# edouardlp/Mask-RCNN-CoreML

Measured on AMD Instinct MI355X. Metric: images/sec (1024x1024, COCO-80), higher is better.
Workload: dtype f32x3

## Files before the change

mask-rcnn-coreml_amd/csrc/conv_dispatch.hip:

```cpp
#include "conv_device.h"
#include "knobs.h"

namespace mrcnn {

void conv_mfma_launch(hipStream_t s, const ConvArgs& a, int mode, int bn, bool wide_waves);
void conv_pp_launch(hipStream_t s, const ConvArgs& a, int mode);
void conv_chain_launch(hipStream_t s, const ConvArgs& p, const ConvArgs& q, int parts, bool wlds, int n_cus);

static inline int conv_wdtype(const ConvDesc& d) { return d.wdtype < 0 ? d.dtype : d.wdtype; }
static inline bool conv_is_split(const ConvDesc& d) { return d.dtype == MRCNN_F32 && (conv_wdtype(d) == MRCNN_F16 || conv_wdtype(d) == MRCNN_F32X3); }
static inline int conv_split_parts(const ConvDesc& d) { return conv_wdtype(d) == MRCNN_F32X3 ? 3 : 2; }
static inline bool conv_is_f16(const ConvDesc& d) { return d.dtype == MRCNN_F16 && (d.wdtype < 0 || d.wdtype == MRCNN_F16) && !d.out_f32; }
static inline bool is_pointwise(const ConvDesc& d) { return d.KH == 1 && d.KW == 1 && d.stride == 1 && !d.padH && !d.padW; }
static inline bool is_3x3_same(const ConvDesc& d) { return d.KH == 3 && d.KW == 3 && d.stride == 1 && d.padH == 1 && d.padW == 1; }
static inline bool dense_in(const ConvDesc& d, int h, int w, int c) { return d.H == h && d.W == w && d.Cin == c && d.in_sW == c && d.in_sH == (long)w * c && d.in_sB == (long)h * w * c; }
static inline bool dense_out(const ConvDesc& d, int h, int w, int c) { return d.OH == h && d.OW == w && d.Cout == c && d.out_sP == c && d.out_sB == (long)h * w * c; }
static inline bool plain_epilogue(const ConvDesc& d, int act) { return !d.out2 && !d.deconv2 && !d.sel_partial && !d.head_w && d.res_shift == 0 && d.act == act && d.scale && d.shift; }
static inline bool fills_chip(long tiles, int n_cus) { return tiles * 8 >= (long)n_cus * 7; }

static thread_local ConvProfile* g_prof = nullptr;
void conv_set_profiler(ConvProfile* p) { g_prof = p; }
static thread_local int* g_range_flag = nullptr;
void conv_set_range_flag(int* device_flag) { g_range_flag = device_flag; }
void ConvProfile::reset()
{
    for (auto& s : by_tile) s = Slot();
    for (auto& s : by_group) s = Slot();
    by_shape.clear();
    pending.clear();
    used = 0;
}
void ConvProfile::collect()
{
    for (auto& pd : pending) {
        float ms = 0;
        HIP_CHECK(hipEventElapsedTime(&ms, pool[pd.e0], pool[pd.e1]));
        by_tile[pd.tile].launches += 1;
        by_tile[pd.tile].ms += ms;
        by_tile[pd.tile].flops += pd.flops;
        by_tile[pd.tile].bytes += pd.bytes;
        Slot& sh = by_shape[pd.shape];
        sh.launches += 1; sh.ms += ms; sh.flops += pd.flops; sh.bytes += pd.bytes;
        Slot& gr = by_group[pd.group == 1 ? 1 : 0];
        gr.launches += 1; gr.ms += ms; gr.flops += pd.flops; gr.bytes += pd.bytes;
    }
    pending.clear();
    used = 0;
}
ConvProfile::~ConvProfile()
{
    for (auto e : pool) (void)hipEventDestroy(e);
}
static double conv_algorithmic_bytes(const ConvDesc& d, const ConvDesc* sc = nullptr)
{
    const double es = d.dtype == MRCNN_F16 ? 2.0 : 4.0;
    const double ws = conv_wdtype(d) == MRCNN_F32 ? 4.0 : 2.0;
    const double M = (double)d.B * d.OH * d.OW;
    const double ncols = d.deconv2 ? 4.0 * d.Cout : d.Cout;
    double b = 0;
    if (d.algo_k > 0) b += (double)d.B * d.H * d.W * 16.0;
    else b += (d.KH * d.KW == 1 ? M : (double)d.B * d.H * d.W) * d.Cin * es;
    b += ncols * d.KH * d.KW * (d.algo_k > 0 ? (double)d.algo_k / (d.KH * d.KW) : (double)d.Cin) * ws;
    if (d.res) b += M * d.Cout * es / (d.res_shift ? 4.0 : 1.0);
    if (sc) b += M * sc->Cin * es + (double)d.Cout * sc->Cin * ws;
    if (d.head_w) b += M * d.head_cols * 4.0;
    else if (!d.sel_partial) b += M * ncols * (d.out_f32 ? 4.0 : es);
    return b;
}
static int prof_event(ConvProfile* p, hipStream_t s)
{
    if (p->used == (int)p->pool.size()) {
        hipEvent_t e;
        HIP_CHECK(hipEventCreate(&e));
        p->pool.push_back(e);
    }
    HIP_CHECK(hipEventRecord(p->pool[p->used], s));
    return p->used++;
}
struct ProfScope {
    ConvProfile* const prof = (g_prof && g_prof->active) ? g_prof : nullptr;
    const hipStream_t s;
    const int e0;
    explicit ProfScope(hipStream_t s_) : s(s_), e0(prof ? prof_event(prof, s_) : 0) {}
    explicit operator bool() const { return prof != nullptr; }
    void finish(ConvTileClass tile, double flops, int M, int N, int K, int group, double bytes) const
    {
        const int e1 = prof_event(prof, s);
        prof->pending.push_back({tile, flops, e0, e1, {M, N, K, tile}, group, bytes});
    }
};

int conv_n_tile(int Cout)
{
    if (Cout > 64) return 128;
    if (Cout > 32) return 64;
    return 32;
}

static int& g_min_blocks = knob("conv_min_blocks", nullptr, 448);
static int& g_min_blocks_split = knob("conv_min_blocks_split", nullptr, 256, "conv_min_blocks");
static inline int min_blocks_for(bool split_mode) { return split_mode ? g_min_blocks_split : g_min_blocks; }
static int& g_direct = knob("conv_direct", "MRCNN_DIRECT", 3);
static int& g_stem = knob("conv_stem", "MRCNN_STEM", 1);
static int& g_tail_dbg = knob("conv_tail_dbg", "MRCNN_TAIL_DBG", 0);
static int& g_tail = knob("conv_tail", "MRCNN_TAIL", 0);
static int& g_bneck = knob("conv_bneck", "MRCNN_BNECK", 1);
static int& g_bneck_stage = knob("conv_bneck_stage", "MRCNN_BNECK_STAGE", 0);
static int& g_c3h = knob("conv_c3h", "MRCNN_C3H", 1);
int conv_c3h_mode() { return g_c3h; }
bool conv_bneck_enabled() { return g_bneck != 0; }
static int& g_scfuse = knob("conv_scfuse", "MRCNN_SCFUSE", 1);
static int& g_sel_wave = knob("mask_sel_wave", "MRCNN_SEL_WAVE", 1);
int conv_sel_part_cols() { return g_sel_wave ? 64 : 128; }
static int& g_kchunk = knob("conv_kchunk", "MRCNN_KCHUNK", 1);
static int& g_ksplit = knob("conv_ksplit", "MRCNN_KSPLIT", 1);
static int& g_ksplit_below = knob("conv_ksplit_below", "MRCNN_KSPLIT_BELOW", 256);
static int& g_halo = knob("conv_halo", "MRCNN_HALO", 1);
bool conv_halo_enabled() { return g_halo != 0; }
static int& g_chain = knob("conv_chain", "MRCNN_CHAIN", 1);
static int& g_tn4 = knob("conv_tn4", nullptr, -1);

static int& g_pp = knob("conv_pp", "MRCNN_PP", 1);
static int& g_pp_min_tiles = knob("conv_pp_min_tiles", "MRCNN_PP_MIN_TILES", 512);
static int& g_pp_min_kt = knob("conv_pp_min_kt", "MRCNN_PP_MIN_KT", 16);
static int& g_pp_dbg = knob("conv_pp_dbg", "MRCNN_PP_DBG", 0);
static int& g_pp_min_fill = knob("conv_pp_min_fill", "MRCNN_PP_MIN_FILL", 85);
static int& g_pp_split = knob("conv_pp_split", "MRCNN_PP_SPLIT", 0);

static void conv_fill_args(const ConvDesc& d, ConvArgs& a)
{
    const bool half = d.dtype == MRCNN_F16;
    a.in = d.in; a.wgt = d.wgt; a.scale = d.scale; a.shift = d.shift; a.res = d.res; a.out = d.out; a.out2 = d.out2;
    a.in_sB = d.in_sB; a.in_sH = d.in_sH; a.in_sW = d.in_sW;
    a.res_sB = d.res_sB; a.res_sH = d.res_sH; a.res_sW = d.res_sW;
    a.out_sB = d.out_sB; a.out_sP = d.out_sP; a.out_sH = d.out_sH; a.out_sW = d.out_sW;
    a.out2_sB = d.out2_sB; a.out2_sP = d.out2_sP;
    a.B = d.B; a.H = d.H; a.W = d.W; a.Cin = d.Cin; a.KH = d.KH; a.KW = d.KW; a.stride = d.stride; a.padH = d.padH; a.padW = d.padW;
    a.OH = d.OH; a.OW = d.OW; a.Cout = d.Cout;
    a.ncols = d.deconv2 ? 4 * d.Cout : d.Cout;
    a.Ktot = d.KH * d.KW * d.Cin;
    const long M = (long)d.B * d.OH * d.OW;
    MRCNN_REQUIRE(M > 0 && M < (1L << 31) - 256, MRCNN_ERR_SHAPE, "conv: M out of range");
    a.M = (int)M;
    a.res_shift = d.res_shift; a.act = d.act; a.n_split = d.n_split; a.deconv2 = d.deconv2;
    a.out_f32 = (!half || d.out_f32) ? 1 : 0;
    a.range_flag = g_range_flag;
    a.dbg = g_pp_dbg;
    a.sel_w = d.sel_w; a.sel_cid = d.sel_cid; a.sel_partial = d.sel_partial;
    a.kchunks = 1; a.ksplit = 1; a.ks_scratch = nullptr; a.ks_count = nullptr;
    a.sel_part_cols = 128;
    a.sc_in = nullptr; a.sc_wgt = nullptr; a.sc_scale = nullptr; a.sc_shift = nullptr;
    a.sc_in_sB = a.sc_in_sH = a.sc_in_sW = 0; a.sc_H = a.sc_W = a.sc_Cin = 0; a.sc_stride = 1;
}

int conv_k_chunks(const ConvDesc& d)
{
    if (!g_kchunk || !conv_is_split(d) || d.KH != 1 || d.KW != 1 || d.Cin < 2048 || d.Cin % 32 != 0 || d.head_w) return 1;
    int n = d.Cin >= 8192 ? 8 : 4;
    while ((d.Cin / 32) % n) n >>= 1;
    return n;
}

static constexpr size_t KS_BYTES = 64u << 20;
static constexpr int KS_TILES = 8192;
static thread_local ConvScratch* g_scratch = nullptr;
void conv_set_scratch(ConvScratch* c) { g_scratch = c; }
size_t ConvScratch::ks_bytes() { return KS_BYTES; }
void ConvScratch::alloc()
{
    ks_buf.alloc(KS_BYTES);
    ks_cnt.alloc(KS_TILES * sizeof(unsigned));
    HIP_CHECK(hipMemset(ks_cnt.p, 0, KS_TILES * sizeof(unsigned)));
}
ConvScratch* conv_current_scratch() { return g_scratch; }

static int conv_vec_ok(const ConvDesc& d, const ConvArgs& a)
{
    const bool half = d.dtype == MRCNN_F16;
    auto al = [](const void* p, size_t n) { return (reinterpret_cast<uintptr_t>(p) & (n - 1)) == 0; };
    const int cpt = half ? 8 : 4;
    return a.ncols % cpt == 0 && d.out2 == nullptr && d.out_sP % cpt == 0 && d.out_sB % cpt == 0 && al(d.out, 16) &&
               (!d.scale || al(d.scale, 16)) && (!d.shift || al(d.shift, 16)) &&
               (!d.res || (d.res_sW % cpt == 0 && d.res_sH % cpt == 0 && d.res_sB % cpt == 0 && al(d.res, 16))) &&
               (!d.deconv2 || (d.Cout % cpt == 0 && d.out_sH % cpt == 0 && d.out_sW % cpt == 0));
}

static bool conv_shortcut_fusable(const ConvDesc& m, const ConvDesc& sc)
{
    if (!conv_is_split(m) || !conv_is_split(sc) || conv_wdtype(m) != conv_wdtype(sc)) return false;
    if (m.KH != 1 || m.KW != 1 || sc.KH != 1 || sc.KW != 1 || m.padH || m.padW || sc.padH || sc.padW || m.stride != 1) return false;
    if (m.B != sc.B || m.OH != sc.OH || m.OW != sc.OW || m.Cout != sc.Cout || m.Npad != sc.Npad || sc.Cin % 32 != 0) return false;
    if (sc.act != ACT_NONE || sc.res || sc.out2 || sc.deconv2 || sc.sel_partial || sc.head_w || m.out2 || m.deconv2 || m.sel_partial || m.head_w || m.act == ACT_SIGMOID) return false;
    if (m.res != sc.out || m.res_shift != 0 || m.res_sW != sc.out_sP || m.res_sB != sc.out_sB || m.res_sH != (long)m.OW * m.res_sW) return false;
    if (sc.out_sB != (long)sc.OH * sc.OW * sc.out_sP) return false;
    return true;
}

static bool conv_shortcut_rides(const ConvDesc& d_in, const ConvDesc* sc)
{
    bool fuse = sc && g_scfuse && conv_shortcut_fusable(d_in, *sc) && conv_k_chunks(d_in) == 1 && conv_k_chunks(*sc) == 1;
    if (fuse) {
        const int bn_max = conv_n_tile(d_in.Cout);
        int bn = bn_max;
        const long tiles_m = ((long)d_in.B * d_in.OH * d_in.OW + BM_DEFAULT - 1) / BM_DEFAULT;
        while (bn > 32 && tiles_m * (d_in.Npad / bn) < min_blocks_for(true)) bn >>= 1;
        ConvDesc probe = d_in;
        probe.res = nullptr;
        ConvArgs pa;
        conv_fill_args(probe, pa);
        if (bn < 64 || g_direct < 2 || !conv_vec_ok(probe, pa)) fuse = false;
#ifndef MRCNN_CONV_ABLATE
        if (g_pp_dbg) fuse = false;
#endif
    }
    return fuse;
}

void conv_forward(hipStream_t s, const ConvDesc& d_in, const ConvDesc* sc)
{
    const bool fuse = conv_shortcut_rides(d_in, sc);
    if (sc && !fuse) conv_forward(s, *sc, nullptr);
    ConvDesc d = d_in;
    if (fuse) { d.res = nullptr; d.res_sB = d.res_sH = d.res_sW = 0; }
    const bool half = d.dtype == MRCNN_F16;
    const int wdtype = conv_wdtype(d);
    if (half && g_c3h && (d.head_w || d.prefer_c3h || g_c3h == 2) && conv3x3h_eligible(d)) {
        const int n_cus_c3h = device_cu_count();
        const ProfScope prof(s);
        conv3x3h_launch(s, d, g_range_flag, n_cus_c3h);
        if (prof) {
            const double M = (double)d.B * d.OH * d.OW;
            prof.finish(TILE_C3H, 2.0 * M * d.Cout * 9.0 * d.Cin, (int)M, d.Cout, 9 * d.Cin, d.group, conv_algorithmic_bytes(d));
        }
        return;
    }
    const bool split = conv_is_split(d);
    const int parts = conv_split_parts(d);
    MRCNN_REQUIRE(d.dtype == MRCNN_F32 || half, MRCNN_ERR_UNSUPPORTED, "conv: dtype %d", d.dtype);
    MRCNN_REQUIRE(wdtype == d.dtype || split, MRCNN_ERR_UNSUPPORTED, "conv: activation dtype %d with filter dtype %d", d.dtype, wdtype);
    const int bk = half ? 64 : 32;
    MRCNN_REQUIRE(d.Cin % bk == 0, MRCNN_ERR_SHAPE, "conv: Cin %d not a multiple of %d", d.Cin, bk);
    ConvArgs a;
    conv_fill_args(d, a);
    MRCNN_REQUIRE(!d.sel_partial || (d.deconv2 && d.sel_w && d.sel_cid && d.Cout % 128 == 0 && d.Npad == 4 * d.Cout && !d.out2),
                  MRCNN_ERR_INVALID, "conv: the selected-class mode needs a 2x2 transposed convolution with Cout a multiple of 128");
    const int bn_max = conv_n_tile(a.ncols);
    MRCNN_REQUIRE(d.Npad % bn_max == 0 && d.Npad >= a.ncols, MRCNN_ERR_SHAPE, "conv: Npad %d incompatible with tile %d", d.Npad, bn_max);
    a.tiles_m = (a.M + BM_DEFAULT - 1) / BM_DEFAULT;
    int bn = bn_max;
    while (bn > 32 && !d.sel_partial && (long)a.tiles_m * (d.Npad / bn) < min_blocks_for(split)) bn >>= 1;
    if (fuse) {
        a.sc_in = sc->in; a.sc_wgt = sc->wgt; a.sc_scale = sc->scale; a.sc_shift = sc->shift;
        a.sc_in_sB = sc->in_sB; a.sc_in_sH = sc->in_sH; a.sc_in_sW = sc->in_sW;
        a.sc_H = sc->H; a.sc_W = sc->W; a.sc_Cin = sc->Cin; a.sc_stride = sc->stride;
    }
    a.kchunks = d.sel_partial ? 1 : conv_k_chunks(d);
    if (a.kchunks > 1 && g_ksplit && (long)a.tiles_m * (d.Npad / bn_max) < g_ksplit_below) {
        int bs = bn_max;
        while (bs > 32 && (long)a.tiles_m * (d.Npad / bs) * a.kchunks < min_blocks_for(true)) bs >>= 1;
        const long tiles = (long)a.tiles_m * (d.Npad / bs);
        if (g_scratch && g_scratch->ks_buf.p && tiles <= KS_TILES && (size_t)tiles * a.kchunks * BM_DEFAULT * bs * 4 <= KS_BYTES) {
            bn = bs;
            a.ksplit = a.kchunks;
            a.ks_scratch = g_scratch->ks_buf.as<float>();
            a.ks_count = g_scratch->ks_cnt.as<unsigned>();
        }
    }
    a.vec_ok = conv_vec_ok(d, a);
    a.tiles_n = d.Npad / bn;
    MRCNN_REQUIRE(!d.sel_partial || (bn == 128 && a.vec_ok), MRCNN_ERR_INVALID, "conv: the selected-class mode needs the 128-wide vector epilogue");
    a.direct = (g_direct && (half || g_direct > 1) && a.vec_ok && !d.out2 && !d.deconv2 && d.act != ACT_SIGMOID && (!half || !a.out_f32)) ? 1 : 0;
    MRCNN_REQUIRE(!fuse || (a.direct && bn >= 64), MRCNN_ERR_INVALID, "conv: fused shortcut without the direct epilogue (conv_forward's own check should have said so)");
    if (a.direct && half && g_direct > 2) a.direct = 2;
    if (d.sel_partial && g_sel_wave && bn == 128 && a.vec_ok && d.act != ACT_SIGMOID && d.Cout % 64 == 0) { a.direct = 1; a.sel_part_cols = 64; }
    int pp_bn = 0;
    {
        const long tiles = (long)((a.M + 255) / 256) * (d.Npad / 256);
        const long rounds = (tiles + 255) / 256;
        const bool fills = tiles >= g_pp_min_tiles && tiles * 100 >= rounds * 256 * g_pp_min_fill;
        const int bk_pp = half ? 64 : 32;
        if (g_pp && (half || (split && g_pp_split)) && d.Cin % bk_pp == 0 && a.Ktot / bk_pp >= g_pp_min_kt && d.Npad % 256 == 0 && fills &&
            a.kchunks == 1 && !fuse && a.vec_ok && (!half || !a.out_f32) && !d.deconv2 && !d.out2 && d.act != ACT_SIGMOID && d.H < 32760 && d.W < 32760)
            pp_bn = 256;
    }
    if (pp_bn) { a.tiles_m = (a.M + 255) / 256; a.tiles_n = d.Npad / pp_bn; }
    const bool wide_waves = split && bn == 128 && !d.sel_partial && (a.kchunks > 1 || fuse || (g_tn4 < 0 ? a.Ktot / bk >= 64 : g_tn4 != 0));
    const ProfScope prof(s);
    const bool halo = g_halo && d.wgt_halo && a.vec_ok && conv_halo_eligible(d);
    MRCNN_REQUIRE(!d.head_w || (halo && conv_halo_head_eligible(d)), MRCNN_ERR_INVALID, "conv: a fused head needs the halo kernel (layer not eligible, or switched off)");
    if (halo) {
        const int n_cus = device_cu_count();
        pp_bn = 0;
        (void)conv_halo_forward(s, a, d, parts, n_cus);
    } else
    if (pp_bn) conv_pp_launch(s, a, half ? 0 : parts);
    else conv_mfma_launch(s, a, half ? 0 : (split ? parts : 1), bn, wide_waves);
    if (prof) {
        const double k = (d.algo_k > 0 ? d.algo_k : a.Ktot) + (fuse ? sc->Cin : 0);
        const ConvTileClass tile = halo ? TILE_HALO : pp_bn == 256 ? TILE_PP_256x256 : (wide_waves ? TILE_128x128_4WAVE : (bn == 128 ? TILE_128x128 : (bn == 64 ? TILE_128x64 : TILE_128x32)));
        prof.finish(tile, 2.0 * (double)a.M * (double)a.ncols * k, a.M, a.ncols, a.Ktot, d.group, conv_algorithmic_bytes(d, fuse ? sc : nullptr));
    }
    HIP_CHECK(hipGetLastError());
}

bool conv_stem_enabled() { return g_stem != 0; }
bool conv_stem_eligible(const ConvDesc& d)
{
    const bool half = conv_is_f16(d);
    const int pxc = half ? 8 : 4;
    return (conv_is_split(d) || half) && d.KH == 7 && d.KW == 1 && d.Cin == 8 * pxc && d.stride == 2 && d.padH == 0 && d.padW == 0 && d.Cout == 64 && d.Npad == 64 &&
           d.act == ACT_RELU && !d.res && !d.out2 && !d.deconv2 && d.in_sW == pxc && d.in_sH == (long)d.W * pxc && d.in_sB == (long)d.H * d.W * pxc &&
           d.OH == (d.H - 7) / 2 + 1 && d.OW == (d.W - 7) / 2 + 1;
}

void conv_stem_forward(hipStream_t s, const ConvDesc& d, void* pooled, int PH, int PW)
{
    MRCNN_REQUIRE(conv_stem_eligible(d) && pooled && PH == (d.OH + 1) / 2 && PW == (d.OW + 1) / 2, MRCNN_ERR_INVALID, "conv_stem_forward: not the stem layer");
    const int n_cus = device_cu_count();
    const ProfScope prof(s);
    conv_stem_launch(s, d.in, d.B, d.H, d.W, d.wgt, d.scale, d.shift, d.OH, d.OW, pooled, PH, PW,
                     d.dtype == MRCNN_F16 ? 1 : conv_split_parts(d), g_range_flag, n_cus, g_stem != 2);
    if (prof) {
        const long M = (long)d.B * d.OH * d.OW;
        const double k = d.algo_k > 0 ? d.algo_k : d.KH * d.KW * d.Cin;
        const double by = (double)d.B * d.H * d.W * 16.0 + 64.0 * k * 2.0 + (double)d.B * PH * PW * 64.0 * (d.dtype == MRCNN_F16 ? 2.0 : 4.0);
        prof.finish(TILE_128x64, 2.0 * (double)M * 64.0 * k, (int)M, 64, d.KH * d.KW * d.Cin, d.group, by);
    }
}

bool conv_tail_fusable(const ConvDesc& d3, const ConvDesc& d1)
{
    if (!conv_is_split(d3) || !conv_is_split(d1) || conv_wdtype(d3) != conv_wdtype(d1)) return false;
    if (!d3.wgt_halo || !d1.wgt_halo || !conv_halo_eligible(d3) || d3.head_w || !conv_halo_tail_geometry_ok(d3.H, d3.W)) return false;
    if (d3.Npad != 256 || d3.act != ACT_RELU) return false;
    if (!conv_halo_tail_packable(d1.KH, d1.KW, d1.Cin, d1.Npad) || d1.Cout != 1024 || !is_pointwise(d1)) return false;
    if (d1.deconv2 || d1.out2 || d1.sel_partial || d1.act == ACT_SIGMOID || d1.res_shift || d1.head_w) return false;
    if (d1.in != d3.out || d1.B != d3.B || d1.OH != d3.OH || d1.OW != d3.OW) return false;
    if (!dense_out(d3, d3.OH, d3.OW, 256) || !dense_in(d1, d3.OH, d3.OW, 256)) return false;
    return true;
}

bool conv_chain_fusable(const ConvDesc& dP, const ConvDesc& dQ, const ConvDesc* sc)
{
    if (!conv_is_split(dP) || !conv_is_split(dQ) || conv_wdtype(dP) != conv_wdtype(dQ)) return false;
    const int C = dQ.Cout, H = dP.OH, W = dP.OW;
    if (!(C == 64 || C == 128) || dQ.Npad != C || dP.Cin != C || dP.Cout != 4 * C || dP.Npad != 4 * C) return false;
    if (!is_pointwise(dP) || !is_pointwise(dQ) || dP.B != dQ.B) return false;
    if (!plain_epilogue(dP, ACT_RELU) || !plain_epilogue(dQ, ACT_RELU) || dQ.res) return false;
    if (!dense_in(dP, H, W, C) || !dense_out(dP, H, W, 4 * C) || dQ.in != dP.out || !dense_in(dQ, H, W, 4 * C) || !dense_out(dQ, H, W, C)) return false;
    if (conv_k_chunks(dP) != 1 || conv_k_chunks(dQ) != 1) return false;
    auto al = [](const void* p) { return (reinterpret_cast<uintptr_t>(p) & 15) == 0; };
    if (!al(dP.in) || !al(dP.out) || !al(dQ.out) || !al(dP.wgt) || !al(dQ.wgt) || !al(dP.scale) || !al(dP.shift) || !al(dQ.scale) || !al(dQ.shift)) return false;
    if (sc) {
        if (!g_scfuse || !conv_shortcut_fusable(dP, *sc) || conv_k_chunks(*sc) != 1 || !sc->scale || !sc->shift) return false;
        if (C == 64 && sc->Cin != 64) return false;
        if (!al(sc->in) || !al(sc->wgt) || !al(sc->scale) || !al(sc->shift) || sc->in_sW % 4 || sc->in_sH % 4 || sc->in_sB % 4 || sc->Npad != 4 * C) return false;
    } else {
        if (!dP.res || !al(dP.res) || dP.res_sW != 4 * C || dP.res_sH != (long)W * 4 * C || dP.res_sB != (long)H * W * 4 * C) return false;
    }
    return true;
}

void conv_forward_chain(hipStream_t s, const ConvDesc& dP, const ConvDesc& dQ, const ConvDesc* sc)
{
    const long tiles = ((long)dP.B * dP.OH * dP.OW + 127) / 128;
    const bool sc_rides = g_chain >= 3 ? sc != nullptr && conv_chain_fusable(dP, dQ, sc) : conv_shortcut_rides(dP, sc);
    const int n_cus = device_cu_count();
    bool chain = g_chain && g_direct >= 2 && conv_chain_fusable(dP, dQ, sc_rides ? sc : nullptr) && (g_chain >= 2 || (dQ.Cout == 64 && fills_chip(tiles, n_cus)));
#ifndef MRCNN_CONV_ABLATE
    if (g_pp_dbg) chain = false;
#endif
    if (!chain) {
        conv_forward(s, dP, sc);
        conv_forward(s, dQ);
        return;
    }
    if (sc && !sc_rides) { conv_forward(s, *sc); sc = nullptr; }
    ConvDesc d = dP;
    if (sc) { d.res = nullptr; d.res_sB = d.res_sH = d.res_sW = 0; }
    ConvArgs aP, aQ;
    conv_fill_args(d, aP);
    conv_fill_args(dQ, aQ);
    if (sc) {
        aP.sc_in = sc->in; aP.sc_wgt = sc->wgt; aP.sc_scale = sc->scale; aP.sc_shift = sc->shift;
        aP.sc_in_sB = sc->in_sB; aP.sc_in_sH = sc->in_sH; aP.sc_in_sW = sc->in_sW;
        aP.sc_H = sc->H; aP.sc_W = sc->W; aP.sc_Cin = sc->Cin; aP.sc_stride = sc->stride;
    }
    const ProfScope prof(s);
    conv_chain_launch(s, aP, aQ, conv_split_parts(dP), dQ.Cout == 64, n_cus);
    if (prof) {
        const double fl = 2.0 * (double)aP.M * ((double)aP.ncols * (aP.Ktot + (sc ? sc->Cin : 0)) + (double)aQ.ncols * aQ.Ktot);
        prof.finish(sc ? TILE_128x128_4WAVE : TILE_128x128, fl, aP.M, aP.ncols, aP.Ktot, dP.group,
                    conv_algorithmic_bytes(d, sc) + conv_algorithmic_bytes(dQ) - (double)aP.M * dQ.Cin * 4.0);
    }
    HIP_CHECK(hipGetLastError());
}

void conv_forward_tail(hipStream_t s, const ConvDesc& d3, const ConvDesc& d1, const ConvDesc* sc, const ConvDesc* q)
{
    const int n_cus = device_cu_count();
    const long tiles = ((long)d3.B * d3.OH * d3.OW + 127) / 128;
    ConvArgs a3, a1;
    bool fuse = g_tail && g_halo && g_scratch && conv_tail_fusable(d3, d1) && fills_chip(tiles, n_cus);
    if (sc && fuse) { conv_forward(s, *sc); sc = nullptr; }
    if (fuse) {
        conv_fill_args(d3, a3);
        conv_fill_args(d1, a1);
        a3.vec_ok = conv_vec_ok(d3, a3);
        a1.vec_ok = conv_vec_ok(d1, a1);
        a3.tiles_m = a1.tiles_m = 0; a3.tiles_n = a1.tiles_n = 0; a3.direct = a1.direct = 1;
        a1.dbg = g_tail_dbg;
        fuse = a3.vec_ok && a1.vec_ok && a3.dbg == 0;
    }
    if (!fuse) {
        conv_forward(s, d3);
        if (q) conv_forward_chain(s, d1, *q, sc);
        else conv_forward(s, d1, sc);
        return;
    }
    const ProfScope prof(s);
    (void)conv_halo_forward(s, a3, d3, conv_split_parts(d3), n_cus, &a1, d1.wgt_halo);
    if (prof) {
        const double fl = 2.0 * (double)a3.M * ((double)a3.ncols * a3.Ktot + (double)a1.ncols * a1.Ktot);
        ConvDesc d3n = d3; d3n.sel_partial = (float*)1;
        prof.finish(TILE_HALO_TAIL, fl, a3.M, a1.ncols, a3.Ktot + a1.Ktot, d3.group, conv_algorithmic_bytes(d3n) + conv_algorithmic_bytes(d1) - (double)a3.M * d1.Cin * 4.0);
    }
    HIP_CHECK(hipGetLastError());
    if (q) conv_forward(s, *q);
}

bool conv_bneck_fusable(const ConvDesc& da, const ConvDesc& db, const ConvDesc& dc)
{
    if (!conv_is_f16(da) || !conv_is_f16(db) || !conv_is_f16(dc)) return false;
    const int C = da.Cout, H = da.H, W = da.W;
    if (!(C == 64 || C == 128 || C == 256) || !bneck_geometry_ok(C, H, W)) return false;
    if (!plain_epilogue(da, ACT_RELU) || !plain_epilogue(db, ACT_RELU) || !plain_epilogue(dc, ACT_RELU) || da.res || db.res) return false;
    if (!is_pointwise(da) || !dense_in(da, H, W, 4 * C) || !dense_out(da, H, W, C)) return false;
    if (!is_3x3_same(db) || db.in != da.out || !dense_in(db, H, W, C) || !dense_out(db, H, W, C)) return false;
    if (!is_pointwise(dc) || dc.in != db.out || !dense_in(dc, H, W, C) || !dense_out(dc, H, W, 4 * C)) return false;
    if (dc.res != da.in || dc.res_sW != 4 * C || dc.res_sH != (long)W * 4 * C || dc.res_sB != (long)H * W * 4 * C) return false;
    if (dc.out == da.in) return false;
    if (da.B != db.B || da.B != dc.B) return false;
    return true;
}

void conv_bneck_forward(hipStream_t s, const ConvDesc& da, const ConvDesc& db, const ConvDesc& dc)
{
    const int n_cus = device_cu_count();
    const int C_ = da.Cout;
    const long ntiles = (long)da.B * (da.H / (C_ == 256 ? 8 : 16)) * (da.W / 16);
    if (!g_bneck || !conv_bneck_fusable(da, db, dc) || (g_bneck < 3 && !fills_chip(ntiles, n_cus))) {
        conv_forward(s, da);
        conv_forward_tail(s, db, dc, nullptr);
        return;
    }
    const ProfScope prof(s);
    bneck_launch(s, da.Cout, da.in, dc.out, da.B, da.H, da.W, da.wgt, db.wgt, dc.wgt, da.scale, da.shift, db.scale, db.shift, dc.scale, dc.shift,
                 g_range_flag, n_cus, g_bneck >= 2 ? nullptr : db.wgt_frag, g_bneck >= 2 ? nullptr : dc.wgt_frag, g_bneck >= 2 ? nullptr : da.wgt_frag);
    if (prof) {
        const double M = (double)da.B * da.H * da.W, C = da.Cout;
        const double fl = 2.0 * M * (4 * C * C + 9 * C * C + 4 * C * C);
        prof.finish(TILE_BNECK, fl, (int)M, 4 * da.Cout, 17 * da.Cout, da.group, 2.0 * M * 4 * C * 2.0 + 17.0 * C * C * 2.0);
    }
}

void conv_bneck_stage_forward(hipStream_t s, const BneckTriple* blocks, int n, const void* layers_dev, unsigned* done)
{
    const int n_cus = device_cu_count();
    bool stage = n >= 2 && g_bneck == 1 && g_bneck_stage && layers_dev && done && g_range_flag;
    if (stage) {
        const ConvDesc& a0 = blocks[0].a;
        const long ntiles = (long)a0.B * (a0.H / 8) * (a0.W / 16);
        stage = a0.Cout == 256 && fills_chip(ntiles, n_cus);
        for (int i = 0; i < n && stage; ++i) {
            const BneckTriple& t = blocks[i];
            stage = conv_bneck_fusable(t.a, t.b, t.c) && t.a.wgt_frag && t.b.wgt_frag && t.c.wgt_frag && t.a.Cout == 256 && t.a.B == a0.B && t.a.H == a0.H && t.a.W == a0.W;
            if (i > 0) stage = stage && t.a.in == blocks[i - 1].c.out && (i < 2 || t.c.out == blocks[i - 2].c.out);
        }
        stage = stage && blocks[1].c.out == a0.in;
    }
    if (!stage) {
        for (int i = 0; i < n; ++i) conv_bneck_forward(s, blocks[i].a, blocks[i].b, blocks[i].c);
        return;
    }
    const ConvDesc& a0 = blocks[0].a;
    const ProfScope prof(s);
    bneck_stage_launch(s, layers_dev, n, const_cast<void*>(a0.in), blocks[0].c.out, a0.B, a0.H, a0.W, done, g_range_flag, n_cus);
    if (prof) {
        const double M = (double)a0.B * a0.H * a0.W, C = a0.Cout;
        const double fl = 2.0 * M * (4 * C * C + 9 * C * C + 4 * C * C) * n;
        prof.finish(TILE_BNECK, fl, (int)M, 4 * a0.Cout, 17 * a0.Cout * n, a0.group, (2.0 * M * 4 * C * 2.0 + 17.0 * C * C * 2.0) * n);
    }
}

bool conv_bneck_first_fusable(const ConvDesc& da, const ConvDesc& db, const ConvDesc& dc, const ConvDesc& ds)
{
    if (!conv_is_f16(da) || !conv_is_f16(db) || !conv_is_f16(dc) || !conv_is_f16(ds)) return false;
    const int C = da.Cout, H = da.H, W = da.W;
    if (C != 64 || da.Cin != C || !bneck_geometry_ok(C, H, W)) return false;
    if (!plain_epilogue(da, ACT_RELU) || !plain_epilogue(db, ACT_RELU) || !plain_epilogue(dc, ACT_RELU) || !plain_epilogue(ds, ACT_NONE) || da.res || db.res || ds.res) return false;
    if (!is_pointwise(da) || !dense_in(da, H, W, C) || !dense_out(da, H, W, C)) return false;
    if (!is_pointwise(ds) || ds.in != da.in || !dense_in(ds, H, W, C) || !dense_out(ds, H, W, 4 * C)) return false;
    if (!is_3x3_same(db) || db.in != da.out || !dense_in(db, H, W, C) || !dense_out(db, H, W, C)) return false;
    if (!is_pointwise(dc) || dc.in != db.out || !dense_in(dc, H, W, C) || !dense_out(dc, H, W, 4 * C)) return false;
    if (dc.res != ds.out || dc.res_sW != 4 * C || dc.res_sH != (long)W * 4 * C || dc.res_sB != (long)H * W * 4 * C) return false;
    if (dc.out == da.in || da.B != db.B || da.B != dc.B || da.B != ds.B) return false;
    return true;
}

void conv_bneck_first_forward(hipStream_t s, const ConvDesc& da, const ConvDesc& db, const ConvDesc& dc, const ConvDesc& ds)
{
    const int n_cus = device_cu_count();
    const long ntiles = (long)da.B * (da.H / 16) * (da.W / 16);
    if (!g_bneck || !conv_bneck_first_fusable(da, db, dc, ds) || (g_bneck < 3 && !fills_chip(ntiles, n_cus))) {
        conv_forward(s, da);
        conv_forward_tail(s, db, dc, &ds);
        return;
    }
    const ProfScope prof(s);
    bneck_launch(s, da.Cout, da.in, dc.out, da.B, da.H, da.W, da.wgt, db.wgt, dc.wgt, da.scale, da.shift, db.scale, db.shift, dc.scale, dc.shift,
                 g_range_flag, n_cus, nullptr, nullptr, nullptr, ds.wgt, ds.scale, ds.shift);
    if (prof) {
        const double M = (double)da.B * da.H * da.W, C = da.Cout;
        const double fl = 2.0 * M * (C * C + 9 * C * C + 4 * C * C + 4 * C * C);
        prof.finish(TILE_BNECK, fl, (int)M, 4 * da.Cout, 18 * da.Cout, da.group, M * C * 2.0 + M * 4 * C * 2.0 + 18.0 * C * C * 2.0);
    }
}

}
```

mask-rcnn-coreml_amd/csrc/engine.h:

```cpp
#pragma once
#include <functional>
#include <map>
#include <mutex>
#include <memory>
#include <string>
#include <vector>

#include "kernels.h"

namespace mrcnn {

struct MrcwTensor {
    int dtype = 0;
    std::vector<uint32_t> dims;
    const unsigned char* data = nullptr;
    size_t nbytes = 0;
    size_t count() const { size_t n = 1; for (auto d : dims) n *= d; return n; }
};
struct MrcwFile {
    std::string path;
    std::vector<unsigned char> buf;
    std::map<std::string, int64_t> ints;
    std::map<std::string, double> doubles;
    std::map<std::string, std::string> strings;
    std::map<std::string, MrcwTensor> tensors;
    void load(const std::string& path);
    int64_t get_int(const std::string& k) const;
    int64_t get_int(const std::string& k, int64_t dflt) const;
    double get_double(const std::string& k, double dflt) const;
    std::string get_string(const std::string& k) const;
    const MrcwTensor& tensor(const std::string& name) const;
    std::vector<float> floats(const std::string& name) const;
};

inline int mode_act(int mode) { return (mode == MRCNN_F32S || mode == MRCNN_F32X3) ? MRCNN_F32 : mode; }
inline int mode_wgt(int mode) { return mode == MRCNN_F32 ? MRCNN_F32 : (mode == MRCNN_F32X3 ? MRCNN_F32X3 : MRCNN_F16); }

struct PackedConv {
    DevBuf wgt, scale, shift;
    std::vector<float> h_scale, h_shift;
    DevBuf wgt_halo;
    DevBuf wgt_c3h;
    DevBuf wgt_frag;
    int Cin = 0, Cout = 0, KH = 1, KW = 1, Npad = 0;
    int dtype = MRCNN_F32;
    int wdtype = MRCNN_F32;
};

struct Tensor4 {
    void* p = nullptr;
    int H = 0, W = 0, C = 0;
    long sB() const { return (long)H * W * C; }
};

using Op = std::function<void(hipStream_t, int )>;

struct SplitGroup {
    std::string name;
    int exp = 0;
    bool fixed = false;
    float absmax = 0.f;
    long long small = 0, inexact = 0, counted = 0;
};
struct ScaledOp {
    const PackedConv* pc = nullptr;
    int g_in = 0, g_out = 0;
    DevBuf scale, shift;
};
using SplitObserver = std::function<void(hipStream_t, int, const void*, size_t)>;

struct Arena {
    char* base = nullptr;
    size_t off = 0;
    void* alloc_e(size_t n_elems, int dtype) { return alloc_b(n_elems * (dtype == MRCNN_F16 ? 2 : 4)); }
    float* alloc_f(size_t n_floats)
    {
        size_t bytes = (n_floats * 4 + 255) / 256 * 256;
        char* r = base ? base + off : nullptr;
        off += bytes;
        return reinterpret_cast<float*>(r);
    }
    void* alloc_b(size_t bytes)
    {
        bytes = (bytes + 255) / 256 * 256;
        char* r = base ? base + off : nullptr;
        off += bytes;
        return r;
    }
};

struct ClassifierHead {
    int nc = 0, pool = 7, C = 256, cap = 0, dtype = MRCNN_F32;
    PackedConv fc1, fc2, fc3;
    DevBuf arena;
    void *h1 = nullptr, *h2 = nullptr, *stage_in = nullptr;
    float *lb = nullptr, *probs = nullptr, *bbox = nullptr, *cls6 = nullptr;
    int mode = MRCNN_F32;
    ScaledOp sop[3];
    int grp[3] = {-1, -1, -1};
    SplitObserver observe;
    void load(const MrcwFile& f, int capacity_rows, int mode);
    void forward(hipStream_t s, const void* pooled_nhwc, int n, float* cls6_out, long cls6_stride);
};

struct MaskHead {
    int nc = 0, pool = 14, C = 256, cap = 0, dtype = MRCNN_F32;
    PackedConv conv[4], deconv, final_full;
    DevBuf final_w, final_b;
    DevBuf arena;
    void *t0 = nullptr, *t1 = nullptr, *feat = nullptr, *stage_in = nullptr;
    float* full = nullptr;
    int mode = MRCNN_F32;
    ScaledOp sop[5];
    int grp[5] = {-1, -1, -1, -1, -1};
    SplitObserver observe;
    void load(const MrcwFile& f, int capacity_rows, int mode);
    void forward_features(hipStream_t s, const void* pooled_nhwc, int n, const int32_t* sel_cid = nullptr, float* sel_partial = nullptr);
    void forward_full(hipStream_t s, int n);
};


struct StageTimer {
    bool enabled = false;
    std::vector<std::string> names;
    std::vector<hipEvent_t> ev;
    std::map<std::string, float> ms;
    void begin(hipStream_t s);
    void mark(hipStream_t s, const char* name);
    void finish();
    ~StageTimer();
};

struct JpegScratch {
    uint8_t* pinned = nullptr;
    size_t pinned_bytes = 0;
    DevBuf staged, planes, rgb;
    DevBuf ent_work;
    JpegScratch() = default;
    JpegScratch(const JpegScratch&) = delete;
    JpegScratch& operator=(const JpegScratch&) = delete;
    ~JpegScratch() { if (pinned) (void)hipHostFree(pinned); }
};

struct Model {
    int kind = 0;
    int max_batch = 1;
    bool mode_defaulted = false;
    int mode = MRCNN_F32;
    int dtype = MRCNN_F32;
    MrcwFile file;
    hipStream_t stream = nullptr;
    bool own_stream = false;
    std::string arch;
    int H = 0, W = 0, nc = 0, pre_nms = 0, max_prop = 0, max_det = 0, na = 3, A = 0, K = 0;
    float mean[3] = {0, 0, 0};
    float prop_std[4], det_std[4];
    float prop_nms_thr = 0.7f, det_score_thr = 0.7f, det_nms_thr = 0.3f;
    int cls_pool = 7, mask_pool = 14;
    double roi_img_w = 0, roi_img_h = 0;
    std::map<std::string, PackedConv> convs;
    DevBuf anchors;
    DevBuf rpn_head_frag;
    ClassifierHead cls_head;
    MaskHead mask_head;
    DevBuf arena;
    std::vector<Op> trunk_ops;
    std::vector<std::unique_ptr<DevBuf>> stage_tabs;
    struct Tap { void* base; long per_image; int dtype; int group = -1; };
    std::map<std::string, Tap> taps;
    uint8_t* d_rgb = nullptr;
    void* stem_in = nullptr;
    DevBuf fit_src;
    size_t fit_table_off = 0;
    uint8_t* fit_pack = nullptr;
    size_t fit_pack_bytes = 0;
    bool fit_mixed = false;
    JpegScratch jpeg;
    float *rpn_logits = nullptr, *rpn_probs = nullptr, *rpn_deltas = nullptr, *rois = nullptr;
    float *cls6 = nullptr, *detections = nullptr, *mask_out = nullptr;
    void *pooled = nullptr, *pooled_mask = nullptr;
    Tensor4 P[4];
    ProposalWorkspace prop_ws;
    DetectionWorkspace det_ws;
    MaskSelectWorkspace msel_ws;
    float* mask_partial = nullptr;
    bool fuse_mask_tail = true;
    StageTimer timer;
    ConvProfile conv_profile;
    ConvScratch conv_scratch;
    struct GraphSlot { hipGraph_t graph = nullptr; hipGraphExec_t exec = nullptr; int eager_runs = 0; };
    std::map<int, GraphSlot> graphs;
    bool use_graph = false;
    std::vector<SplitGroup> sgroups;
    std::vector<std::unique_ptr<ScaledOp>> sops;
    int g_P[4] = {-1, -1, -1, -1}, g_rpn[5] = {-1, -1, -1, -1, -1}, g_pooled = -1, g_pooled_mask = -1;
    int calib_phase = 0;
    DevBuf calib_buf;
    bool split_calibrated = false;
    int new_split_group(const std::string& name, bool fixed = false);
    ScaledOp* new_scaled_op(const PackedConv* pc, int g_in, int g_out);
    void apply_split_exponents();
    void observe_split(hipStream_t s, int group, const void* x, size_t n);
    void calibrate_split(const uint8_t* rgb, int batch, int h, int w, int memspace, bool apply);
    void measure_split_groups(const uint8_t* rgb, int batch, int h, int w, int memspace, bool fit, bool resident);
    static int split_exponent_for(float absmax);
    bool recover_range(int batch, int h, int w, bool fit);
    long range_recoveries = 0;
    bool exponents_from_artefact = false;
    DevBuf range_flag;
    long range_overflows = 0;
    long graph_launches = 0;
    hipEvent_t ev_p0 = nullptr, ev_p1 = nullptr;
    double gpu_busy_ms = 0;
    long predict_calls = 0;
    struct PipeSlot {
        DevBuf rgb, det, mask, flag;
        hipEvent_t ev_in = nullptr, ev_done = nullptr;
        int batch = 0;
        bool busy = false;
    };
    PipeSlot pipe[2];
    hipStream_t pipe_in = nullptr, pipe_out = nullptr;
    long pipe_submitted = 0, pipe_collected = 0;
    void submit(const uint8_t* rgb_host, int batch, int h, int w);
    void collect(float* det_host, float* masks_host, int* batch_out);
    std::mutex eval_mu;

    ~Model();
    void load(int kind, const std::string& path, int max_batch, int dtype);
    void build_maskrcnn();
    void predict(const uint8_t* rgb, int batch, int h, int w, int memspace, float* det, float* masks, bool sync, bool fit = false, bool resident = false);
    void predict_images(const mrcnn_image* images, int batch, int memspace, float* det, float* masks);
    void predict_tiles(const mrcnn_image* images, int n_images, const mrcnn_tile* tiles, int n_tiles, int memspace, float* det, float* masks);
    void enqueue_pipeline(hipStream_t s, int batch, const int* fit = nullptr);
    void drop_graphs();
    void read_tensor(const std::string& name, int image, float* dst, int64_t cap, int64_t* count);
};

}

struct mrcnn_model {
    mrcnn::Model m;
};
```

mask-rcnn-coreml_amd/csrc/engine_internal.h:

```cpp
#pragma once
#include "engine.h"

namespace mrcnn {

float half_to_float(uint16_t h);
void upload(DevBuf& d, const std::vector<float>& h);
PackedConv pack_conv_oihw(const MrcwFile& f, const std::string& conv, const std::string& bn, int mode);
PackedConv pack_conv1(const MrcwFile& f, int mode);
PackedConv pack_stacked_1x1(const MrcwFile& f, const std::vector<std::string>& names, int mode);
PackedConv pack_deconv2(const MrcwFile& f, const std::string& name, int mode);
void init_scaled_op(ScaledOp& op, const PackedConv* pc, int g_in, int g_out);

struct ConvView {
    void* p = nullptr;
    int H = 0, W = 0;
    long sB = 0, sH = 0, sW = 0;
};
inline ConvView dense_view(const void* p, int H, int W, int C)
{
    return {const_cast<void*>(p), H, W, (long)H * W * C, (long)W * C, (long)C};
}
inline ConvView view_of(const Tensor4& t) { return dense_view(t.p, t.H, t.W, t.C); }

enum : unsigned { RETILED_NONE = 0, RETILED_HALO = 1, RETILED_C3H = 2, RETILED_FRAG = 4, RETILED_ALL = 7 };

inline ConvDesc make_conv_desc(const PackedConv& pc, const float* scale, const float* shift, const ConvView& in, const ConvView& out,
                               int stride, int pad, int act, unsigned retiled)
{
    ConvDesc d;
    d.dtype = pc.dtype; d.wdtype = pc.wdtype;
    d.in = in.p; d.H = in.H; d.W = in.W; d.Cin = pc.Cin;
    d.in_sB = in.sB; d.in_sH = in.sH; d.in_sW = in.sW;
    d.wgt = pc.wgt.p; d.KH = pc.KH; d.KW = pc.KW; d.stride = stride; d.padH = d.padW = pad;
    if (retiled & RETILED_HALO) d.wgt_halo = pc.wgt_halo.p;
    if (retiled & RETILED_C3H) d.wgt_c3h = pc.wgt_c3h.p;
    if (retiled & RETILED_FRAG) d.wgt_frag = pc.wgt_frag.p;
    d.scale = scale; d.shift = shift;
    d.act = act;
    d.out = out.p; d.OH = out.H; d.OW = out.W; d.Cout = pc.Cout; d.Npad = pc.Npad;
    d.out_sB = out.sB; d.out_sP = out.sW;
    return d;
}
inline void set_residual(ConvDesc& d, const ConvView& res, int res_shift)
{
    d.res = res.p; d.res_sB = res.sB; d.res_sH = res.sH; d.res_sW = res.sW; d.res_shift = res_shift;
}

void run_conv_dense(hipStream_t s, const PackedConv& pc, const void* in, int B, int H, int W, void* out, int stride,
                    int pad, int act, const void* res = nullptr, int out_f32 = 0, const ScaledOp* sop = nullptr);

template <class F>
void lay_out_twice(DevBuf& arena, F&& lay_out)
{
    Arena ar;
    lay_out(ar, false);
    arena.alloc(ar.off);
    ar.base = arena.as<char>();
    ar.off = 0;
    lay_out(ar, true);
}

}
```

mask-rcnn-coreml_amd/csrc/engine_weights.hip:

```cpp
#include "engine_internal.h"
#include "conv_pack.h"

#include <math.h>
#include <string.h>

#include <fstream>

namespace mrcnn {

float half_to_float(uint16_t h)
{
    const uint32_t sign = (uint32_t)(h & 0x8000u) << 16;
    uint32_t exp = (h >> 10) & 0x1Fu, man = h & 0x3FFu, f;
    if (exp == 0) {
        if (man == 0) f = sign;
        else {
            exp = 113;
            while ((man & 0x400u) == 0) { man <<= 1; --exp; }
            man &= 0x3FFu;
            f = sign | (exp << 23) | (man << 13);
        }
    } else if (exp == 31) f = sign | 0x7F800000u | (man << 13);
    else f = sign | ((exp + 112) << 23) | (man << 13);
    float r;
    memcpy(&r, &f, 4);
    return r;
}

void MrcwFile::load(const std::string& p)
{
    path = p;
    std::ifstream in(p, std::ios::binary | std::ios::ate);
    MRCNN_REQUIRE(in.good(), MRCNN_ERR_IO, "cannot open model artefact '%s'", p.c_str());
    const std::streamsize sz = in.tellg();
    in.seekg(0);
    buf.resize((size_t)sz);
    in.read(reinterpret_cast<char*>(buf.data()), sz);
    MRCNN_REQUIRE(in.good() && sz >= 16 && memcmp(buf.data(), "MRCW", 4) == 0, MRCNN_ERR_IO, "'%s' is not a .mrcw file", p.c_str());
    size_t pos = 4;
    auto need = [&](size_t n) { MRCNN_REQUIRE(pos + n <= buf.size(), MRCNN_ERR_IO, "'%s': truncated header", p.c_str()); };
    auto rd = [&](void* dst, size_t n) { need(n); memcpy(dst, buf.data() + pos, n); pos += n; };
    uint32_t ver, n_meta, n_t;
    rd(&ver, 4); rd(&n_meta, 4); rd(&n_t, 4);
    MRCNN_REQUIRE(ver == 1, MRCNN_ERR_IO, "'%s': unsupported .mrcw version %u", p.c_str(), ver);
    for (uint32_t i = 0; i < n_meta; ++i) {
        uint16_t kl; rd(&kl, 2);
        need(kl);
        std::string k((const char*)buf.data() + pos, kl); pos += kl;
        uint8_t t; rd(&t, 1);
        if (t == 0) { int64_t v; rd(&v, 8); ints[k] = v; }
        else if (t == 1) { double v; rd(&v, 8); doubles[k] = v; }
        else { uint32_t sl; rd(&sl, 4); need(sl); strings[k] = std::string((const char*)buf.data() + pos, sl); pos += sl; }
    }
    struct Ent { std::string name; MrcwTensor t; uint64_t off; };
    std::vector<Ent> ents;
    for (uint32_t i = 0; i < n_t; ++i) {
        uint16_t nl; rd(&nl, 2);
        need(nl);
        Ent e;
        e.name = std::string((const char*)buf.data() + pos, nl); pos += nl;
        uint8_t dt, nd; rd(&dt, 1); rd(&nd, 1);
        e.t.dtype = dt;
        e.t.dims.resize(nd);
        for (int d = 0; d < nd; ++d) rd(&e.t.dims[d], 4);
        uint64_t nb; rd(&e.off, 8); rd(&nb, 8);
        e.t.nbytes = (size_t)nb;
        ents.push_back(std::move(e));
    }
    const size_t base = (pos + 63) / 64 * 64;
    for (auto& e : ents) {
        MRCNN_REQUIRE(base + e.off + e.t.nbytes <= buf.size(), MRCNN_ERR_IO, "'%s': tensor %s out of bounds", p.c_str(), e.name.c_str());
        MRCNN_REQUIRE(e.t.dtype == 0 || e.t.dtype == 2, MRCNN_ERR_IO, "'%s': tensor %s has unsupported dtype", p.c_str(), e.name.c_str());
        e.t.data = buf.data() + base + e.off;
        tensors[e.name] = e.t;
    }
}
int64_t MrcwFile::get_int(const std::string& k) const
{
    auto it = ints.find(k);
    MRCNN_REQUIRE(it != ints.end(), MRCNN_ERR_IO, "'%s': missing integer metadata key '%s'", path.c_str(), k.c_str());
    return it->second;
}
int64_t MrcwFile::get_int(const std::string& k, int64_t dflt) const
{
    auto it = ints.find(k);
    return it == ints.end() ? dflt : it->second;
}
double MrcwFile::get_double(const std::string& k, double dflt) const
{
    auto it = doubles.find(k);
    if (it != doubles.end()) return it->second;
    auto ii = ints.find(k);
    return ii == ints.end() ? dflt : (double)ii->second;
}
std::string MrcwFile::get_string(const std::string& k) const
{
    auto it = strings.find(k);
    MRCNN_REQUIRE(it != strings.end(), MRCNN_ERR_IO, "'%s': missing string metadata key '%s'", path.c_str(), k.c_str());
    return it->second;
}
const MrcwTensor& MrcwFile::tensor(const std::string& name) const
{
    auto it = tensors.find(name);
    MRCNN_REQUIRE(it != tensors.end(), MRCNN_ERR_IO, "'%s': missing tensor '%s'", path.c_str(), name.c_str());
    return it->second;
}
std::vector<float> MrcwFile::floats(const std::string& name) const
{
    const MrcwTensor& t = tensor(name);
    std::vector<float> v(t.count());
    if (t.dtype == 0) memcpy(v.data(), t.data, v.size() * 4);
    else {
        const uint16_t* h = reinterpret_cast<const uint16_t*>(t.data);
        for (size_t i = 0; i < v.size(); ++i) v[i] = half_to_float(h[i]);
    }
    return v;
}

void upload(DevBuf& d, const std::vector<float>& h)
{
    d.alloc(h.size() * 4);
    HIP_CHECK(hipMemcpy(d.p, h.data(), h.size() * 4, hipMemcpyHostToDevice));
}

static uint16_t float_to_half(float f)
{
    uint32_t x;
    memcpy(&x, &f, 4);
    const uint32_t sign = (x >> 16) & 0x8000u;
    x &= 0x7FFFFFFFu;
    if (x >= 0x7F800000u) return (uint16_t)(sign | 0x7C00u | (x > 0x7F800000u ? 0x200u : 0));
    if (x >= 0x477FF000u) return (uint16_t)(sign | 0x7C00u);
    if (x < 0x38800000u) {
        if (x < 0x33000000u) return (uint16_t)sign;
        const int e = (int)(x >> 23);
        uint32_t m = (x & 0x7FFFFFu) | 0x800000u;
        const int shift = 126 - e;
        const uint32_t half_m = m >> shift, rem = m & ((1u << shift) - 1), mid = 1u << (shift - 1);
        uint32_t r = half_m;
        if (rem > mid || (rem == mid && (half_m & 1))) ++r;
        return (uint16_t)(sign | r);
    }
    uint32_t r = ((x - 0x38000000u) >> 13);
    const uint32_t rem = x & 0x1FFFu;
    if (rem > 0x1000u || (rem == 0x1000u && (r & 1))) ++r;
    return (uint16_t)(sign | r);
}

static void upload_w(DevBuf& d, const std::vector<float>& h, int dtype, bool must_be_exact = false, const char* what = "")
{
    if (dtype != MRCNN_F16 && dtype != MRCNN_F32X3) { upload(d, h); return; }
    std::vector<uint16_t> hh(h.size());
    for (size_t i = 0; i < h.size(); ++i) {
        hh[i] = float_to_half(h[i]);
        if (must_be_exact) {
            const _Float16 back = __builtin_bit_cast(_Float16, hh[i]);
            MRCNN_REQUIRE((float)back == h[i], MRCNN_ERR_UNSUPPORTED,
                          "%s: filter value %.9g is not fp16-representable; MRCNN_F32S needs the fp16 filters the converter writes", what, h[i]);
        }
    }
    d.alloc(hh.size() * 2);
    HIP_CHECK(hipMemcpy(d.p, hh.data(), hh.size() * 2, hipMemcpyHostToDevice));
}

static void fold_bn(const MrcwFile& f, const std::string& conv, const std::string& bn, int Cout, int Npad,
                    std::vector<float>& scale, std::vector<float>& shift)
{
    const std::vector<float> bias = f.floats(conv + "/bias");
    MRCNN_REQUIRE((int)bias.size() == Cout, MRCNN_ERR_IO, "%s/bias has %zu entries, expected %d", conv.c_str(), bias.size(), Cout);
    scale.assign(Npad, 0.f);
    shift.assign(Npad, 0.f);
    if (bn.empty()) {
        for (int o = 0; o < Cout; ++o) { scale[o] = 1.f; shift[o] = bias[o]; }
        return;
    }
    const std::vector<float> g = f.floats(bn + "/gamma"), be = f.floats(bn + "/beta"), mu = f.floats(bn + "/mean"),
                             var = f.floats(bn + "/variance");
    const float eps = (float)f.get_double("bn_eps", 1e-3);
    for (int o = 0; o < Cout; ++o) {
        const float sc = g[o] / sqrtf(var[o] + eps);
        scale[o] = sc;
        shift[o] = (bias[o] - mu[o]) * sc + be[o];
    }
}

static PackedConv new_pack(int mode, int Cin, int Cout, int KH, int KW)
{
    PackedConv pc;
    pc.dtype = mode_act(mode); pc.wdtype = mode_wgt(mode);
    pc.Cin = Cin; pc.Cout = Cout; pc.KH = KH; pc.KW = KW;
    const int bn_tile = conv_n_tile(Cout);
    pc.Npad = (Cout + bn_tile - 1) / bn_tile * bn_tile;
    return pc;
}
static void finish_pack(PackedConv& pc, const std::vector<float>& w, const std::vector<float>& sc, const std::vector<float>& sh)
{
    upload_w(pc.wgt, w, pc.wdtype, pc.wdtype != pc.dtype, "MRCNN_F32S / MRCNN_F32X3");
    upload(pc.scale, sc);
    upload(pc.shift, sh);
    pc.h_scale = sc; pc.h_shift = sh;
}

PackedConv pack_conv_oihw(const MrcwFile& f, const std::string& conv, const std::string& bn, int dtype)
{
    const MrcwTensor& t = f.tensor(conv + "/kernel");
    MRCNN_REQUIRE(t.dims.size() == 4, MRCNN_ERR_IO, "%s/kernel is not 4-D", conv.c_str());
    const int O = t.dims[0], I = t.dims[1], KH = t.dims[2], KW = t.dims[3];
    const std::vector<float> k = f.floats(conv + "/kernel");
    PackedConv pc = new_pack(dtype, I, O, KH, KW);
    const std::vector<float> w = pack_filter_rows(O, I, KH, KW, pc.Npad, [&](int o, int y, int x, int i) { return k[(((size_t)o * I + i) * KH + y) * KW + x]; });
    std::vector<float> sc, sh;
    fold_bn(f, conv, bn, O, pc.Npad, sc, sh);
    finish_pack(pc, w, sc, sh);
    if (pc.wdtype != pc.dtype && conv_halo_packable(KH, KW, I, pc.Npad)) {
        conv_halo_pack(nullptr, pc.wgt.p, pc.Npad, I, pc.wgt_halo);
        HIP_CHECK(hipStreamSynchronize(nullptr));
    } else if (pc.wdtype != pc.dtype && conv_halo_tail_packable(KH, KW, I, pc.Npad) && O == pc.Npad) {
        conv_halo_pack(nullptr, pc.wgt.p, pc.Npad, I, pc.wgt_halo, 1);
        HIP_CHECK(hipStreamSynchronize(nullptr));
    }
    if (pc.dtype == MRCNN_F16 && pc.wdtype == MRCNN_F16 && conv3x3h_packable(KH, KW, I, O, pc.Npad)) {
        conv3x3h_pack(nullptr, pc.wgt.p, O, I, pc.wgt_c3h);
        HIP_CHECK(hipStreamSynchronize(nullptr));
    }
    if (pc.dtype == MRCNN_F16 && pc.wdtype == MRCNN_F16 && O == pc.Npad && bneck_frag_wanted(KH, KW, I, O)) {
        bneck_pack_frag(nullptr, pc.wgt.p, O, KH * KW * I, pc.wgt_frag);
        HIP_CHECK(hipStreamSynchronize(nullptr));
    }
    return pc;
}

PackedConv pack_conv1(const MrcwFile& f, int dtype)
{
    const MrcwTensor& t = f.tensor("conv1/kernel");
    MRCNN_REQUIRE(t.dims.size() == 4 && t.dims[1] == 3 && t.dims[2] == 7 && t.dims[3] == 7, MRCNN_ERR_IO, "conv1/kernel must be [O,3,7,7]");
    const int O = t.dims[0];
    const std::vector<float> k = f.floats("conv1/kernel");
    const int px = mode_act(dtype) == MRCNN_F16 ? 8 : 4;
    const int row = 8 * px;
    PackedConv pc = new_pack(dtype, row, O, 7, 1);
    std::vector<float> w((size_t)pc.Npad * 7 * row, 0.f);
    for (int o = 0; o < O; ++o)
        for (int ci = 0; ci < 3; ++ci)
            for (int y = 0; y < 7; ++y)
                for (int x = 0; x < 7; ++x)
                    w[((size_t)o * 7 + y) * row + x * px + ci] = k[(((size_t)o * 3 + ci) * 7 + y) * 7 + x];
    std::vector<float> sc, sh;
    fold_bn(f, "conv1", "bn_conv1", O, pc.Npad, sc, sh);
    finish_pack(pc, w, sc, sh);
    return pc;
}

PackedConv pack_stacked_1x1(const MrcwFile& f, const std::vector<std::string>& names, int dtype)
{
    int O = 0, I = -1;
    for (auto& n : names) {
        const MrcwTensor& t = f.tensor(n + "/kernel");
        MRCNN_REQUIRE(t.dims.size() == 2 || (t.dims.size() == 4 && t.dims[2] == 1 && t.dims[3] == 1), MRCNN_ERR_IO,
                      "%s/kernel is not an inner product / 1x1 kernel", n.c_str());
        MRCNN_REQUIRE(I < 0 || I == (int)t.dims[1], MRCNN_ERR_IO, "%s: input size mismatch", n.c_str());
        I = t.dims[1];
        O += t.dims[0];
    }
    PackedConv pc = new_pack(dtype, I, O, 1, 1);
    std::vector<float> w((size_t)pc.Npad * I, 0.f), sc(pc.Npad, 0.f), sh(pc.Npad, 0.f);
    int o0 = 0;
    for (auto& n : names) {
        const std::vector<float> k = f.floats(n + "/kernel"), b = f.floats(n + "/bias");
        memcpy(w.data() + (size_t)o0 * I, k.data(), k.size() * 4);
        for (size_t o = 0; o < b.size(); ++o) { sc[o0 + o] = 1.f; sh[o0 + o] = b[o]; }
        o0 += (int)b.size();
    }
    finish_pack(pc, w, sc, sh);
    return pc;
}

PackedConv pack_deconv2(const MrcwFile& f, const std::string& name, int dtype)
{
    const MrcwTensor& t = f.tensor(name + "/kernel");
    MRCNN_REQUIRE(t.dims.size() == 4 && t.dims[2] == 2 && t.dims[3] == 2, MRCNN_ERR_IO, "%s/kernel must be [I,O,2,2]", name.c_str());
    const int I = t.dims[0], O = t.dims[1];
    const std::vector<float> k = f.floats(name + "/kernel"), b = f.floats(name + "/bias");
    PackedConv pc = new_pack(dtype, I, O, 1, 1);
    pc.Npad = 4 * O;
    MRCNN_REQUIRE(pc.Npad % conv_n_tile(pc.Npad) == 0, MRCNN_ERR_SHAPE, "%s: 4*O must be a multiple of the N tile", name.c_str());
    const std::vector<float> w = pack_deconv2_rows(I, O, pc.Npad, [&](int dy, int dx, int o, int i) { return k[(((size_t)i * O + o) * 2 + dy) * 2 + dx]; });
    std::vector<float> sc(pc.Npad, 1.f), sh(pc.Npad);
    for (int dy = 0; dy < 2; ++dy)
        for (int dx = 0; dx < 2; ++dx)
            for (int o = 0; o < O; ++o) sh[(size_t)deconv2_row(dy, dx, o, O)] = b[o];
    finish_pack(pc, w, sc, sh);
    return pc;
}

void init_scaled_op(ScaledOp& op, const PackedConv* pc, int g_in, int g_out)
{
    op.pc = pc; op.g_in = g_in; op.g_out = g_out;
    upload(op.scale, pc->h_scale);
    upload(op.shift, pc->h_shift);
}

}
```

mask-rcnn-coreml_amd/csrc/kernels.h:

```cpp
#pragma once
#include <stddef.h>
#include <algorithm>
#include <map>
#include <tuple>
#include <vector>

#include "common.h"

namespace mrcnn {


struct ProposalWorkspace {
    int B = 0, A = 0, K = 0, Kpad = 0, max_keep = 0, nblk = 0, W = 0;
    uint32_t* keys = nullptr;
    uint32_t* hist = nullptr;
    uint32_t* blockhist = nullptr;
    uint32_t* state = nullptr;
    uint64_t* cand = nullptr;
    int32_t* topk_idx = nullptr;
    float* boxes = nullptr;
    uint64_t* nms_mask = nullptr;
    int32_t* keep_idx = nullptr;
    int32_t* keep_count = nullptr;
    static size_t bytes(int B, int A, int K, int max_keep);
    void bind(void* base, int B, int A, int K, int max_keep);
};

void proposal_forward(hipStream_t s, const ProposalWorkspace& ws, const float* probs, long probs_sB,
                      const float* deltas, long deltas_sB, const float* anchors, const float std4[4],
                      float nms_thr, float* rois, long rois_sB, long row_stride);

struct DetectionWorkspace {
    int B = 0, N = 0, max_det = 0, W = 0, Npad = 0;
    int32_t* count = nullptr;
    int32_t* src = nullptr;
    float* boxes = nullptr;
    float* score = nullptr;
    int32_t* cls = nullptr;
    uint64_t* nms_mask = nullptr;
    int32_t* keep_idx = nullptr;
    int32_t* keep_count = nullptr;
    static size_t bytes(int B, int N, int max_det);
    void bind(void* base, int B, int N, int max_det);
};

void detection_forward(hipStream_t s, const DetectionWorkspace& ws, const float* rois, long rois_sB,
                       long roi_stride, const float* cls6, long cls_sB, const float std4[4],
                       float score_thr, float nms_thr, int num_classes_hint, float* out, long out_sB,
                       long row_stride);

struct PyramidMaps {
    const void* data[4];
    int H[4], W[4];
    long sB[4];
    float mul[4] = {1.f, 1.f, 1.f, 1.f};
};
void roi_align_forward(hipStream_t s, const PyramidMaps& maps, int C, int layout_nhwc, const float* rois,
                       long rois_sB, long roi_stride, int n_rois, int B, int pool, double image_w,
                       double image_h, void* out, long out_sB, long out_row_stride, int dtype,
                       int32_t* row_flags = nullptr);

void letterbox_forward(hipStream_t s, const uint8_t* src, int h, int w, uint8_t* dst, int H, int W, int nh, int nw, int py, int px);
void preprocess_scalefit_forward(hipStream_t s, const uint8_t* src, int B, int h, int w, int H, int W, int nh, int nw, int py, int px, int pad,
                                 const float mean[3], void* out, int dtype);
struct ImageGeom {
    long long offset;
    int h, w, nh, nw, py, px;
    int pitch;
};
void preprocess_images_forward(hipStream_t s, const uint8_t* src, const ImageGeom* tab, int B, int H, int W, int pad, const float mean[3],
                               void* out, int dtype);
void paste_masks_forward(hipStream_t s, const float* det, long det_stride, const float* masks, int n, int S, int H, int W,
                         float thr, uint8_t* out);
void paste_masks_source_forward(hipStream_t s, const float* det, const float* masks, const ImageGeom* tab, int batch, int rows, int S,
                                int H, int W, long max_bytes, float thr, float* det_src, int4* boxes, uint8_t* out);
constexpr int RLE_SEGS = 16;
struct RleSeg { uint32_t count, last; };
void masks_rle_count_forward(hipStream_t s, const float* det, const float* masks, const ImageGeom* tab, int batch, int rows, int S, int H, int W,
                             float thr, float* det_src, int4* boxes, RleSeg* segs, uint32_t* nruns, long long* run_offsets, uint32_t* areas,
                             int32_t* bboxes);
void masks_rle_write_forward(hipStream_t s, const float* masks, const ImageGeom* tab, int batch, int rows, int S, float thr, const int4* boxes,
                             const RleSeg* segs, const long long* run_offsets, uint32_t* counts);
void unletterbox_boxes_forward(hipStream_t s, const float* det, const ImageGeom* tab, int batch, int rows, int H, int W, float* det_src, int4* boxes);

void instance_map_forward(hipStream_t s, const float* det, const float* masks, const ImageGeom* tab, int batch, int rows, int S, int H, int W,
                          long max_pixels, float thr, float min_score, float* det_src, int4* boxes, int16_t* map, uint32_t* visible);
void render_detections_forward(hipStream_t s, const float* det, const float* masks, const ImageGeom* tab, const uint8_t* const* srcs, int batch,
                               int rows, int S, int H, int W, long max_pixels, float thr, float min_score, int alpha, int stroke, float* det_src,
                               int4* boxes, uint8_t* out);

struct JpegComp {
    long long block0;
    long long plane0;
    int blocks_w, blocks_h;
    int width, height;
};
struct JpegDesc {
    long long out_offset;
    long long block0;
    long long chunk0;
    int h, w, ncomp, mode;
    int reserved[2];
    JpegComp comp[3];
    uint16_t quant[3][64];
};
static_assert(sizeof(JpegDesc) % 16 == 0 && offsetof(JpegDesc, quant) % 16 == 0, "JpegDesc: quant rows are loaded 16 bytes at a time");
void jpeg_decode_forward(hipStream_t s, const JpegDesc* tab, int batch, const int16_t* coef, long long total_blocks, uint8_t* planes,
                         long long total_chunks, uint8_t* out);

struct JpegEncDesc {
    const uint8_t* rgb;
    long long block0, blocks;
    int h, w, sampling, ncomp;
    int hs, vs, mcus_x, blocks_per_mcu;
    int header0, header_len;
    int reserved[4];
    uint16_t quant[2][64];
};
static_assert(sizeof(JpegEncDesc) % 16 == 0, "JpegEncDesc: a table of them keeps 16-byte alignment");
struct JpegEncHuffman {
    uint32_t dc[2][16];
    uint32_t ac[2][256];
    uint8_t zigzag_of[64];
};
constexpr int JPEG_ENC_CHUNK = 128;
constexpr int JPEG_ENC_BLOCK_BYTES = 208;
struct JpegEncBuffers {
    const JpegEncDesc* tab;
    const JpegEncHuffman* huff;
    const uint8_t* headers;
    int16_t* coef;
    uint32_t* block_bits;
    unsigned long long* block_scan;
    long long* image_chunk0;
    long long* image_bytes;
    uint32_t* stream;
    uint32_t* chunk_ff;
    unsigned long long* chunk_scan;
    long long* file_offsets;
    uint8_t* files;
    long long max_chunks, files_capacity;
};
void jpeg_encode_forward(hipStream_t s, const JpegEncBuffers& b, int batch, long long total_blocks);

struct PngDesc {
    const void* pixels;
    long long block0, blocks;
    long long n;
    int h, w;
    int header0, header_len;
};
static_assert(sizeof(PngDesc) % 16 == 0, "PngDesc: a table of them keeps 16-byte alignment");
struct PngBuffers {
    const PngDesc* tab;
    const uint8_t* headers;
    uint32_t* block_bits;
    unsigned long long* block_scan;
    unsigned long long* adler;
    long long* file_offsets;
    uint32_t* files;
    long long files_capacity;
};
void png_encode_forward(hipStream_t s, const PngBuffers& b, int batch, long long total_blocks, int format, int rows);

enum Act { ACT_NONE = 0, ACT_RELU = 1, ACT_SIGMOID = 2 };

struct ConvDesc {
    int dtype = MRCNN_F32;
    int out_f32 = 0;
    int wdtype = -1;
    const void* in = nullptr;
    int B = 0, H = 0, W = 0, Cin = 0;
    long in_sB = 0, in_sH = 0, in_sW = 0;
    const void* wgt = nullptr;
    const void* wgt_halo = nullptr;
    const void* wgt_frag = nullptr;
    const void* wgt_c3h = nullptr;
    int prefer_c3h = 0;
    int KH = 1, KW = 1, stride = 1, padH = 0, padW = 0;
    const float* scale = nullptr;
    const float* shift = nullptr;
    const void* res = nullptr;
    long res_sB = 0, res_sH = 0, res_sW = 0;
    int res_shift = 0;
    int act = ACT_NONE;
    void* out = nullptr;
    int OH = 0, OW = 0, Cout = 0, Npad = 0;
    long out_sB = 0, out_sP = 0;
    void* out2 = nullptr;
    int n_split = 0;
    long out2_sB = 0, out2_sP = 0;
    int deconv2 = 0;
    long out_sH = 0, out_sW = 0;
    int algo_k = 0;
    int group = 0;
    const float* sel_w = nullptr;
    const int32_t* sel_cid = nullptr;
    float* sel_partial = nullptr;
    const void* head_w = nullptr;
    const float* head_bias = nullptr;
    float* head_out = nullptr; float* head_out2 = nullptr;
    long head_out_sB = 0, head_out_sP = 0, head_out2_sB = 0, head_out2_sP = 0;
    int head_split = 0, head_cols = 0;
    float head_mul = 1.f;
};

enum ConvTileClass {
    TILE_128x128 = 0,
    TILE_128x64 = 1,
    TILE_128x32 = 2,
    TILE_128x128_4WAVE = 3,
    TILE_PP_256x256 = 4,
    TILE_HALO = 5,
    TILE_HALO_TAIL = 6,
    TILE_BNECK = 7,
    TILE_C3H = 8,
    TILE_CLASSES
};
struct ConvProfile {
    struct Slot { long launches = 0; double ms = 0, flops = 0, bytes = 0; };
    Slot by_tile[TILE_CLASSES];
    std::vector<hipEvent_t> pool;
    struct Shape { int M, N, K, tile; bool operator<(const Shape& o) const { return std::tie(M, N, K, tile) < std::tie(o.M, o.N, o.K, o.tile); } };
    std::map<Shape, Slot> by_shape;
    struct Pending { int tile; double flops; int e0, e1; Shape shape; int group = 0; double bytes = 0; };
    Slot by_group[2];
    std::vector<Pending> pending;
    int used = 0;
    bool active = false;
    void reset();
    void collect();
    ~ConvProfile();
};
void conv_set_profiler(ConvProfile* p);
void boxes_one_time_init();
void conv_set_range_flag(int* device_flag);
struct ConvScratch {
    DevBuf ks_buf, ks_cnt, park;
    void alloc();
    static size_t ks_bytes();
};
void conv_set_scratch(ConvScratch* c);
int conv_n_tile(int Cout);
void conv_forward(hipStream_t s, const ConvDesc& d, const ConvDesc* sc = nullptr);
struct ConvArgs;
void conv_halo_pack(hipStream_t s, const void* wgt_std, int Npad, int Cin, DevBuf& out, int taps = 9);
void conv_halo_pack_head(hipStream_t s, const void* wgt_std, int Npad, int Cin, DevBuf& out);
bool conv_halo_eligible(const ConvDesc& d);
bool conv_halo_head_eligible(const ConvDesc& d);
bool conv_halo_enabled();
bool conv_halo_packable(int KH, int KW, int Cin, int Npad);
int conv_halo_forward(hipStream_t s, ConvArgs a, const ConvDesc& d, int parts, int n_cus, const ConvArgs* tail = nullptr, const void* tail_w = nullptr);
bool conv_halo_tail_packable(int KH, int KW, int Cin, int Npad);
bool conv_halo_tail_geometry_ok(int H, int W);
bool conv_tail_fusable(const ConvDesc& d3, const ConvDesc& d1);
int conv_sel_part_cols();
void conv_forward_tail(hipStream_t s, const ConvDesc& d3, const ConvDesc& d1, const ConvDesc* sc = nullptr, const ConvDesc* q = nullptr);
bool conv_chain_fusable(const ConvDesc& dP, const ConvDesc& dQ, const ConvDesc* sc = nullptr);
void conv_forward_chain(hipStream_t s, const ConvDesc& dP, const ConvDesc& dQ, const ConvDesc* sc = nullptr);

bool conv_bneck_fusable(const ConvDesc& da, const ConvDesc& db, const ConvDesc& dc);
bool conv_bneck_first_fusable(const ConvDesc& da, const ConvDesc& db, const ConvDesc& dc, const ConvDesc& ds);
void conv_bneck_first_forward(hipStream_t s, const ConvDesc& da, const ConvDesc& db, const ConvDesc& dc, const ConvDesc& ds);
bool conv_bneck_enabled();
void conv_bneck_forward(hipStream_t s, const ConvDesc& da, const ConvDesc& db, const ConvDesc& dc);
bool bneck_geometry_ok(int C, int H, int W);
void bneck_launch(hipStream_t s, int C, const void* x, void* y, int B, int H, int W, const void* w1, const void* w2, const void* w3,
                  const float* s1, const float* h1, const float* s2, const float* h2, const float* s3, const float* h3, int* range_flag, int n_cus,
                  const void* w2f = nullptr, const void* w3f = nullptr, const void* w1f = nullptr,
                  const void* ws = nullptr, const float* ss = nullptr, const float* hs = nullptr);
void bneck_stage_launch(hipStream_t s, const void* layers_dev, int nlayers, void* pp0, void* pp1, int B, int H, int W, unsigned* done, int* range_flag, int n_cus);
size_t bneck_layer_record_bytes();
void bneck_layer_record(void* dst, const void* w1f, const void* w2f, const void* w3f, const float* s1, const float* h1, const float* s2, const float* h2,
                        const float* s3, const float* h3);
struct BneckTriple { ConvDesc a, b, c; };
void conv_bneck_stage_forward(hipStream_t s, const BneckTriple* blocks, int n, const void* layers_dev, unsigned* done);
void bneck_pack_frag(hipStream_t s, const void* wgt_std, int N, int K, DevBuf& out);
bool bneck_frag_wanted(int KH, int KW, int Cin, int Cout);

void conv3x3h_pack(hipStream_t s, const void* wgt_std, int N, int Cin, DevBuf& out);
bool conv3x3h_packable(int KH, int KW, int Cin, int Cout, int Npad);
bool conv3x3h_eligible(const ConvDesc& d);
void conv3x3h_launch(hipStream_t s, const ConvDesc& d, int* range_flag, int n_cus);
int conv_c3h_mode();

bool conv_stem_eligible(const ConvDesc& d);
bool conv_stem_enabled();
void conv_stem_forward(hipStream_t s, const ConvDesc& d, void* pooled, int PH, int PW);
void conv_stem_launch(hipStream_t s, const void* in, int B, int Hp, int Wp, const void* wgt, const float* scale, const float* shift, int CH, int CW,
                      void* out, int PH, int PW, int parts, int* range_flag, int n_cus, bool compact = true);

void preprocess_forward(hipStream_t s, const uint8_t* rgb, int B, int H, int W, int pad, const float mean[3],
                        void* out, int dtype);
void maxpool3x3s2_forward(hipStream_t s, const void* in, int B, int H, int W, int C, void* out, int OH, int OW, int dtype);
void softmax_pairs_forward(hipStream_t s, const float* logits, float* probs, long n_pairs);
void softmax_rows_forward(hipStream_t s, const float* logits, long ld, int nc, long n, float* probs);
void copy_columns_forward(hipStream_t s, const float* src, long ld, int c0, int ncols, long n, float* dst);
void classifier_postprocess_forward(hipStream_t s, const float* probs, const float* bbox, int nc, long n,
                                    float* out, long out_row_stride);
void nchw_to_nhwc_forward(hipStream_t s, const float* in, long n, int C, int H, int W, void* out, int dtype);
void nhwc_to_nchw_forward(hipStream_t s, const float* in, long n, int C, int H, int W, float* out);
void copy_rows_forward(hipStream_t s, const float* src, long src_stride, long n, long len, float* dst, long dst_stride);

struct MaskSelectWorkspace {
    int32_t* flags = nullptr;
    int32_t* mapping = nullptr;
    int32_t* kept = nullptr;
    int32_t* sel_cid = nullptr;
};
void mask_valid_rows_forward(hipStream_t s, const void* pooled, long pooled_sB, long row_stride, long row_len,
                             int D, int B, const MaskSelectWorkspace& ws, int dtype);
void mask_select_forward(hipStream_t s, const void* feat, long feat_sB, int HW, int C, const float* w,
                         const float* bias, int nc, const float* det, long det_sB, long det_stride, int D, int B,
                         const MaskSelectWorkspace& ws, float* out, long out_sB, long out_stride, int dtype);
void mask_select_classes(hipStream_t s, const float* det, long det_sB, long det_stride, int D, int B, int nc,
                         const MaskSelectWorkspace& ws, int32_t* sel_cid);
void mask_select_from_partials(hipStream_t s, const float* partial, int parts, int HW, const float* bias, int nc, const float* det,
                               long det_sB, long det_stride, int D, int B, const MaskSelectWorkspace& ws, float* out, long out_sB,
                               long out_stride);
void mask_select_from_full_forward(hipStream_t s, const float* masks, long masks_sB, int HW, int nc,
                                   const float* det, long det_sB, long det_stride, int D, int B,
                                   const MaskSelectWorkspace& ws, float* out, long out_sB, long out_stride);

using IouGroup = mrcnn_iou_group;
using MatchGroup = mrcnn_match_group;
void rle_prefix_forward(hipStream_t s, const uint32_t* counts, const long long* run_offsets, long n_rle, uint32_t* pre_b, uint32_t* pre_o,
                        unsigned long long* totals, uint32_t* areas, uint2* extent = nullptr);

struct RleDrawRec { long long r0; int nruns; uint32_t first, last; int y1, x1, y2, x2; int drawn; };
struct RleDrawJob {
    const RleDrawRec* rec;
    const uint32_t* pre_b;
    const ImageGeom* tab;
    int n_images, slots;
    int max_h, max_w;
};
void rle_draw_prepare(hipStream_t s, const long long* run_offsets, const unsigned long long* totals, const uint2* extent, const float* det,
                      float min_score, const RleDrawJob& job, RleDrawRec* rec, unsigned long long* bad);
void rle_decode_forward(hipStream_t s, const RleDrawJob& job, uint8_t* out);
void instance_map_rle_forward(hipStream_t s, const RleDrawJob& job, int16_t* map, uint32_t* visible);
void render_detections_rle_forward(hipStream_t s, const RleDrawJob& job, const uint8_t* const* srcs, int alpha, int stroke, uint8_t* out);
void rle_iou_forward(hipStream_t s, const uint32_t* d_b, const long long* d_off, const unsigned long long* d_total, const uint32_t* d_area,
                     const uint32_t* g_b, const uint32_t* g_o, const long long* g_off, const uint32_t* g_area, const uint8_t* g_crowd,
                     const IouGroup* groups, const long long* block_starts, int n_groups, long long n_blocks, uint32_t* inter, double* iou);
void box_iou_xywh_forward(hipStream_t s, const double* db, const double* gb, const uint8_t* g_crowd, const IouGroup* groups,
                          const long long* pair_starts, int n_groups, long long n_pairs, double* iou);
void coco_match_forward(hipStream_t s, const double* iou, const MatchGroup* groups, int n_groups, const int32_t* dt_idx, const double* dt_area,
                        const int32_t* gt_idx, const double* gt_area, const uint8_t* gt_crowd, const double* ranges, int A, const double* thrs, int T,
                        int32_t* dt_match, uint8_t* dt_ignore, int32_t* gt_match);

struct PolyRec { long long pt0; int npts, ann; };
struct PolyAnn { long long pt0, pt1; int poly0, h, w, pad; };
struct PolyBig { long long ann, offset, padded; };
constexpr int POLY_LDS_TOGGLES = MRCNN_POLY_LDS_TOGGLES;
void poly_count_forward(hipStream_t s, const double* xy, const int32_t* pt_poly, const PolyRec* polys, const PolyAnn* anns, long n_pts, long n_anns,
                        uint32_t* edge_cnt, long long* edge_start, long long* tog_off);
void poly_encode_lds_forward(hipStream_t s, const double* xy, const int32_t* pt_poly, const PolyRec* polys, const PolyAnn* anns, long n_anns,
                             const long long* edge_start, uint32_t* bnd, uint32_t* nb, uint32_t* nruns, uint32_t* areas, int32_t* bboxes);
void poly_encode_big_forward(hipStream_t s, const double* xy, const int32_t* pt_poly, const PolyRec* polys, const PolyAnn* anns,
                             const long long* edge_start, const PolyBig* big, const PolyBig* h_big, int n_big, unsigned long long* keys, int32_t* cov,
                             uint32_t* bnd, uint32_t* nb, uint32_t* nruns, uint32_t* areas, int32_t* bboxes);
void poly_offsets_forward(hipStream_t s, const uint32_t* nruns, long n, long long* run_offsets);
void poly_write_forward(hipStream_t s, const PolyAnn* anns, long n_anns, const long long* tog_off, const uint32_t* bnd, const uint32_t* nb,
                        const long long* run_offsets, uint32_t* counts);

constexpr int POLYGON_LDS_CORNERS = MRCNN_POLYGON_LDS_CORNERS;
struct PolygonImage { long long unit0; int h, w; };
struct PolygonSet {
    const uint32_t* pre_b;
    const long long* run_offsets;
    const unsigned long long* totals;
    const PolygonImage* tab;
    int n_images, slots;
    long long units;
    uint32_t* unit_cnt;
    unsigned long long* unit_start;
    long long* corner0;
};
void polygons_count_forward(hipStream_t s, const PolygonSet& set, unsigned long long* summary);
struct PolygonWork {
    uint32_t* corner;
    uint32_t *succ, *lead, *dist;
    uint32_t *head, *len;
    unsigned long long *ring_id, *vertex0;
    unsigned long long* sort; uint32_t* pad_size; unsigned long long* pad_start;
    uint32_t *next_a, *next_b; unsigned long long *md_a, *md_b;
};
void polygons_trace_forward(hipStream_t s, const PolygonSet& set, const PolygonWork& w, long long n_corners, long long most, long long* rle_rings);
void polygons_write_forward(hipStream_t s, const PolygonWork& w, long long n_corners, long long n_rings, long long* ring_offsets, long long* ring_areas,
                            int32_t* xy);

constexpr int COCO_ACC_CHUNK = MRCNN_COCO_ACC_CHUNK;
struct AccChunk { long long seg0; int seg_len, at; };
const uint32_t* coco_acc_sort_forward(hipStream_t s, const double* scores, const AccChunk* chunks, long n_chunks, long long longest,
                                      unsigned long long* keys_a, uint32_t* perm_a, unsigned long long* keys_b, uint32_t* perm_b);
void coco_acc_permute_forward(hipStream_t s, const uint32_t* perm, const int32_t* ranks, const uint8_t* matched, const uint8_t* ignore, long long n_dt,
                              int planes, uint8_t* code, int32_t* srank);
void coco_acc_scan_forward(hipStream_t s, const uint8_t* code, const int32_t* srank, const long long* cat_off, const long long* npig,
                           const int32_t* max_dets, const double* rec_thrs, long long n_dt, int K, int A, int M, int T, int R, double* precision,
                           double* recall);

}
```

mask-rcnn-coreml_amd/csrc/kernels_conv_chain.hip:

```cpp
#include "conv_device.h"

namespace mrcnn {

struct ChainArgs { ConvArgs p, q; };

__device__ __forceinline__ void chain_stage_acc(float* stage, const f32x16& acc, int l31, int kk)
{
#pragma unroll
    for (int q = 0; q < 4; ++q)
        *reinterpret_cast<float4*>(&stage[l31 * 32 + (((2 * q + kk) ^ (l31 & 7)) << 2)]) = make_float4(acc[4 * q], acc[4 * q + 1], acc[4 * q + 2], acc[4 * q + 3]);
}

struct ChainParts { f16x8 hi, lo, lo2; };
template <int PARTS>
__device__ __forceinline__ ChainParts chain_split(const uint4 u0, const uint4 u1)
{
    ChainParts p;
    if constexpr (PARTS == 3) split_hi_mid_lo(u0, u1, p.hi, p.lo, p.lo2);
    else { split_hi_lo(u0, u1, p.hi, p.lo); p.lo2 = p.lo; }
    return p;
}
template <int PARTS, int N>
__device__ __forceinline__ void chain_mfma_parts(f32x16 (&acc)[N], const uint4 (&bv)[N], const ChainParts& pt)
{
    const f16x8 hi = pt.hi, lo = pt.lo, lo2 = pt.lo2;
    _Pragma("unroll") for (int j = 0; j < N; ++j) acc[j] = __builtin_amdgcn_mfma_f32_32x32x16_f16(__builtin_bit_cast(f16x8, bv[j]), hi, acc[j], 0, 0, 0);
    _Pragma("unroll") for (int j = 0; j < N; ++j) acc[j] = __builtin_amdgcn_mfma_f32_32x32x16_f16(__builtin_bit_cast(f16x8, bv[j]), lo, acc[j], 0, 0, 0);
    if constexpr (PARTS == 3)
        _Pragma("unroll") for (int j = 0; j < N; ++j) acc[j] = __builtin_amdgcn_mfma_f32_32x32x16_f16(__builtin_bit_cast(f16x8, bv[j]), lo2, acc[j], 0, 0, 0);
}

template <int C, int PARTS, bool SC, bool WLDS>
__global__ __launch_bounds__(WLDS ? 512 : 256, WLDS ? 1 : 2) void k_conv_chain(const ChainArgs ca)
{
    static_assert(!WLDS || C == 64, "the LDS-resident form holds C = 64's filters");
    constexpr int NW = WLDS ? 8 : 4, C4 = 4 * C, KT = C / 32, TNP = 2, TNQ = C / 32;
    constexpr int A_BYTES = WLDS ? 0 : KT * 32 * 128;
    constexpr int W_BYTES = WLDS ? C4 * C * 2 : 0;
    constexpr int WF_BYTES = W_BYTES * (SC ? 3 : 2);
    __shared__ __attribute__((aligned(16))) unsigned char smem[WF_BYTES + NW * (A_BYTES + 32 * 32 * 4)];
    const ConvArgs& a = ca.p;
    const ConvArgs& aq = ca.q;
    const int t = threadIdx.x;
    const int wave = t >> 6, lane = t & 63;
    const int l31 = lane & 31, kk = lane >> 5;
    unsigned char* const As = smem + WF_BYTES + wave * A_BYTES;
    float* const stage = reinterpret_cast<float*>(smem + WF_BYTES + NW * A_BYTES) + wave * (32 * 32);
    const float* const in = static_cast<const float*>(a.in);
    const _Float16* const w3 = static_cast<const _Float16*>(a.wgt);
    const _Float16* const w1 = static_cast<const _Float16*>(aq.wgt);
    const float* const res = static_cast<const float*>(a.res);
    float* const out = static_cast<float*>(a.out);
    float* const outq = static_cast<float*>(aq.out);
    const _Float16* const wsc = static_cast<const _Float16*>(a.sc_wgt);
    const int swzb = (l31 >> 2) & 3;
    if constexpr (WLDS) {
        auto stage_filter = [&](unsigned char* dst, const _Float16* src, int rows, int K) {
            const int cpr = K / 8;
            for (int idx = t; idx < rows * cpr; idx += NW * 64) {
                const int r = idx / cpr, ch = idx - r * cpr;
                *reinterpret_cast<uint4*>(dst + ((ch >> 2) * rows + r) * 64 + (((ch & 3) ^ ((r >> 2) & 3)) << 4)) = *reinterpret_cast<const uint4*>(src + (long)r * K + ch * 8);
            }
        };
        stage_filter(smem, w3, C4, C);
        stage_filter(smem + W_BYTES, w1, C, C4);
        if constexpr (SC) stage_filter(smem + 2 * W_BYTES, wsc, C4, C);
        __syncthreads();
    }
    bool out_of_range = false, out_of_range_q = false;
    for (int row0 = (blockIdx.x * NW + wave) * 32; row0 < a.M; row0 += gridDim.x * NW * 32) {
    ChainParts ap[WLDS ? 2 * KT : 1];
    if constexpr (WLDS) {
        const int m = row0 + l31;
#pragma unroll
        for (int g = 0; g < 2 * KT; ++g) {
            uint4 u0 = make_uint4(0u, 0u, 0u, 0u), u1 = u0;
            if (m < a.M) { u0 = *reinterpret_cast<const uint4*>(in + (long)m * C + g * 16 + 8 * kk); u1 = *reinterpret_cast<const uint4*>(in + (long)m * C + g * 16 + 8 * kk + 4); }
            ap[g] = chain_split<PARTS>(u0, u1);
        }
    } else {
#pragma unroll
        for (int it = 0; it < C / 8; ++it) {
            const int idx = it * 64 + lane;
            const int r = idx / (C / 4), ch = idx - r * (C / 4);
            const int m = row0 + r;
            uint4 v = make_uint4(0u, 0u, 0u, 0u);
            if (m < a.M) v = *reinterpret_cast<const uint4*>(in + (long)m * C + ch * 4);
            *reinterpret_cast<uint4*>(As + (ch >> 3) * 4096 + r * 128 + (((ch & 7) ^ ((r >> 1) & 7)) << 4)) = v;
        }
        __builtin_amdgcn_wave_barrier();
    }

    const int swz = (l31 >> 1) & 7;
    const unsigned char* const la = As + l31 * 128;
    const int ca0 = ((0 + 2 * kk) ^ swz) << 4, ca1 = ((1 + 2 * kk) ^ swz) << 4, ca2 = ((4 + 2 * kk) ^ swz) << 4, ca3 = ((5 + 2 * kk) ^ swz) << 4;
    const int rrow = lane >> 3, c4 = (lane & 7) * 4;
    const bool relu = a.act == ACT_RELU, reluq = aq.act == ACT_RELU;
    bool ok[4];
    long mrow[4];
#pragma unroll
    for (int ps = 0; ps < 4; ++ps) { const int m = row0 + 8 * ps + rrow; ok[ps] = m < a.M; mrow[ps] = m; }

    const float* sc_row = nullptr;
    bool sc_ok = false;
    if constexpr (SC) {
        const int m = row0 + l31;
        sc_ok = m < a.M;
        const int ohw = a.OH * a.OW;
        const int mm = sc_ok ? m : 0;
        const int b = mm / ohw, rem = mm - b * ohw;
        const int oh = rem / a.OW, ow = rem - oh * a.OW;
        sc_row = static_cast<const float*>(a.sc_in) + (long)b * a.sc_in_sB + (long)(oh * a.sc_stride) * a.sc_in_sH + (long)(ow * a.sc_stride) * a.sc_in_sW + 8 * kk;
    }
    uint4 xr[SC && WLDS ? C / 4 : 1];
    if constexpr (SC && WLDS) {
#pragma unroll
        for (int i = 0; i < C / 4; ++i) {
            xr[i] = make_uint4(0u, 0u, 0u, 0u);
            if (sc_ok) xr[i] = *reinterpret_cast<const uint4*>(sc_row + (i >> 1) * 16 + (i & 1) * 4);
        }
    }

    f32x16 accQ[TNQ];
#pragma unroll
    for (int j = 0; j < TNQ; ++j)
#pragma unroll
        for (int e = 0; e < 16; ++e) accQ[j][e] = 0.0f;

    for (int nc = 0; nc < C4; nc += TNP * 32) {
        float4 rv[TNP][4];
        if constexpr (!SC) {
#pragma unroll
            for (int j = 0; j < TNP; ++j)
#pragma unroll
                for (int ps = 0; ps < 4; ++ps) {
                    rv[j][ps] = make_float4(0.f, 0.f, 0.f, 0.f);
                    if (res && ok[ps]) rv[j][ps] = *reinterpret_cast<const float4*>(res + mrow[ps] * C4 + nc + j * 32 + c4);
                }
        }
        f32x16 accP[TNP], accS[TNP];
#pragma unroll
        for (int j = 0; j < TNP; ++j)
#pragma unroll
            for (int e = 0; e < 16; ++e) { accP[j][e] = 0.0f; accS[j][e] = 0.0f; }
#pragma unroll
        for (int kt = 0; kt < KT; ++kt) {
#pragma unroll
            for (int g = 0; g < 2; ++g) {
                uint4 bv[TNP];
                if constexpr (WLDS) {
#pragma unroll
                    for (int j = 0; j < TNP; ++j) bv[j] = *reinterpret_cast<const uint4*>(smem + (kt * C4 + nc + j * 32 + l31) * 64 + (((2 * g + kk) ^ swzb) << 4));
                    chain_mfma_parts<PARTS, TNP>(accP, bv, ap[2 * kt + g]);
                } else {
                    const uint4 u0 = *reinterpret_cast<const uint4*>(la + kt * 4096 + (g ? ca2 : ca0));
                    const uint4 u1 = *reinterpret_cast<const uint4*>(la + kt * 4096 + (g ? ca3 : ca1));
#pragma unroll
                    for (int j = 0; j < TNP; ++j) bv[j] = *reinterpret_cast<const uint4*>(w3 + (long)(nc + j * 32 + l31) * C + kt * 32 + g * 16 + 8 * kk);
                    chain_mfma_parts<PARTS, TNP>(accP, bv, chain_split<PARTS>(u0, u1));
                }
            }
        }
        if constexpr (SC) {
            for (int g = 0; g < (WLDS ? C / 16 : a.sc_Cin / 16); ++g) {
                uint4 u0 = make_uint4(0u, 0u, 0u, 0u), u1 = u0;
                if constexpr (WLDS) { u0 = xr[2 * g]; u1 = xr[2 * g + 1]; }
                else if (sc_ok) { u0 = *reinterpret_cast<const uint4*>(sc_row + g * 16); u1 = *reinterpret_cast<const uint4*>(sc_row + g * 16 + 4); }
                uint4 bv[TNP];
#pragma unroll
                for (int j = 0; j < TNP; ++j) {
                    if constexpr (WLDS) bv[j] = *reinterpret_cast<const uint4*>(smem + 2 * W_BYTES + ((g >> 1) * C4 + nc + j * 32 + l31) * 64 + (((2 * (g & 1) + kk) ^ swzb) << 4));
                    else bv[j] = *reinterpret_cast<const uint4*>(wsc + (long)(nc + j * 32 + l31) * a.sc_Cin + g * 16 + 8 * kk);
                }
                chain_mfma_parts<PARTS, TNP>(accS, bv, chain_split<PARTS>(u0, u1));
            }
        }
#pragma unroll
        for (int j = 0; j < TNP; ++j) {
            const int n = nc + j * 32 + c4;
            float4 rj[4];
            if constexpr (SC) {
                chain_stage_acc(stage, accS[j], l31, kk);
                __builtin_amdgcn_wave_barrier();
                const float4 sc2 = *reinterpret_cast<const float4*>(a.sc_scale + n), sh2 = *reinterpret_cast<const float4*>(a.sc_shift + n);
#pragma unroll
                for (int ps = 0; ps < 4; ++ps) {
                    float4 y = *reinterpret_cast<const float4*>(&stage[(8 * ps + rrow) * 32 + (((lane & 7) ^ rrow) << 2)]);
                    y.x = y.x * sc2.x + sh2.x; y.y = y.y * sc2.y + sh2.y; y.z = y.z * sc2.z + sh2.z; y.w = y.w * sc2.w + sh2.w;
                    out_of_range = out_of_range || !(fabsf(y.x) < 65504.0f) || !(fabsf(y.y) < 65504.0f) || !(fabsf(y.z) < 65504.0f) || !(fabsf(y.w) < 65504.0f);
                    rj[ps] = y;
                }
                __builtin_amdgcn_wave_barrier();
            } else {
#pragma unroll
                for (int ps = 0; ps < 4; ++ps) rj[ps] = rv[j][ps];
            }
            chain_stage_acc(stage, accP[j], l31, kk);
            __builtin_amdgcn_wave_barrier();
            const float4 sc = *reinterpret_cast<const float4*>(a.scale + n), sh = *reinterpret_cast<const float4*>(a.shift + n);
            float4 xs[4];
#pragma unroll
            for (int ps = 0; ps < 4; ++ps) {
                float4 x = *reinterpret_cast<const float4*>(&stage[(8 * ps + rrow) * 32 + (((lane & 7) ^ rrow) << 2)]);
                x.x = x.x * sc.x + sh.x; x.y = x.y * sc.y + sh.y; x.z = x.z * sc.z + sh.z; x.w = x.w * sc.w + sh.w;
                if (SC || res) { x.x += rj[ps].x; x.y += rj[ps].y; x.z += rj[ps].z; x.w += rj[ps].w; }
                if (relu) { x.x = fmaxf(x.x, 0.f); x.y = fmaxf(x.y, 0.f); x.z = fmaxf(x.z, 0.f); x.w = fmaxf(x.w, 0.f); }
                if (ok[ps]) {
                    out_of_range = out_of_range || !(fabsf(x.x) < 65504.0f) || !(fabsf(x.y) < 65504.0f) || !(fabsf(x.z) < 65504.0f) || !(fabsf(x.w) < 65504.0f);
                    *reinterpret_cast<float4*>(out + mrow[ps] * C4 + n) = x;
                }
                xs[ps] = x;
            }
            __builtin_amdgcn_wave_barrier();
#pragma unroll
            for (int ps = 0; ps < 4; ++ps) *reinterpret_cast<float4*>(&stage[(8 * ps + rrow) * 32 + (((lane & 7) ^ rrow) << 2)]) = xs[ps];
            __builtin_amdgcn_wave_barrier();
#pragma unroll
            for (int g = 0; g < 2; ++g) {
                const uint4 u0 = *reinterpret_cast<const uint4*>(&stage[l31 * 32 + (((4 * g + 2 * kk) ^ (l31 & 7)) << 2)]);
                const uint4 u1 = *reinterpret_cast<const uint4*>(&stage[l31 * 32 + (((4 * g + 2 * kk + 1) ^ (l31 & 7)) << 2)]);
                uint4 bq[TNQ];
#pragma unroll
                for (int jq = 0; jq < TNQ; ++jq) {
                    if constexpr (WLDS) bq[jq] = *reinterpret_cast<const uint4*>(smem + W_BYTES + ((nc / 32 + j) * C + jq * 32 + l31) * 64 + (((2 * g + kk) ^ swzb) << 4));
                    else bq[jq] = *reinterpret_cast<const uint4*>(w1 + (long)(jq * 32 + l31) * C4 + nc + j * 32 + g * 16 + 8 * kk);
                }
                chain_mfma_parts<PARTS, TNQ>(accQ, bq, chain_split<PARTS>(u0, u1));
            }
            __builtin_amdgcn_wave_barrier();
        }
    }
#pragma unroll
    for (int jq = 0; jq < TNQ; ++jq) {
        const int n = jq * 32 + c4;
        chain_stage_acc(stage, accQ[jq], l31, kk);
        __builtin_amdgcn_wave_barrier();
        const float4 sc = *reinterpret_cast<const float4*>(aq.scale + n), sh = *reinterpret_cast<const float4*>(aq.shift + n);
#pragma unroll
        for (int ps = 0; ps < 4; ++ps) {
            float4 x = *reinterpret_cast<const float4*>(&stage[(8 * ps + rrow) * 32 + (((lane & 7) ^ rrow) << 2)]);
            x.x = x.x * sc.x + sh.x; x.y = x.y * sc.y + sh.y; x.z = x.z * sc.z + sh.z; x.w = x.w * sc.w + sh.w;
            if (reluq) { x.x = fmaxf(x.x, 0.f); x.y = fmaxf(x.y, 0.f); x.z = fmaxf(x.z, 0.f); x.w = fmaxf(x.w, 0.f); }
            if (ok[ps]) {
                out_of_range_q = out_of_range_q || !(fabsf(x.x) < 65504.0f) || !(fabsf(x.y) < 65504.0f) || !(fabsf(x.z) < 65504.0f) || !(fabsf(x.w) < 65504.0f);
                *reinterpret_cast<float4*>(outq + mrow[ps] * C + n) = x;
            }
        }
        __builtin_amdgcn_wave_barrier();
    }
    }
    if (a.range_flag && out_of_range) atomicOr(a.range_flag, 1);
    if (aq.range_flag && out_of_range_q) atomicOr(aq.range_flag, 1);
}

void conv_chain_launch(hipStream_t s, const ConvArgs& p, const ConvArgs& q, int parts, bool wlds, int n_cus)
{
    ChainArgs ca{p, q};
    dim3 grid((p.M + 127) / 128), block(256);
    const bool sc = p.sc_in != nullptr;
    const int C = q.Cout;
    MRCNN_REQUIRE((C == 64 || C == 128) && (parts == 2 || parts == 3), MRCNN_ERR_INVALID, "conv_chain_launch: C %d, %d parts", C, parts);
    if (wlds) {
        MRCNN_REQUIRE(C == 64 && (!sc || p.sc_Cin == 64) && n_cus > 0, MRCNN_ERR_INVALID, "conv_chain_launch: the LDS-resident form holds C = 64's filters");
        const int tiles256 = (p.M + 255) / 256;
        grid = dim3(tiles256 < n_cus ? tiles256 : n_cus); block = dim3(512);
#define MRCNN_CHAIN_W(P_, S_) hipLaunchKernelGGL((k_conv_chain<64, P_, S_, true>), grid, block, 0, s, ca)
        if (parts == 3) { if (sc) MRCNN_CHAIN_W(3, true); else MRCNN_CHAIN_W(3, false); }
        else { if (sc) MRCNN_CHAIN_W(2, true); else MRCNN_CHAIN_W(2, false); }
#undef MRCNN_CHAIN_W
        return;
    }
    MRCNN_REQUIRE(C == 128, MRCNN_ERR_INVALID, "conv_chain_launch: C = 64 runs the LDS-resident form");
#define MRCNN_CHAIN(C_, P_, S_) hipLaunchKernelGGL((k_conv_chain<C_, P_, S_, false>), grid, block, 0, s, ca)
    if (parts == 3) { if (sc) MRCNN_CHAIN(128, 3, true); else MRCNN_CHAIN(128, 3, false); }
    else { if (sc) MRCNN_CHAIN(128, 2, true); else MRCNN_CHAIN(128, 2, false); }
#undef MRCNN_CHAIN
}

}
```

mask-rcnn-coreml_amd/csrc/kernels_conv_halo.hip:

```cpp
#include "conv_device.h"
#include "knobs.h"

#include <stdlib.h>
#include <map>
#include <mutex>
#include <string>
#include <utility>

namespace mrcnn {

ConvScratch* conv_current_scratch();

static constexpr int HALO_MAX_SLOT = 640;
static constexpr unsigned HALO_OOB = 0xC0000000u;
enum { HALO_GEO_LINEAR = 0,
       HALO_GEO_ROW = 1,
       HALO_GEO_2ROWS = 2,
       HALO_GEO_4ROWS = 3 };

typedef unsigned u32x4 __attribute__((ext_vector_type(4)));
typedef unsigned u32x2 __attribute__((ext_vector_type(2)));

struct HaloArgs {
    ConvArgs a;
    const void* wgt_halo;
    int NH;
    int geo;
    int ecols;
    int pitch;
    int img_skew;
    int tiles_row, tiles_img;
    int n_tiles;
    const void* head_w;
    const float* head_bias;
    float* head_out; float* head_out2;
    long head_out_sB, head_out_sP, head_out2_sB, head_out2_sP;
    int head_split, head_cols;
    float head_mul;
    ConvArgs t;
    const void* t_w;
    void* t_park;
};

template <int PARTS>
__device__ __forceinline__ void split4(const u32x4 v, u32x2 (&out)[PARTS])
{
    const float a[4] = {__uint_as_float(v[0]), __uint_as_float(v[1]), __uint_as_float(v[2]), __uint_as_float(v[3])};
#pragma unroll
    for (int p = 0; p < 2; ++p) {
        const uint32_t h2 = cvt_pk_rne(a[2 * p], a[2 * p + 1]);
        float r0, r1;
        asm("v_fma_mix_f32 %0, %1, -1.0, %2 op_sel:[0,0,0] op_sel_hi:[1,0,0]" : "=v"(r0) : "v"(h2), "v"(a[2 * p]));
        asm("v_fma_mix_f32 %0, %1, -1.0, %2 op_sel:[1,0,0] op_sel_hi:[1,0,0]" : "=v"(r1) : "v"(h2), "v"(a[2 * p + 1]));
        const uint32_t m2 = cvt_pk_rne(r0, r1);
        out[0][p] = h2;
        out[1][p] = m2;
        if constexpr (PARTS == 3) {
            float q0, q1;
            asm("v_fma_mix_f32 %0, %1, -1.0, %2 op_sel:[0,0,0] op_sel_hi:[1,0,0]" : "=v"(q0) : "v"(m2), "v"(r0));
            asm("v_fma_mix_f32 %0, %1, -1.0, %2 op_sel:[1,0,0] op_sel_hi:[1,0,0]" : "=v"(q1) : "v"(m2), "v"(r1));
            out[2][p] = cvt_pk_rne(q0, q1);
        }
    }
}

template <int PARTS, int TN, bool HEAD = false, bool DBG = false, int TM = 2, int MAXPC = 5, bool TAIL = false, int WN = 4>
__global__ __launch_bounds__(512, 2) void k_conv_halo(const HaloArgs ha)
{
    const ConvArgs& a = ha.a;
    static_assert(WN == 4 || (WN == 2 && TM == 1 && TN == 1 && !HEAD && !TAIL) || (WN == 1 && TM == 1 && TN == 2 && !HEAD && !TAIL),
                  "wave arrangement 2 x 4; 4 x 2 with one accumulator per wave; 8 x 1 with two (256 x 64 tiles)");
    static_assert(!HEAD || TN == 2, "the fused head walks the K groups of 256-column tiles");
    static_assert(!TAIL || (TM == 2 && TN == 2 && !HEAD), "the fused tail needs the whole 128 x 256 tile in one block");
    static_assert(MAXPC >= 2 && MAXPC <= 5, "staging pieces per thread");
    constexpr int WMR = 8 / WN;
    constexpr int BM = WMR * TM * 32, BN = WN * TN * 32;
    constexpr int PLANE = (HALO_MAX_SLOT + 1) * 32;
    constexpr int PBUF = PARTS * PLANE;
    constexpr int STAGE = 8 * 32 * 36 * 4;
    constexpr int HPART = 4 * BM * 32 * 4;
    constexpr int HRUN = HEAD ? BM * 32 * 4 : 0;
    constexpr int PLANES_ = 2 * PBUF > PBUF + STAGE ? 2 * PBUF : PBUF + STAGE;
    constexpr int TAILPL = 16 * 64 * 32;
    constexpr int TAILN = 1024;
    constexpr int TPLANES = TAIL ? PARTS * TAILPL + STAGE : 0;
    constexpr int PLANES__ = HEAD && HPART > PLANES_ ? HPART : PLANES_;
    constexpr int PLANES = TPLANES > PLANES__ ? TPLANES : PLANES__;
    constexpr int TAB1 = TAIL ? 2 * TAILN * 4 : 0;
    __shared__ __attribute__((aligned(16))) unsigned char smem[PLANES + 2 * 2 * BN * 4 + HRUN + TAB1];
    unsigned char* const planes = smem;
    float* const s_tab0 = reinterpret_cast<float*>(smem + PLANES);
    float* const h_run = reinterpret_cast<float*>(smem + PLANES + 2 * 2 * BN * 4);
    float* const tab1 = reinterpret_cast<float*>(smem + PLANES + 2 * 2 * BN * 4 + HRUN);

    const int t = threadIdx.x;
    const int lane = t & 63;
    const int wave = __builtin_amdgcn_readfirstlane(t >> 6);
    const int wm = WN == 4 ? wave >> 2 : (WN == 2 ? wave >> 1 : wave), wn = WN == 4 ? wave & 3 : (WN == 2 ? wave & 1 : 0);
    const int l31 = lane & 31, kk = lane >> 5;
    const int ohw = a.OH * a.OW;
    const int NH = ha.NH, NS = NH * 9;

    const int T = HEAD ? a.tiles_m : ha.n_tiles;
    const int n_inner = HEAD ? a.tiles_n : 1;
    const int nb = gridDim.x;
    const int bid = blockIdx.x;
    int t_first, t_end, t_step;
    {
        const int q = T >> 3, r8 = T & 7;
        const int xcd = bid & 7, j = bid >> 3;
        const int lo = xcd < r8 ? xcd * (q + 1) : r8 * (q + 1) + (xcd - r8) * q;
        const int cnt = q + (xcd < r8 ? 1 : 0);
        const int per = nb >> 3;
        t_first = lo + j; t_end = lo + cnt; t_step = per;
        if (nb < 8) { t_first = bid; t_end = T; t_step = nb; }
    }

    typedef unsigned srd_t __attribute__((ext_vector_type(4)));
    srd_t srdB;
    {
        const unsigned long long wa = (unsigned long long)(uintptr_t)ha.wgt_halo;
        srdB[0] = __builtin_amdgcn_readfirstlane((unsigned)wa);
        srdB[1] = __builtin_amdgcn_readfirstlane((unsigned)(wa >> 32) & 0xffffu);
        srdB[2] = 0xffffffffu;
        srdB[3] = 0x00020000u;
    }
    const unsigned vlane16 = (unsigned)lane * 16u;
    srd_t srdT;
    {
        const unsigned long long ta_ = (unsigned long long)(uintptr_t)(TAIL ? ha.t_w : ha.wgt_halo);
        srdT[0] = __builtin_amdgcn_readfirstlane((unsigned)ta_);
        srdT[1] = __builtin_amdgcn_readfirstlane((unsigned)(ta_ >> 32) & 0xffffu);
        srdT[2] = 0xffffffffu;
        srdT[3] = 0x00020000u;
    }
    if constexpr (TAIL) {
        const float4 one = make_float4(1.f, 1.f, 1.f, 1.f), zero = make_float4(0.f, 0.f, 0.f, 0.f);
        if (t < TAILN / 4) {
            *reinterpret_cast<float4*>(&tab1[4 * t]) = ha.t.scale ? *reinterpret_cast<const float4*>(ha.t.scale + 4 * t) : one;
            *reinterpret_cast<float4*>(&tab1[TAILN + 4 * t]) = ha.t.shift ? *reinterpret_cast<const float4*>(ha.t.shift + 4 * t) : zero;
        }
    }
    const int dbg = DBG ? a.dbg : 0;
    const bool dbg_nodma = dbg & 1, dbg_nobar = dbg & 2, dbg_nords = dbg & 4, dbg_nomma = dbg & 8, dbg_nostage = dbg & 16;
    const bool dbg_noloads = dbg & 64, dbg_nosplit = dbg & 128, dbg_nowrite = dbg & 256;

    int tile_par = 0;
    for (int unit = t_first; unit < t_end; unit += t_step)
    for (int inner = 0; inner < n_inner; ++inner, tile_par ^= 1) {
        const int mt = HEAD ? unit : unit / a.tiles_n, nt = HEAD ? inner : unit - mt * a.tiles_n;
        const int n0 = nt * BN;
        float* const s_tab = s_tab0 + tile_par * 2 * BN;
        const int Hp = a.H + 2;
        const int pitch = ha.pitch, ecols = ha.ecols;
        int m0, b0, gy_first, col0, rows;
        if (ha.geo == HALO_GEO_2ROWS || ha.geo == HALO_GEO_4ROWS) {
            const int trows = ha.geo == HALO_GEO_2ROWS ? 2 : 4;
            b0 = mt / ha.tiles_img;
            const int r = mt - b0 * ha.tiles_img, rp = r / ha.tiles_row, cb = r - rp * ha.tiles_row;
            m0 = b0 * ohw + trows * rp * a.OW + 64 * cb;
            gy_first = b0 * Hp + trows * rp + 1;
            col0 = 64 * cb - 1;
            rows = trows + 2;
        } else {
            m0 = mt * BM;
            const int m_last = (m0 + BM - 1 < a.M ? m0 + BM - 1 : a.M - 1);
            b0 = m0 / ohw;
            const int rem0 = m0 - b0 * ohw, oh0 = rem0 / a.OW, ow0 = rem0 - oh0 * a.OW;
            const int b1 = m_last / ohw, rem1 = m_last - b1 * ohw, oh1 = rem1 / a.OW;
            gy_first = b0 * Hp + oh0 + 1;
            const int gy_last = b1 * Hp + oh1 + 1;
            col0 = ha.geo == HALO_GEO_ROW ? ow0 - 1 : -1;
            rows = gy_last - gy_first + 3;
        }
        const int npx = rows * ecols;
        srd_t srdA;
        {
            const unsigned long long ia = (unsigned long long)(uintptr_t)(static_cast<const float*>(a.in) + (long)b0 * a.in_sB);
            const unsigned long long rest = (unsigned long long)(a.B - b0) * (unsigned long long)a.in_sB * 4ull;
            srdA[0] = __builtin_amdgcn_readfirstlane((unsigned)ia);
            srdA[1] = __builtin_amdgcn_readfirstlane((unsigned)(ia >> 32) & 0xffffu);
            srdA[2] = __builtin_amdgcn_readfirstlane((unsigned)(rest < 0x80000000ull ? rest : 0x80000000ull));
            srdA[3] = 0x00020000u;
        }
        unsigned p_off[MAXPC], p_lds[MAXPC];
#pragma unroll
        for (int i = 0; i < MAXPC; ++i) {
            const int j = t + 512 * i;
            const int px = j >> 2, qt = j & 3;
            const int r = px / ecols, c = px - r * ecols;
            const int gy = gy_first - 1 + r;
            const int b = gy / Hp, y = gy - b * Hp - 1;
            const int x = col0 + c;
            const bool ok = px < npx && (unsigned)y < (unsigned)a.H && (unsigned)x < (unsigned)a.W && b < a.B;
            p_off[i] = ok ? (unsigned)(((long)(b - b0) * a.in_sB + (long)y * a.in_sH + (long)x * a.in_sW + qt * 4) * 4) : HALO_OOB;
            if (DBG && (a.dbg & 32)) p_off[i] = (unsigned)((px & 63) * 1024 + qt * 16);
            const int slot = r * pitch + c + (b - b0) * ha.img_skew;
            p_lds[i] = px < npx ? (unsigned)(slot * 32 + (((qt >> 1) ^ ((slot >> 3) & 1)) << 4) + (qt & 1) * 8) : (unsigned)(HALO_MAX_SLOT * 32 + qt * 8);
        }
        int base_idx[TM];
        int wave_row0;
        if (ha.geo == HALO_GEO_2ROWS || ha.geo == HALO_GEO_4ROWS) {
            if constexpr (WN == 4) {
                wave_row0 = m0 + wm * a.OW;
#pragma unroll
                for (int i = 0; i < TM; ++i) base_idx[i] = wm * pitch + i * 32 + l31;
            } else {
                wave_row0 = m0 + (wm >> 1) * a.OW + (wm & 1) * 32;
                base_idx[0] = (wm >> 1) * pitch + (wm & 1) * 32 + l31;
            }
        } else {
            wave_row0 = m0 + wm * (TM * 32);
            const int ow0 = col0 + 1;
#pragma unroll
            for (int i = 0; i < TM; ++i) {
                const int m = wave_row0 + i * 32 + l31;
                const int mm = m < a.M ? m : a.M - 1;
                const int b = mm / ohw, rem = mm - b * ohw, oh = rem / a.OW, ow = rem - oh * a.OW;
                base_idx[i] = ha.geo == HALO_GEO_ROW ? (ow - ow0) : (b * Hp + oh + 1 - gy_first) * pitch + ow + (b - b0) * ha.img_skew;
            }
        }
        unsigned sob[TN];
#pragma unroll
        for (int j = 0; j < TN; ++j) sob[j] = (unsigned)(((size_t)(n0 / 32 + wn * TN + j) * NS) * 1024u);

        if (t < BN / 2) {
            const int c = (t < BN / 4 ? t : t - BN / 4) * 4;
            const float* src = t < BN / 4 ? a.scale : a.shift;
            const float fill = t < BN / 4 ? 1.0f : 0.0f;
            *reinterpret_cast<float4*>(&s_tab[(t < BN / 4 ? 0 : BN) + c]) =
                src ? *reinterpret_cast<const float4*>(src + n0 + c) : make_float4(fill, fill, fill, fill);
        }

#define HALO_LOAD(I) if constexpr ((I) < MAXPC) asm volatile("buffer_load_dwordx4 %0, %1, %2, 0 offen" : "=v"(st[(I) < MAXPC ? (I) : 0]) : "v"(p_off[(I) < MAXPC ? (I) : 0]), "s"(srdA) : "memory");
#define HALO_LOADS()  { HALO_LOAD(0) HALO_LOAD(1) HALO_LOAD(2) HALO_LOAD(3) HALO_LOAD(4) }
#define HALO_ADVANCE() { _Pragma("unroll") for (int i = 0; i < MAXPC; ++i) p_off[i] += (p_off[i] < HALO_OOB ? 64u : 0u); }
#define HALO_PIN1(I)  if constexpr ((I) < MAXPC) asm volatile("" : "+v"(st[(I) < MAXPC ? (I) : 0]));
#define HALO_PIN()    { HALO_PIN1(0) HALO_PIN1(1) HALO_PIN1(2) HALO_PIN1(3) HALO_PIN1(4) }
#define HALO_WRITE1(BUF, I_)                                                                                     \
    if constexpr ((I_) < MAXPC) {                                                                                \
        constexpr int I = (I_) < MAXPC ? (I_) : 0;                                                               \
        u32x2 parts[PARTS];                                                                                      \
        if (DBG && dbg_nosplit) { _Pragma("unroll") for (int p = 0; p < PARTS; ++p) { parts[p][0] = st[I][0]; parts[p][1] = st[I][p]; } } \
        else split4<PARTS>(st[I], parts);                                                                        \
        if (DBG && dbg_nowrite) { _Pragma("unroll") for (int p = 0; p < PARTS; ++p) asm volatile("" ::"v"(parts[p])); } \
        else {                                                                                                   \
            _Pragma("unroll") for (int p = 0; p < PARTS; ++p)                                                    \
                *reinterpret_cast<u32x2*>(planes + (BUF) * PBUF + p * PLANE + p_lds[I]) = parts[p];              \
        }                                                                                                        \
    }
#define HALO_WRITE(BUF) { HALO_WRITE1(BUF, 0) HALO_WRITE1(BUF, 1) HALO_WRITE1(BUF, 2) HALO_WRITE1(BUF, 3) HALO_WRITE1(BUF, 4) }
#define HALO_BLOAD(BV, STEP_)                                                                                    \
    {                                                                                                            \
        _Pragma("unroll") for (int j = 0; j < TN; ++j) {                                                         \
            const unsigned so_ = sob[j] + (unsigned)(STEP_) * 1024u;                                             \
            asm volatile("buffer_load_dwordx4 %0, %1, %2, %3 offen" : "=v"(BV[j]) : "v"(vlane16), "s"(srdB), "s"(so_) : "memory"); \
        }                                                                                                        \
    }
#define HALO_BPIN(BV) { _Pragma("unroll") for (int j = 0; j < TN; ++j) asm volatile("" : "+v"(BV[j])); }
        u32x4 st[MAXPC];
        u32x4 bv0[TN], bv1[TN], bv2[TN], bv3[TN];

        HALO_LOADS()
        HALO_ADVANCE()
        HALO_BLOAD(bv0, 0)
        HALO_BLOAD(bv1, 1)
        HALO_BLOAD(bv2, 2)
        asm volatile("s_waitcnt vmcnt(0)" ::: "memory");
        HALO_PIN()
        HALO_BPIN(bv0)
        HALO_BPIN(bv1)
        HALO_BPIN(bv2)
        HALO_WRITE(0)
        __syncthreads();

        f32x16 acc[TM][TN];
#pragma unroll
        for (int i = 0; i < TM; ++i)
#pragma unroll
            for (int j = 0; j < TN; ++j)
#pragma unroll
                for (int e = 0; e < 16; ++e) acc[i][j][e] = 0.0f;

#define HALO_AFRAGS(AV, PB_, TAP_)                                                                               \
    {                                                                                                            \
        _Pragma("unroll") for (int i = 0; i < TM; ++i) {                                                         \
            const int idx_ = base_idx[i] + ((TAP_) / 3) * pitch + ((TAP_) % 3);                                  \
            const unsigned a_addr_ = (unsigned)(idx_ << 5) + (unsigned)(((kk << 4) ^ ((idx_ << 1) & 16)));       \
            _Pragma("unroll") for (int p = 0; p < PARTS; ++p) AV[i][p] = *reinterpret_cast<const uint4*>(planes + (PB_) * PBUF + p * PLANE + a_addr_); \
        }                                                                                                        \
    }
#define HALO_STEP(BVC, BVN3, TAP, PB)                                                                            \
    {                                                                                                            \
          \
        if (!(DBG && dbg_nodma)) HALO_BLOAD(BVN3, step + 3 < NS ? step + 3 : NS - 1)                             \
        if ((TAP) == 0 && next_slab && !(DBG && dbg_noloads)) { HALO_LOADS() HALO_ADVANCE() }                    \
        if (!(DBG && dbg_nomma)) {                                                                               \
        _Pragma("unroll") for (int p = 0; p < PARTS; ++p)                                                        \
            _Pragma("unroll") for (int i = 0; i < TM; ++i)                                                       \
                _Pragma("unroll") for (int j = 0; j < TN; ++j)                                                   \
                    acc[i][j] = __builtin_amdgcn_mfma_f32_32x32x16_f16(__builtin_bit_cast(f16x8, BVC[j]), __builtin_bit_cast(f16x8, av[i][p]), acc[i][j], 0, 0, 0); \
        }                                                                                                        \
                                 \
        if (!(DBG && dbg_nords)) {                                                                               \
            if ((TAP) == 8) HALO_AFRAGS(av, (PB) ^ 1, 0)                                                         \
            else HALO_AFRAGS(av, PB, ((TAP) + 1) % 9)                                                            \
        }                                                                                                        \
            \
        if ((TAP) == 4 && next_slab) { HALO_PIN() HALO_WRITE1((PB) ^ 1, 0) HALO_WRITE1((PB) ^ 1, 4) }            \
        if ((TAP) == 5 && next_slab) HALO_WRITE1((PB) ^ 1, 1)                                                    \
        if ((TAP) == 6 && next_slab) HALO_WRITE1((PB) ^ 1, 2)                                                    \
        if ((TAP) == 7 && next_slab) HALO_WRITE1((PB) ^ 1, 3)                                                    \
        if (DBG && (dbg_nodma || dbg_noloads)) asm volatile("s_waitcnt vmcnt(0)" ::: "memory");                  \
        else if ((TAP) <= 2 && next_slab) asm volatile("s_waitcnt vmcnt(%0)" ::"n"(2 * TN + MAXPC) : "memory");  \
        else asm volatile("s_waitcnt vmcnt(%0)" ::"n"(2 * TN) : "memory");                                       \
        HALO_BPIN(bv0) HALO_BPIN(bv1) HALO_BPIN(bv2) HALO_BPIN(bv3)                                              \
        if ((TAP) == 7 && !(DBG && dbg_nobar)) __syncthreads();                                                  \
        ++step;                                                                                                  \
    }
#define HALO_SLAB(B0, B1, B2, B3, PB)                                                                            \
    HALO_STEP(B0, B3, 0, PB) HALO_STEP(B1, B0, 1, PB) HALO_STEP(B2, B1, 2, PB) HALO_STEP(B3, B2, 3, PB) HALO_STEP(B0, B3, 4, PB) \
    HALO_STEP(B1, B0, 5, PB) HALO_STEP(B2, B1, 6, PB) HALO_STEP(B3, B2, 7, PB) HALO_STEP(B0, B3, 8, PB)
        uint4 av[TM][PARTS];
        HALO_AFRAGS(av, 0, 0)
        int step = 0;
        for (int h = 0; h < NH; h += 4) {
            { const bool next_slab = !dbg_nostage;                 HALO_SLAB(bv0, bv1, bv2, bv3, 0) }
            { const bool next_slab = !dbg_nostage;                 HALO_SLAB(bv1, bv2, bv3, bv0, 1) }
            { const bool next_slab = !dbg_nostage;                 HALO_SLAB(bv2, bv3, bv0, bv1, 0) }
            { const bool next_slab = h + 4 < NH && !dbg_nostage;   HALO_SLAB(bv3, bv0, bv1, bv2, 1) }
        }
        asm volatile("s_waitcnt vmcnt(0)" ::: "memory");
        HALO_BPIN(bv0) HALO_BPIN(bv1) HALO_BPIN(bv2) HALO_BPIN(bv3)
#undef HALO_SLAB
#undef HALO_STEP
#undef HALO_AFRAGS
#undef HALO_BPIN
#undef HALO_BLOAD
#undef HALO_WRITE
#undef HALO_WRITE1
#undef HALO_PIN
#undef HALO_PIN1
#undef HALO_ADVANCE
#undef HALO_LOADS
#undef HALO_LOAD
        if constexpr (TAIL) {
            const ConvArgs& t1 = ha.t;
            unsigned char* const tpl = smem;
            float* const tstage = reinterpret_cast<float*>(smem + PARTS * TAILPL) + wave * (32 * 36);
            const bool relu3 = a.act == ACT_RELU;
            bool oor = false;
            if (t1.dbg & 4) { if (acc[0][0][0] == 123.456f) tab1[1] = acc[1][1][3]; continue; }
            float4* const park = static_cast<float4*>(ha.t_park) + ((size_t)blockIdx.x * 4 + wn) * 16 * 64 + lane;
            auto stage_piece = [&](const float (&x)[4], int i, int j, int q) {
                u32x4 v = {__float_as_uint(x[0]), __float_as_uint(x[1]), __float_as_uint(x[2]), __float_as_uint(x[3])};
                u32x2 parts[PARTS];
                split4<PARTS>(v, parts);
                const int row = i * 32 + l31, g = wn * 4 + j * 2 + (q >> 1);
                const unsigned addr = (unsigned)((g * 64 + row) * 32 + ((((q & 1) ^ (row >> 3)) & 1) << 4) + 8 * kk);
#pragma unroll
                for (int p = 0; p < PARTS; ++p) *reinterpret_cast<u32x2*>(tpl + p * TAILPL + addr) = parts[p];
            };
            __syncthreads();
            if (!(t1.dbg & 8))
#pragma unroll
            for (int i = 0; i < TM; ++i)
#pragma unroll
                for (int j = 0; j < TN; ++j)
#pragma unroll
                    for (int q = 0; q < 4; ++q) {
                        const int cl = wn * 64 + j * 32 + 8 * q + 4 * kk;
                        const float4 sc = *reinterpret_cast<const float4*>(s_tab + cl), sh = *reinterpret_cast<const float4*>(s_tab + BN + cl);
                        float x[4] = {acc[i][j][4 * q + 0] * sc.x + sh.x, acc[i][j][4 * q + 1] * sc.y + sh.y,
                                      acc[i][j][4 * q + 2] * sc.z + sh.z, acc[i][j][4 * q + 3] * sc.w + sh.w};
#pragma unroll
                        for (int r = 0; r < 4; ++r) {
                            if (relu3) x[r] = fmaxf(x[r], 0.f);
                            oor = oor || !(fabsf(x[r]) < 65504.0f);
                        }
                        if (wm == 0) stage_piece(x, i, j, q);
                        else park[((i * 2 + j) * 4 + q) * 64] = make_float4(x[0], x[1], x[2], x[3]);
                    }
            if (a.range_flag && oor) atomicOr(a.range_flag, 1);
#pragma unroll 1
            for (int h = 0; h < 2; ++h) {
                if (h == 1 && wm == 1 && !(t1.dbg & 8)) {
#pragma unroll
                    for (int i = 0; i < TM; ++i)
#pragma unroll
                        for (int j = 0; j < TN; ++j)
#pragma unroll
                            for (int q = 0; q < 4; ++q) {
                                const float4 y = park[((i * 2 + j) * 4 + q) * 64];
                                const float x[4] = {y.x, y.y, y.z, y.w};
                                stage_piece(x, i, j, q);
                            }
                }
                __syncthreads();
                const int half_row0 = ha.geo == HALO_GEO_2ROWS ? m0 + h * a.OW : m0 + h * 64;
#pragma unroll 1
                for (int it = 0; it < 2; ++it) {
                    const int n1 = it * 512 + wave * 64;
                    f32x16 acc1[2][2];
#pragma unroll
                    for (int i = 0; i < 2; ++i)
#pragma unroll
                        for (int j = 0; j < 2; ++j)
#pragma unroll
                            for (int e = 0; e < 16; ++e) acc1[i][j][e] = 0.0f;
                    const unsigned wofs = (unsigned)((n1 / 32) * 16 * 1024);
                    u32x4 bw[3][2];
#define TAIL_BLOAD(SET, S_)                                                                                      \
    {                                                                                                            \
        _Pragma("unroll") for (int j = 0; j < 2; ++j) {                                                          \
            const unsigned so_ = wofs + (unsigned)((j * 16 + (S_)) * 1024);                                      \
            asm volatile("buffer_load_dwordx4 %0, %1, %2, %3 offen" : "=v"(bw[SET][j]) : "v"(vlane16), "s"(srdT), "s"(so_) : "memory"); \
        }                                                                                                        \
    }
#define TAIL_BPIN() { _Pragma("unroll") for (int q_ = 0; q_ < 3; ++q_) _Pragma("unroll") for (int j = 0; j < 2; ++j) asm volatile("" : "+v"(bw[q_][j])); }
                    TAIL_BLOAD(0, 0)
                    TAIL_BLOAD(1, 1)
                    const unsigned a_off = (unsigned)(l31 * 32 + ((kk ^ ((l31 >> 3) & 1)) << 4));
                    uint4 fa[2][PARTS];
#pragma unroll
                    for (int i = 0; i < 2; ++i)
#pragma unroll
                        for (int p = 0; p < PARTS; ++p) fa[i][p] = *reinterpret_cast<const uint4*>(tpl + p * TAILPL + (i * 32) * 32 + a_off);
                    asm volatile("s_waitcnt vmcnt(2)" ::: "memory");
                    TAIL_BPIN()
#pragma unroll
                    for (int s = 0; s < 16; ++s) {
                        if (t1.dbg & 2) { asm volatile("s_waitcnt vmcnt(0)" ::: "memory"); break; }
                        if (s + 2 < 16) TAIL_BLOAD((s + 2) % 3, s + 2)
#pragma unroll
                        for (int i = 0; i < 2; ++i)
#pragma unroll
                            for (int p = 0; p < PARTS; ++p)
#pragma unroll
                                for (int j = 0; j < 2; ++j)
                                    acc1[i][j] = __builtin_amdgcn_mfma_f32_32x32x16_f16(__builtin_bit_cast(f16x8, bw[s % 3][j]), __builtin_bit_cast(f16x8, fa[i][p]),
                                                                                        acc1[i][j], 0, 0, 0);
                        if (s + 1 < 16) {
#pragma unroll
                            for (int i = 0; i < 2; ++i)
#pragma unroll
                                for (int p = 0; p < PARTS; ++p)
                                    fa[i][p] = *reinterpret_cast<const uint4*>(tpl + p * TAILPL + ((s + 1) * 64 + i * 32) * 32 + a_off);
                        }
                        if (s + 2 < 16) asm volatile("s_waitcnt vmcnt(2)" ::: "memory");
                        else asm volatile("s_waitcnt vmcnt(0)" ::: "memory");
                        TAIL_BPIN()
                    }
#undef TAIL_BPIN
#undef TAIL_BLOAD
                    if (!(t1.dbg & 1))
                        conv_epilogue_wave<TAILN, 2, 2, true>(t1, acc1, tstage, tab1, half_row0, 0, n1, lane);
                    else if (acc1[0][0][0] == 123.456f) tab1[0] = acc1[1][1][3];
                }
                __syncthreads();
            }
        } else if constexpr (!HEAD) {
            conv_epilogue_wave<BN, TM, TN>(a, acc, reinterpret_cast<float*>(planes + PBUF) + wave * (32 * 36), s_tab, wave_row0, n0,
                                           wn * TN * 32, lane);
        } else {
            const bool relu = a.act == ACT_RELU;
            bool out_of_range = false;
            f32x16 hp[TM];
#pragma unroll
            for (int i = 0; i < TM; ++i)
#pragma unroll
                for (int e = 0; e < 16; ++e) hp[i][e] = 0.0f;
            const unsigned hw_off = (unsigned)(((n0 + wn * TN * 32) / 16) * 1024);
#pragma unroll
            for (int j = 0; j < TN; ++j)
#pragma unroll
                for (int g = 0; g < 2; ++g) {
                    const uint4 wf = *reinterpret_cast<const uint4*>(static_cast<const char*>(ha.head_w) + hw_off + (j * 2 + g) * 1024 + lane * 16);
#pragma unroll
                    for (int i = 0; i < TM; ++i) {
                        u32x4 v0, v1;
#pragma unroll
                        for (int q2 = 0; q2 < 2; ++q2) {
                            const int cl = wn * TN * 32 + j * 32 + 8 * (2 * g + q2) + 4 * kk;
                            const float4 sc = *reinterpret_cast<const float4*>(s_tab + cl), sh = *reinterpret_cast<const float4*>(s_tab + BN + cl);
                            float x[4] = {acc[i][j][8 * g + 4 * q2 + 0] * sc.x + sh.x, acc[i][j][8 * g + 4 * q2 + 1] * sc.y + sh.y,
                                          acc[i][j][8 * g + 4 * q2 + 2] * sc.z + sh.z, acc[i][j][8 * g + 4 * q2 + 3] * sc.w + sh.w};
#pragma unroll
                            for (int r = 0; r < 4; ++r) {
                                if (relu) x[r] = fmaxf(x[r], 0.f);
                                out_of_range = out_of_range || !(fabsf(x[r]) < 65504.0f);
                                if (q2 == 0) v0[r] = __float_as_uint(x[r]); else v1[r] = __float_as_uint(x[r]);
                            }
                        }
                        u32x2 p0[PARTS], p1[PARTS];
                        split4<PARTS>(v0, p0);
                        split4<PARTS>(v1, p1);
#pragma unroll
                        for (int p = 0; p < PARTS; ++p) {
                            const u32x4 af = {p0[p][0], p0[p][1], p1[p][0], p1[p][1]};
                            hp[i] = __builtin_amdgcn_mfma_f32_32x32x16_f16(__builtin_bit_cast(f16x8, wf), __builtin_bit_cast(f16x8, af), hp[i], 0, 0, 0);
                        }
                    }
                }
            if (a.range_flag && out_of_range) atomicOr(a.range_flag, 1);
            float* const part = reinterpret_cast<float*>(planes);
#pragma unroll
            for (int i = 0; i < TM; ++i)
#pragma unroll
                for (int q = 0; q < 4; ++q)
                    *reinterpret_cast<float4*>(&part[((wn * BM) + wm * (TM * 32) + i * 32 + l31) * 32 + (((2 * q + kk) ^ (l31 & 7)) << 2)]) =
                        make_float4(hp[i][4 * q], hp[i][4 * q + 1], hp[i][4 * q + 2], hp[i][4 * q + 3]);
            __syncthreads();
            const bool last = inner == n_inner - 1;
#pragma unroll
            for (int k = 0; k < BM / 16; ++k) {
                const int o = t + 512 * k, row = o >> 5, col = o & 31;
                float sum = inner == 0 ? 0.0f : h_run[o];
                const int pc = ((((col >> 2) ^ (row & 7)) << 2) | (col & 3));
                sum += part[(0 * BM + row) * 32 + pc];
                sum += part[(1 * BM + row) * 32 + pc];
                sum += part[(2 * BM + row) * 32 + pc];
                sum += part[(3 * BM + row) * 32 + pc];
                if (!last) h_run[o] = sum;
                else {
                    const int m = ha.geo == HALO_GEO_2ROWS ? m0 + (row >> 6) * a.OW + (row & 63) : m0 + row;
                    if (m < a.M && col < ha.head_cols) {
                        const float y = sum * ha.head_mul + ha.head_bias[col];
                        const int b = m / ohw, pix = m - b * ohw;
                        if (col < ha.head_split) ha.head_out[(long)b * ha.head_out_sB + (long)pix * ha.head_out_sP + col] = y;
                        else ha.head_out2[(long)b * ha.head_out2_sB + (long)pix * ha.head_out2_sP + (col - ha.head_split)] = y;
                    }
                }
            }
            __syncthreads();
        }
    }
}

static constexpr int HALO_LAT_MAX_SLOT = 320;
template <int PARTS, int MAXPC>
__global__ __launch_bounds__(256, 2) void k_conv_halo_lat(const HaloArgs ha)
{
    const ConvArgs& a = ha.a;
    static_assert(MAXPC >= 3 && MAXPC <= 5, "staging pieces per thread");
    constexpr int BM = 64, BN = 64, NT = 256, D = 11, NSET = 12;
    constexpr int PLANE = (HALO_LAT_MAX_SLOT + 1) * 32;
    constexpr int PBUF = PARTS * PLANE;
    static_assert(PBUF >= 4 * 32 * 32 * 4, "the four wave-private epilogue tiles live in plane buffer 1");
    __shared__ __attribute__((aligned(16))) unsigned char smem[2 * PBUF + 2 * 2 * BN * 4];
    unsigned char* const planes = smem;
    float* const s_tab0 = reinterpret_cast<float*>(smem + 2 * PBUF);

    const int t = threadIdx.x;
    const int lane = t & 63;
    const int wave = __builtin_amdgcn_readfirstlane(t >> 6);
    const int wm = wave >> 1, wn = wave & 1;
    const int l31 = lane & 31, kk = lane >> 5;
    const int ohw = a.OH * a.OW;
    const int NH = ha.NH, NS = NH * 9;

    const int T = ha.n_tiles;
    const int nb = gridDim.x;
    const int bid = blockIdx.x;
    int t_first, t_end, t_step;
    {
        const int q = T >> 3, r8 = T & 7;
        const int xcd = bid & 7, j = bid >> 3;
        const int lo = xcd < r8 ? xcd * (q + 1) : r8 * (q + 1) + (xcd - r8) * q;
        const int cnt = q + (xcd < r8 ? 1 : 0);
        const int per = nb >> 3;
        t_first = lo + j; t_end = lo + cnt; t_step = per;
        if (nb < 8) { t_first = bid; t_end = T; t_step = nb; }
    }
    typedef unsigned srd_t __attribute__((ext_vector_type(4)));
    srd_t srdB;
    {
        const unsigned long long wa = (unsigned long long)(uintptr_t)ha.wgt_halo;
        srdB[0] = __builtin_amdgcn_readfirstlane((unsigned)wa);
        srdB[1] = __builtin_amdgcn_readfirstlane((unsigned)(wa >> 32) & 0xffffu);
        srdB[2] = 0xffffffffu;
        srdB[3] = 0x00020000u;
    }
    const unsigned vlane16 = (unsigned)lane * 16u;

    int tile_par = 0;
    for (int unit = t_first; unit < t_end; unit += t_step, tile_par ^= 1) {
        const int mt = unit / a.tiles_n, nt = unit - mt * a.tiles_n;
        const int n0 = nt * BN;
        float* const s_tab = s_tab0 + tile_par * 2 * BN;
        const int Hp = a.H + 2;
        const int pitch = ha.pitch, ecols = ha.ecols;
        const int m0 = mt * BM;
        const int m_last = (m0 + BM - 1 < a.M ? m0 + BM - 1 : a.M - 1);
        const int b0 = m0 / ohw;
        const int rem0 = m0 - b0 * ohw, oh0 = rem0 / a.OW, ow0 = rem0 - oh0 * a.OW;
        const int b1 = m_last / ohw, rem1 = m_last - b1 * ohw, oh1 = rem1 / a.OW;
        const int gy_first = b0 * Hp + oh0 + 1;
        const int gy_last = b1 * Hp + oh1 + 1;
        const int col0 = ha.geo == HALO_GEO_ROW ? ow0 - 1 : -1;
        const int rows = gy_last - gy_first + 3;
        const int npx = rows * ecols;
        srd_t srdA;
        {
            const unsigned long long ia = (unsigned long long)(uintptr_t)(static_cast<const float*>(a.in) + (long)b0 * a.in_sB);
            const unsigned long long rest = (unsigned long long)(a.B - b0) * (unsigned long long)a.in_sB * 4ull;
            srdA[0] = __builtin_amdgcn_readfirstlane((unsigned)ia);
            srdA[1] = __builtin_amdgcn_readfirstlane((unsigned)(ia >> 32) & 0xffffu);
            srdA[2] = __builtin_amdgcn_readfirstlane((unsigned)(rest < 0x80000000ull ? rest : 0x80000000ull));
            srdA[3] = 0x00020000u;
        }
        unsigned p_off[MAXPC], p_lds[MAXPC];
#pragma unroll
        for (int i = 0; i < MAXPC; ++i) {
            const int j = t + NT * i;
            const int px = j >> 2, qt = j & 3;
            const int r = px / ecols, c = px - r * ecols;
            const int gy = gy_first - 1 + r;
            const int b = gy / Hp, y = gy - b * Hp - 1;
            const int x = col0 + c;
            const bool ok = px < npx && (unsigned)y < (unsigned)a.H && (unsigned)x < (unsigned)a.W && b < a.B;
            p_off[i] = ok ? (unsigned)(((long)(b - b0) * a.in_sB + (long)y * a.in_sH + (long)x * a.in_sW + qt * 4) * 4) : HALO_OOB;
            const int slot = r * pitch + c + (b - b0) * ha.img_skew;
            p_lds[i] = px < npx ? (unsigned)(slot * 32 + (((qt >> 1) ^ ((slot >> 3) & 1)) << 4) + (qt & 1) * 8) : (unsigned)(HALO_LAT_MAX_SLOT * 32 + qt * 8);
        }
        const int wave_row0 = m0 + wm * 32;
        int base_idx;
        {
            const int m = wave_row0 + l31;
            const int mm = m < a.M ? m : a.M - 1;
            const int b = mm / ohw, rem = mm - b * ohw, oh = rem / a.OW, ow = rem - oh * a.OW;
            base_idx = ha.geo == HALO_GEO_ROW ? (ow - ow0) : (b * Hp + oh + 1 - gy_first) * pitch + ow + (b - b0) * ha.img_skew;
        }
        const unsigned sob = (unsigned)(((size_t)(n0 / 32 + wn) * NS) * 1024u);
        if (t < BN / 2) {
            const int c = (t < BN / 4 ? t : t - BN / 4) * 4;
            const float* src = t < BN / 4 ? a.scale : a.shift;
            const float fill = t < BN / 4 ? 1.0f : 0.0f;
            *reinterpret_cast<float4*>(&s_tab[(t < BN / 4 ? 0 : BN) + c]) =
                src ? *reinterpret_cast<const float4*>(src + n0 + c) : make_float4(fill, fill, fill, fill);
        }

#define LAT_LOAD(S, I) if constexpr ((I) < MAXPC) asm volatile("buffer_load_dwordx4 %0, %1, %2, 0 offen" : "=v"(st[S][(I) < MAXPC ? (I) : 0]) : "v"(p_off[(I) < MAXPC ? (I) : 0]), "s"(srdA) : "memory");
#define LAT_LOADS(S) { LAT_LOAD(S, 0) LAT_LOAD(S, 1) LAT_LOAD(S, 2) LAT_LOAD(S, 3) LAT_LOAD(S, 4) }
#define LAT_ADVANCE() { _Pragma("unroll") for (int i = 0; i < MAXPC; ++i) p_off[i] += (p_off[i] < HALO_OOB ? 64u : 0u); }
#define LAT_PIN1(S, I) if constexpr ((I) < MAXPC) asm volatile("" : "+v"(st[S][(I) < MAXPC ? (I) : 0]));
#define LAT_PIN(S) { LAT_PIN1(S, 0) LAT_PIN1(S, 1) LAT_PIN1(S, 2) LAT_PIN1(S, 3) LAT_PIN1(S, 4) }
#define LAT_WRITE1(S, BUF, I_)                                                                                   \
    if constexpr ((I_) < MAXPC) {                                                                                \
        constexpr int I = (I_) < MAXPC ? (I_) : 0;                                                               \
        u32x2 parts[PARTS];                                                                                      \
        split4<PARTS>(st[S][I], parts);                                                                          \
        _Pragma("unroll") for (int p = 0; p < PARTS; ++p)                                                        \
            *reinterpret_cast<u32x2*>(planes + (BUF) * PBUF + p * PLANE + p_lds[I]) = parts[p];                  \
    }
#define LAT_BLOAD(SET, SO_) asm volatile("buffer_load_dwordx4 %0, %1, %2, %3 offen" : "=v"(bv[SET]) : "v"(vlane16), "s"(srdB), "s"(SO_) : "memory");
#define LAT_BPIN() { _Pragma("unroll") for (int q_ = 0; q_ < NSET; ++q_) asm volatile("" : "+v"(bv[q_])); }
#define LAT_BARRIER() asm volatile("s_waitcnt lgkmcnt(0)\n\ts_barrier" ::: "memory")
#define LAT_AFRAGS(AV, PB_, TAP_)                                                                                \
    {                                                                                                            \
        const int idx_ = base_idx + ((TAP_) / 3) * pitch + ((TAP_) % 3);                                         \
        const unsigned a_addr_ = (unsigned)(idx_ << 5) + (unsigned)(((kk << 4) ^ ((idx_ << 1) & 16)));           \
        _Pragma("unroll") for (int p = 0; p < PARTS; ++p) AV[p] = *reinterpret_cast<const uint4*>(planes + (PB_) * PBUF + p * PLANE + a_addr_); \
    }
#ifdef MRCNN_CONV_ABLATE
#define LAT_ABL(BIT) (!(a.dbg & (BIT)))
#else
#define LAT_ABL(BIT) true
#endif
        u32x4 st[2][MAXPC];
        u32x4 bv[NSET];
        LAT_LOADS(0)
        LAT_ADVANCE()
        const bool two = NH > 1;
        if (two) { LAT_LOADS(1) LAT_ADVANCE() }
        const unsigned so_last = sob + (unsigned)(NS - 1) * 1024u;
        unsigned so_next = sob;
#pragma unroll
        for (int q_ = 0; q_ < D; ++q_) {
            if (q_) so_next = so_next + 1024u < so_last ? so_next + 1024u : so_last;
            LAT_BLOAD(q_, so_next)
        }
        if (two) asm volatile("s_waitcnt vmcnt(%0)" ::"n"(D + MAXPC) : "memory");
        else asm volatile("s_waitcnt vmcnt(%0)" ::"n"(D) : "memory");
        LAT_PIN(0)
        LAT_WRITE1(0, 0, 0) LAT_WRITE1(0, 0, 1) LAT_WRITE1(0, 0, 2) LAT_WRITE1(0, 0, 3) LAT_WRITE1(0, 0, 4)
        LAT_BARRIER();

        f32x16 acc;
#pragma unroll
        for (int e = 0; e < 16; ++e) acc[e] = 0.0f;
        uint4 av[2][PARTS];
        LAT_AFRAGS(av[0], 0, 0)
        asm volatile("s_waitcnt vmcnt(%0)" ::"n"(D - 1) : "memory");
        LAT_BPIN()
#define LAT_PIECE(TAP) ((TAP) >= 4 && (TAP) <= 7 ? (TAP) - 4 : ((TAP) == 3 ? 4 : 99))
#define LAT_MFMA(K, P) acc = __builtin_amdgcn_mfma_f32_32x32x16_f16(__builtin_bit_cast(f16x8, bv[(K) % NSET]), __builtin_bit_cast(f16x8, av[(K) & 1][P]), acc, 0, 0, 0);
#define LAT_STEP(K, TAP, PB, HP)                                                                                 \
    {                                                                                                            \
        constexpr int PI = LAT_PIECE(TAP) < MAXPC ? LAT_PIECE(TAP) : 0;                                          \
        constexpr bool HASP = LAT_PIECE(TAP) < MAXPC;                                                            \
        if (LAT_ABL(1)) { so_next = so_next + 1024u < so_last ? so_next + 1024u : so_last; LAT_BLOAD(((K) + D) % NSET, so_next) } \
        if ((TAP) == 0 && stage_now) { LAT_LOADS(HP) LAT_ADVANCE() }                                             \
        if (LAT_ABL(4)) {                                                                                        \
            if ((TAP) == 8) LAT_AFRAGS(av[((K) + 1) & 1], (PB) ^ 1, 0)                                           \
            else LAT_AFRAGS(av[((K) + 1) & 1], PB, ((TAP) + 1) % 9)                                              \
        }                                                                                                        \
        if (LAT_ABL(2)) { _Pragma("unroll") for (int p = 0; p < PARTS; ++p) LAT_MFMA(K, p) }                     \
        if (HASP && write_next && LAT_ABL(8)) { LAT_PIN1((HP) ^ 1, PI) LAT_WRITE1((HP) ^ 1, (PB) ^ 1, PI) }      \
        if (stage_now) {                                                                                         \
            if ((TAP) <= 1 && stage_prev) asm volatile("s_waitcnt vmcnt(%0)" ::"n"(D - 1 + 2 * MAXPC) : "memory"); \
            else asm volatile("s_waitcnt vmcnt(%0)" ::"n"(D - 1 + MAXPC) : "memory");                            \
        } else {                                                                                                 \
            if ((TAP) <= 1 && stage_prev) asm volatile("s_waitcnt vmcnt(%0)" ::"n"(D - 1 + MAXPC) : "memory");   \
            else asm volatile("s_waitcnt vmcnt(%0)" ::"n"(D - 1) : "memory");                                    \
        }                                                                                                        \
        LAT_BPIN()                                                                                               \
        if ((TAP) == 7) LAT_BARRIER();                                                                           \
    }
#define LAT_SLAB(K0, PB, HP)                                                                                     \
    LAT_STEP((K0) + 0, 0, PB, HP) LAT_STEP((K0) + 1, 1, PB, HP) LAT_STEP((K0) + 2, 2, PB, HP) LAT_STEP((K0) + 3, 3, PB, HP) LAT_STEP((K0) + 4, 4, PB, HP) \
    LAT_STEP((K0) + 5, 5, PB, HP) LAT_STEP((K0) + 6, 6, PB, HP) LAT_STEP((K0) + 7, 7, PB, HP) LAT_STEP((K0) + 8, 8, PB, HP)
        for (int h = 0; h < NH; h += 4) {
            if (!LAT_ABL(32)) break;
            { const bool stage_now = h + 2 < NH && LAT_ABL(8), write_next = h + 1 < NH && LAT_ABL(8), stage_prev = h >= 1 && h + 1 < NH && LAT_ABL(8); LAT_SLAB(0, 0, 0) }
            { const bool stage_now = h + 3 < NH && LAT_ABL(8), write_next = h + 2 < NH && LAT_ABL(8), stage_prev = h + 2 < NH && LAT_ABL(8);           LAT_SLAB(9, 1, 1) }
            { const bool stage_now = h + 4 < NH && LAT_ABL(8), write_next = h + 3 < NH && LAT_ABL(8), stage_prev = h + 3 < NH && LAT_ABL(8);           LAT_SLAB(18, 0, 0) }
            { const bool stage_now = h + 5 < NH && LAT_ABL(8), write_next = h + 4 < NH && LAT_ABL(8), stage_prev = h + 4 < NH && LAT_ABL(8);           LAT_SLAB(27, 1, 1) }
        }
        asm volatile("s_waitcnt vmcnt(0)" ::: "memory");
        LAT_BPIN()
#undef LAT_SLAB
#undef LAT_STEP
#undef LAT_MFMA
#undef LAT_PIECE
#undef LAT_AFRAGS
#undef LAT_BARRIER
#undef LAT_BPIN
#undef LAT_BLOAD
#undef LAT_WRITE1
#undef LAT_PIN
#undef LAT_PIN1
#undef LAT_ADVANCE
#undef LAT_LOADS
#undef LAT_LOAD
        f32x16 accs[1][1];
        accs[0][0] = acc;
        if (!LAT_ABL(16)) { if (acc[0] == 123.456f) s_tab[0] = acc[3]; continue; }
        conv_epilogue_wave<BN, 1, 1>(a, accs, reinterpret_cast<float*>(planes + PBUF) + wave * (32 * 32), s_tab, wave_row0, n0, wn * 32, lane);
#undef LAT_ABL
    }
}

__global__ __launch_bounds__(256) void k_halo_pack(const uint4* __restrict__ src, int Npad, int Cin, int taps, uint4* __restrict__ dst)
{
    const int NH = Cin / 16;
    const long total = (long)(Npad / 32) * NH * taps * 64;
    for (long e = (long)blockIdx.x * 256 + threadIdx.x; e < total; e += (long)gridDim.x * 256) {
        const int piece = (int)(e & 63);
        const long gs = e >> 6;
        const int step = (int)(gs % (NH * taps));
        const int g = (int)(gs / (NH * taps));
        const int h = step / taps, tap = step - h * taps;
        const int r = piece & 31, half = piece >> 5;
        const int n = g * 32 + r;
        dst[e] = src[(((long)n * taps + tap) * Cin + 16 * h + 8 * half) / 8];
    }
}

__global__ __launch_bounds__(256) void k_halo_pack_head(const uint16_t* __restrict__ src, int Cin, uint16_t* __restrict__ dst)
{
    const long total = (long)(Cin / 16) * 64 * 8;
    for (long e = (long)blockIdx.x * 256 + threadIdx.x; e < total; e += (long)gridDim.x * 256) {
        const int sl = (int)(e & 7), lane = (int)((e >> 3) & 63);
        const int G = (int)(e >> 9);
        const int n = lane & 31, kk = lane >> 5;
        dst[e] = src[(long)n * Cin + 16 * G + 4 * kk + (sl & 3) + 8 * (sl >> 2)];
    }
}

void conv_halo_pack_head(hipStream_t s, const void* wgt_std, int Npad, int Cin, DevBuf& out)
{
    MRCNN_REQUIRE(Npad == 32 && Cin % 16 == 0, MRCNN_ERR_SHAPE, "halo head packing: Npad %d (must be 32) / Cin %d", Npad, Cin);
    out.alloc((size_t)32 * Cin * 2);
    hipLaunchKernelGGL(k_halo_pack_head, dim3(64), dim3(256), 0, s, static_cast<const uint16_t*>(wgt_std), Cin, static_cast<uint16_t*>(out.p));
    HIP_CHECK(hipGetLastError());
}

void conv_halo_pack(hipStream_t s, const void* wgt_std, int Npad, int Cin, DevBuf& out, int taps)
{
    MRCNN_REQUIRE(Npad % 32 == 0 && Cin % 16 == 0 && (taps == 9 || taps == 1), MRCNN_ERR_SHAPE, "halo packing: Npad %d / Cin %d / taps %d", Npad, Cin, taps);
    const size_t bytes = (size_t)Npad * taps * Cin * 2;
    out.alloc(bytes);
    const long total = (long)bytes / 16;
    const int grid = (int)((total + 255) / 256 < 4096 ? (total + 255) / 256 : 4096);
    hipLaunchKernelGGL(k_halo_pack, dim3(grid), dim3(256), 0, s, static_cast<const uint4*>(wgt_std), Npad, Cin, taps, static_cast<uint4*>(out.p));
    HIP_CHECK(hipGetLastError());
}

static int halo_linear_rows(int H, int W, int bm)
{
    const int rows_touched = (bm - 1 + W - 1) / W + 1;
    const long ohw = (long)H * W;
    const int boundaries = ohw % bm == 0 ? 0 : (int)((bm - 1 + ohw - 1) / ohw);
    return rows_touched + 2 * boundaries + 2;
}

static int& g_halo_lat = knob("halo_lat", "MRCNN_HALO_LAT", 1);
static int& g_halo_rounds = knob("halo_rounds", "MRCNN_HALO_ROUNDS", 1);
static int& g_halo_n64 = knob("halo_n64", "MRCNN_HALO_N64", 2);
static int& g_halo_geo = knob("halo_geo", "MRCNN_HALO_GEO", 1);

struct HaloGeo { int geo, ecols, pitch, img_skew, tiles_row, tiles_img, rows, maxpc, slots; bool ok; };

static HaloGeo halo_geometry(int H, int W, int bm)
{
    HaloGeo g{};
    int slots_extra = 0;
    if (g_halo_geo == 0) {
        const bool row = W % 128 == 0;
        g.geo = row ? HALO_GEO_ROW : HALO_GEO_LINEAR;
        g.ecols = g.pitch = row ? 130 : W + 2;
        g.rows = row ? 3 : halo_linear_rows(H, W, bm);
        g.maxpc = 5;
        g.ok = g.rows * g.ecols <= 528;
        return g;
    }
    if (bm == 256) {
        if (W % 64 != 0 || H % 4 != 0) return g;
        g.geo = HALO_GEO_4ROWS; g.ecols = g.pitch = 66; g.rows = 6;
        g.tiles_row = W / 64; g.tiles_img = (H / 4) * g.tiles_row;
    } else if (bm == 128 && W % 64 == 0 && W >= 128 && H % 2 == 0) {
        g.geo = HALO_GEO_2ROWS; g.ecols = g.pitch = 66; g.rows = 4;
        g.tiles_row = W / 64; g.tiles_img = (H / 2) * g.tiles_row;
    } else if (W % bm == 0) {
        g.geo = HALO_GEO_ROW; g.ecols = g.pitch = bm + 2; g.rows = 3;
    } else {
        g.geo = HALO_GEO_LINEAR; g.ecols = W + 2; g.rows = halo_linear_rows(H, W, bm);
        g.pitch = W % 32 == 0 ? W + 2 : W + 16;
        const long ohw = (long)H * W;
        const int boundaries = ohw % bm == 0 ? 0 : (int)((bm - 1 + ohw - 1) / ohw);
        g.img_skew = g.pitch == W + 16 ? (16 - (2 * W) % 16) % 16 : 0;
        if (g.rows * g.pitch + boundaries * g.img_skew > HALO_MAX_SLOT) { g.pitch = W + 2; g.img_skew = 0; }
        slots_extra = boundaries * g.img_skew;
    }
    const int px = g.rows * g.ecols;
    g.maxpc = px <= 256 ? 2 : px <= 384 ? 3 : 5;
    g.slots = g.rows * g.pitch + slots_extra;
    g.ok = px <= 640 && g.slots <= HALO_MAX_SLOT;
    return g;
}

bool conv_halo_eligible(const ConvDesc& d)
{
    const int wdtype = d.wdtype < 0 ? d.dtype : d.wdtype;
    const bool split = d.dtype == MRCNN_F32 && (wdtype == MRCNN_F16 || wdtype == MRCNN_F32X3);
    if (!split || d.KH != 3 || d.KW != 3 || d.stride != 1 || d.padH != 1 || d.padW != 1) return false;
    if (d.OH != d.H || d.OW != d.W || d.Cin % 64 != 0 || (d.Npad % 128 != 0 && !(d.Npad == 64 && g_halo_n64)) || d.Cout % 4 != 0) return false;
    if (d.deconv2 || d.out2 || d.sel_partial || d.act == ACT_SIGMOID || d.res) return false;
    if (d.H >= 32760 || d.W >= 32760 || (double)d.in_sB * 8.0 >= 2.0e9) return false;
    const bool legacy_ok = (d.W % 128 == 0 ? 3 * 130 : halo_linear_rows(d.H, d.W, 128) * (d.W + 2)) <= 528;
    if (g_halo_geo == 0) return legacy_ok;
    const bool rows2_ok = d.W % 64 == 0 && d.H % 2 == 0;
    return (legacy_ok || rows2_ok) && halo_geometry(d.H, d.W, 128).ok && halo_geometry(d.H, d.W, 64).ok;
}

template <int PARTS, int TN, bool HEAD, int TM>
static void halo_launch_pc(hipStream_t s, const HaloArgs& ha, int maxpc, int grid)
{
    if (maxpc == 2) {
        if constexpr (!HEAD) hipLaunchKernelGGL((k_conv_halo<PARTS, TN, HEAD, false, TM, 2>), dim3(grid), dim3(512), 0, s, ha);
        else hipLaunchKernelGGL((k_conv_halo<PARTS, TN, HEAD, false, TM, 3>), dim3(grid), dim3(512), 0, s, ha);
    } else if (maxpc == 3) hipLaunchKernelGGL((k_conv_halo<PARTS, TN, HEAD, false, TM, 3>), dim3(grid), dim3(512), 0, s, ha);
    else hipLaunchKernelGGL((k_conv_halo<PARTS, TN, HEAD, false, TM, 5>), dim3(grid), dim3(512), 0, s, ha);
}

template <int PARTS>
static void halo_launch(hipStream_t s, const HaloArgs& ha, int bm, int bn, int maxpc, int grid)
{
    if (ha.a.dbg && !ha.head_w && bn == 256 && PARTS == 3) {
        if (maxpc <= 3) hipLaunchKernelGGL((k_conv_halo<3, 2, false, true, 2, 3>), dim3(grid), dim3(512), 0, s, ha);
        else hipLaunchKernelGGL((k_conv_halo<3, 2, false, true, 2, 5>), dim3(grid), dim3(512), 0, s, ha);
        return;
    }
    if (bn == 64 && bm == 256) {
        hipLaunchKernelGGL((k_conv_halo<PARTS, 2, false, false, 1, 5, false, 1>), dim3(grid), dim3(512), 0, s, ha);
        return;
    }
    if (bn == 64) {
        if (maxpc == 2) hipLaunchKernelGGL((k_conv_halo<PARTS, 1, false, false, 1, 2, false, 2>), dim3(grid), dim3(512), 0, s, ha);
        else if (maxpc == 3) hipLaunchKernelGGL((k_conv_halo<PARTS, 1, false, false, 1, 3, false, 2>), dim3(grid), dim3(512), 0, s, ha);
        else hipLaunchKernelGGL((k_conv_halo<PARTS, 1, false, false, 1, 5, false, 2>), dim3(grid), dim3(512), 0, s, ha);
        return;
    }
    if (ha.head_w && bm == 64) hipLaunchKernelGGL((k_conv_halo<PARTS, 2, true, false, 1, 3>), dim3(grid), dim3(512), 0, s, ha);
    else if (ha.head_w) halo_launch_pc<PARTS, 2, true, 2>(s, ha, maxpc, grid);
    else if (bn == 256) halo_launch_pc<PARTS, 2, false, 2>(s, ha, maxpc, grid);
    else if (bm == 128) halo_launch_pc<PARTS, 1, false, 2>(s, ha, maxpc, grid);
    else halo_launch_pc<PARTS, 1, false, 1>(s, ha, maxpc, grid);
}

bool conv_halo_packable(int KH, int KW, int Cin, int Npad) { return KH == 3 && KW == 3 && Cin % 64 == 0 && (Npad % 128 == 0 || Npad == 64); }

bool conv_halo_head_eligible(const ConvDesc& d)
{
    return conv_halo_eligible(d) && d.Npad % 256 == 0 && d.Npad == d.Cout && ((long)d.OH * d.OW) % 128 == 0 && (long)d.OH * d.OW >= 4096 &&
           d.head_cols >= 1 && d.head_cols <= 32 && d.head_split >= 0 && d.head_split <= d.head_cols;
}

bool conv_halo_tail_packable(int KH, int KW, int Cin, int Npad) { return KH == 1 && KW == 1 && Cin == 256 && Npad == 1024; }
bool conv_halo_tail_geometry_ok(int H, int W) { const HaloGeo g = halo_geometry(H, W, 128); return g.ok && g.maxpc <= 3; }

int conv_halo_forward(hipStream_t s, ConvArgs a, const ConvDesc& d, int parts, int n_cus, const ConvArgs* t1, const void* t_w)
{
    HaloArgs ha;
    ha.t_w = t_w;
    ha.t_park = nullptr;
    if (t1) ha.t = *t1;
    int bm = 128, bn = d.Npad % 256 == 0 ? 256 : (d.Npad % 128 == 0 ? 128 : 64);
    if (bn == 64 && g_halo_n64 >= 2 && g_halo_geo && halo_geometry(d.H, d.W, 256).ok && (long)(a.M / 256) >= (long)n_cus * 2) bm = 256;
    if (!d.head_w && !t1 && bn != 64) {
        if (bn > 128 && (long)((a.M + 127) / 128) * (d.Npad / bn) < n_cus) bn = 128;
        if (bn == 128 && (long)((a.M + 127) / 128) * (d.Npad / bn) * 4 < (long)n_cus * 3) bm = 64;
        if (bn == 128 && bm == 128 && g_halo_rounds) {
            const long t128 = (long)((a.M + 127) / 128) * (d.Npad / bn), t64 = (long)((a.M + 63) / 64) * (d.Npad / bn);
            const long r128 = (t128 + n_cus - 1) / n_cus, r64 = (t64 + n_cus - 1) / n_cus;
            if (r64 * 575 < r128 * 1000 && halo_geometry(d.H, d.W, 64).ok) bm = 64;
        }
    }
    if (d.head_w && (long)((a.M + 127) / 128) * 4 < (long)n_cus * 3 && d.W % 64 == 0) bm = 64;
    MRCNN_REQUIRE(!t1 || (bn == 256 && d.Npad == 256), MRCNN_ERR_INVALID, "fused tail: the 3x3 layer must have exactly 256 output columns");
    int lat_pc = 0;
    if (!d.head_w && !t1 && g_halo_lat && g_halo_geo && bm == 64 && bn == 128 && (long)((a.M + 63) / 64) * (d.Npad / 128) * 8 < (long)n_cus * 3 * g_halo_lat) {
        const HaloGeo g64 = halo_geometry(d.H, d.W, 64);
        const int px = g64.rows * g64.ecols;
        if (g64.ok && g64.geo != HALO_GEO_2ROWS && px <= 320 && g64.slots <= HALO_LAT_MAX_SLOT) { lat_pc = px <= 192 ? 3 : px <= 256 ? 4 : 5; bn = 64; }
    }
    const int tiles_m = (a.M + bm - 1) / bm;
    a.tiles_m = tiles_m;
    a.tiles_n = d.Npad / bn;
    a.direct = 1;
    ha.a = a;
    ha.wgt_halo = d.wgt_halo;
    ha.NH = d.Cin / 16;
    const HaloGeo g = halo_geometry(d.H, d.W, bm);
    MRCNN_REQUIRE(g.ok, MRCNN_ERR_SHAPE, "halo kernel: no tile geometry for %dx%d (conv_halo_eligible should have said so)", d.H, d.W);
    ha.geo = g.geo; ha.ecols = g.ecols; ha.pitch = g.pitch; ha.img_skew = g.img_skew; ha.tiles_row = g.tiles_row; ha.tiles_img = g.tiles_img;
    ha.n_tiles = a.tiles_m * a.tiles_n;
    ha.head_w = d.head_w; ha.head_bias = d.head_bias; ha.head_out = d.head_out; ha.head_out2 = d.head_out2;
    ha.head_out_sB = d.head_out_sB; ha.head_out_sP = d.head_out_sP; ha.head_out2_sB = d.head_out2_sB; ha.head_out2_sP = d.head_out2_sP;
    ha.head_split = d.head_split; ha.head_cols = d.head_cols; ha.head_mul = d.head_mul;
    const int units = d.head_w ? a.tiles_m : ha.n_tiles;
    int grid = units < n_cus ? units : n_cus;
    if (grid >= 8) grid &= ~7;
    if (t1) {
        ha.t.direct = 1;
        {
            ConvScratch* const sc = conv_current_scratch();
            MRCNN_REQUIRE(sc, MRCNN_ERR_INVALID, "fused tail without a ConvScratch (conv_forward_tail checks)");
            if (sc->park.bytes < (size_t)grid * 65536) {
                hipStreamCaptureStatus cap = hipStreamCaptureStatusNone;
                HIP_CHECK(hipStreamIsCapturing(s, &cap));
                MRCNN_REQUIRE(cap == hipStreamCaptureStatusNone, MRCNN_ERR_INVALID, "fused tail: the parking buffer must exist before a stream capture (run the predict once eagerly)");
                HIP_CHECK(hipStreamSynchronize(s));
                sc->park.alloc((size_t)grid * 65536);
            }
            ha.t_park = sc->park.p;
        }
        MRCNN_REQUIRE(g.maxpc <= 3, MRCNN_ERR_INVALID, "fused tail: the tile's input region needs more than three staging pieces (conv_halo_tail_geometry_ok)");
        if (parts == 3) hipLaunchKernelGGL((k_conv_halo<3, 2, false, false, 2, 3, true>), dim3(grid), dim3(512), 0, s, ha);
        else hipLaunchKernelGGL((k_conv_halo<2, 2, false, false, 2, 3, true>), dim3(grid), dim3(512), 0, s, ha);
        return bn;
    }
    if (lat_pc) {
        grid = units < 2 * n_cus ? units : 2 * n_cus;
        if (grid >= 8) grid &= ~7;
#define MRCNN_LAT(P, PC) hipLaunchKernelGGL((k_conv_halo_lat<P, PC>), dim3(grid), dim3(256), 0, s, ha)
        if (parts == 3) { if (lat_pc == 3) MRCNN_LAT(3, 3); else if (lat_pc == 4) MRCNN_LAT(3, 4); else MRCNN_LAT(3, 5); }
        else { if (lat_pc == 3) MRCNN_LAT(2, 3); else if (lat_pc == 4) MRCNN_LAT(2, 4); else MRCNN_LAT(2, 5); }
#undef MRCNN_LAT
        return bn;
    }
    if (parts == 3) halo_launch<3>(s, ha, bm, bn, g.maxpc, grid);
    else halo_launch<2>(s, ha, bm, bn, g.maxpc, grid);
    return bn;
}

}
```

Measured before the change: 440.4.

## Add streaming C=128 bottleneck chain kernel with fragment-ordered prepacked filters

Replaces the C=128 path of the fused 1x1-expand/1x1-reduce bottleneck chain with a new streaming kernel. It reads filters prepacked at load time into MFMA-fragment order (a new group-major pack option) and software-pipelines their global loads against the MFMA work. It also turns the chain on by default for C=128 stages when the tile count fills twice the CU count, both with and without a fused shortcut. The aim is to remove the strided per-lane global weight reads and the split per-conv launches for these stages. In exchange it adds extra packed weight buffers, 32-bit offset limits and a much more complex kernel.

```diff
diff --git a/mask-rcnn-coreml_amd/csrc/conv_dispatch.hip b/mask-rcnn-coreml_amd/csrc/conv_dispatch.hip
--- a/mask-rcnn-coreml_amd/csrc/conv_dispatch.hip
+++ b/mask-rcnn-coreml_amd/csrc/conv_dispatch.hip
@@ -5,7 +5,7 @@
 
 void conv_mfma_launch(hipStream_t s, const ConvArgs& a, int mode, int bn, bool wide_waves);
 void conv_pp_launch(hipStream_t s, const ConvArgs& a, int mode);
-void conv_chain_launch(hipStream_t s, const ConvArgs& p, const ConvArgs& q, int parts, bool wlds, int n_cus);
+void conv_chain_launch(hipStream_t s, const ConvArgs& p, const ConvArgs& q, int parts, bool wlds, int n_cus, const void* w3f, const void* w1f, const void* wscf);
 
 static inline int conv_wdtype(const ConvDesc& d) { return d.wdtype < 0 ? d.dtype : d.wdtype; }
 static inline bool conv_is_split(const ConvDesc& d) { return d.dtype == MRCNN_F32 && (conv_wdtype(d) == MRCNN_F16 || conv_wdtype(d) == MRCNN_F32X3); }
@@ -340,6 +340,14 @@
     return true;
 }
 
+bool conv_chain_packable(int KH, int KW, int Cin, int Npad, bool* group_major)
+{
+    if (KH != 1 || KW != 1) return false;
+    const bool w1 = Npad == 128 && Cin == 512, w3 = Npad == 512 && (Cin == 128 || Cin == 256);
+    if (group_major) *group_major = w1;
+    return w1 || w3;
+}
+
 bool conv_chain_fusable(const ConvDesc& dP, const ConvDesc& dQ, const ConvDesc* sc)
 {
     if (!conv_is_split(dP) || !conv_is_split(dQ) || conv_wdtype(dP) != conv_wdtype(dQ)) return false;
@@ -349,6 +357,7 @@
     if (!plain_epilogue(dP, ACT_RELU) || !plain_epilogue(dQ, ACT_RELU) || dQ.res) return false;
     if (!dense_in(dP, H, W, C) || !dense_out(dP, H, W, 4 * C) || dQ.in != dP.out || !dense_in(dQ, H, W, 4 * C) || !dense_out(dQ, H, W, C)) return false;
     if (conv_k_chunks(dP) != 1 || conv_k_chunks(dQ) != 1) return false;
+    if (C == 128 && (!dP.wgt_chain || !dQ.wgt_chain || (sc && (!sc->wgt_chain || sc->Cin != 256 || (long)sc->B * sc->in_sB * 4 >= (1L << 31))) || (long)dP.B * H * W * 2048 >= (1L << 31))) return false;
     auto al = [](const void* p) { return (reinterpret_cast<uintptr_t>(p) & 15) == 0; };
     if (!al(dP.in) || !al(dP.out) || !al(dQ.out) || !al(dP.wgt) || !al(dQ.wgt) || !al(dP.scale) || !al(dP.shift) || !al(dQ.scale) || !al(dQ.shift)) return false;
     if (sc) {
@@ -366,7 +375,9 @@
     const long tiles = ((long)dP.B * dP.OH * dP.OW + 127) / 128;
     const bool sc_rides = g_chain >= 3 ? sc != nullptr && conv_chain_fusable(dP, dQ, sc) : conv_shortcut_rides(dP, sc);
     const int n_cus = device_cu_count();
-    bool chain = g_chain && g_direct >= 2 && conv_chain_fusable(dP, dQ, sc_rides ? sc : nullptr) && (g_chain >= 2 || (dQ.Cout == 64 && fills_chip(tiles, n_cus)));
+    constexpr bool PAYS_C128_IDENTITY = true, PAYS_C128_ENTRY = true;
+    const bool pays = dQ.Cout == 64 ? fills_chip(tiles, n_cus) : fills_chip(tiles, 2 * n_cus) && (sc_rides ? PAYS_C128_ENTRY : PAYS_C128_IDENTITY);
+    bool chain = g_chain && g_direct >= 2 && conv_chain_fusable(dP, dQ, sc_rides ? sc : nullptr) && (g_chain >= 2 || pays);
 #ifndef MRCNN_CONV_ABLATE
     if (g_pp_dbg) chain = false;
 #endif
@@ -387,7 +398,7 @@
         aP.sc_H = sc->H; aP.sc_W = sc->W; aP.sc_Cin = sc->Cin; aP.sc_stride = sc->stride;
     }
     const ProfScope prof(s);
-    conv_chain_launch(s, aP, aQ, conv_split_parts(dP), dQ.Cout == 64, n_cus);
+    conv_chain_launch(s, aP, aQ, conv_split_parts(dP), dQ.Cout == 64, n_cus, dP.wgt_chain, dQ.wgt_chain, sc ? sc->wgt_chain : nullptr);
     if (prof) {
         const double fl = 2.0 * (double)aP.M * ((double)aP.ncols * (aP.Ktot + (sc ? sc->Cin : 0)) + (double)aQ.ncols * aQ.Ktot);
         prof.finish(sc ? TILE_128x128_4WAVE : TILE_128x128, fl, aP.M, aP.ncols, aP.Ktot, dP.group,
diff --git a/mask-rcnn-coreml_amd/csrc/engine.h b/mask-rcnn-coreml_amd/csrc/engine.h
--- a/mask-rcnn-coreml_amd/csrc/engine.h
+++ b/mask-rcnn-coreml_amd/csrc/engine.h
@@ -40,6 +40,7 @@
     DevBuf wgt, scale, shift;
     std::vector<float> h_scale, h_shift;
     DevBuf wgt_halo;
+    DevBuf wgt_chain;
     DevBuf wgt_c3h;
     DevBuf wgt_frag;
     int Cin = 0, Cout = 0, KH = 1, KW = 1, Npad = 0;
diff --git a/mask-rcnn-coreml_amd/csrc/engine_internal.h b/mask-rcnn-coreml_amd/csrc/engine_internal.h
--- a/mask-rcnn-coreml_amd/csrc/engine_internal.h
+++ b/mask-rcnn-coreml_amd/csrc/engine_internal.h
@@ -22,7 +22,7 @@
 }
 inline ConvView view_of(const Tensor4& t) { return dense_view(t.p, t.H, t.W, t.C); }
 
-enum : unsigned { RETILED_NONE = 0, RETILED_HALO = 1, RETILED_C3H = 2, RETILED_FRAG = 4, RETILED_ALL = 7 };
+enum : unsigned { RETILED_NONE = 0, RETILED_HALO = 1, RETILED_C3H = 2, RETILED_FRAG = 4, RETILED_CHAIN = 8, RETILED_ALL = 15 };
 
 inline ConvDesc make_conv_desc(const PackedConv& pc, const float* scale, const float* shift, const ConvView& in, const ConvView& out,
                                int stride, int pad, int act, unsigned retiled)
@@ -35,6 +35,7 @@
     if (retiled & RETILED_HALO) d.wgt_halo = pc.wgt_halo.p;
     if (retiled & RETILED_C3H) d.wgt_c3h = pc.wgt_c3h.p;
     if (retiled & RETILED_FRAG) d.wgt_frag = pc.wgt_frag.p;
+    if (retiled & RETILED_CHAIN) d.wgt_chain = pc.wgt_chain.p;
     d.scale = scale; d.shift = shift;
     d.act = act;
     d.out = out.p; d.OH = out.H; d.OW = out.W; d.Cout = pc.Cout; d.Npad = pc.Npad;
diff --git a/mask-rcnn-coreml_amd/csrc/engine_weights.hip b/mask-rcnn-coreml_amd/csrc/engine_weights.hip
--- a/mask-rcnn-coreml_amd/csrc/engine_weights.hip
+++ b/mask-rcnn-coreml_amd/csrc/engine_weights.hip
@@ -219,6 +219,11 @@
         conv_halo_pack(nullptr, pc.wgt.p, pc.Npad, I, pc.wgt_halo, 1);
         HIP_CHECK(hipStreamSynchronize(nullptr));
     }
+    bool group_major = false;
+    if (pc.wdtype != pc.dtype && O == pc.Npad && conv_chain_packable(KH, KW, I, pc.Npad, &group_major)) {
+        conv_halo_pack(nullptr, pc.wgt.p, pc.Npad, I, pc.wgt_chain, 1, group_major);
+        HIP_CHECK(hipStreamSynchronize(nullptr));
+    }
     if (pc.dtype == MRCNN_F16 && pc.wdtype == MRCNN_F16 && conv3x3h_packable(KH, KW, I, O, pc.Npad)) {
         conv3x3h_pack(nullptr, pc.wgt.p, O, I, pc.wgt_c3h);
         HIP_CHECK(hipStreamSynchronize(nullptr));
diff --git a/mask-rcnn-coreml_amd/csrc/kernels.h b/mask-rcnn-coreml_amd/csrc/kernels.h
--- a/mask-rcnn-coreml_amd/csrc/kernels.h
+++ b/mask-rcnn-coreml_amd/csrc/kernels.h
@@ -174,6 +174,7 @@
     long in_sB = 0, in_sH = 0, in_sW = 0;
     const void* wgt = nullptr;
     const void* wgt_halo = nullptr;
+    const void* wgt_chain = nullptr;
     const void* wgt_frag = nullptr;
     const void* wgt_c3h = nullptr;
     int prefer_c3h = 0;
@@ -244,7 +245,7 @@
 int conv_n_tile(int Cout);
 void conv_forward(hipStream_t s, const ConvDesc& d, const ConvDesc* sc = nullptr);
 struct ConvArgs;
-void conv_halo_pack(hipStream_t s, const void* wgt_std, int Npad, int Cin, DevBuf& out, int taps = 9);
+void conv_halo_pack(hipStream_t s, const void* wgt_std, int Npad, int Cin, DevBuf& out, int taps = 9, bool group_major = false);
 void conv_halo_pack_head(hipStream_t s, const void* wgt_std, int Npad, int Cin, DevBuf& out);
 bool conv_halo_eligible(const ConvDesc& d);
 bool conv_halo_head_eligible(const ConvDesc& d);
@@ -256,6 +257,7 @@
 bool conv_tail_fusable(const ConvDesc& d3, const ConvDesc& d1);
 int conv_sel_part_cols();
 void conv_forward_tail(hipStream_t s, const ConvDesc& d3, const ConvDesc& d1, const ConvDesc* sc = nullptr, const ConvDesc* q = nullptr);
+bool conv_chain_packable(int KH, int KW, int Cin, int Npad, bool* group_major);
 bool conv_chain_fusable(const ConvDesc& dP, const ConvDesc& dQ, const ConvDesc* sc = nullptr);
 void conv_forward_chain(hipStream_t s, const ConvDesc& dP, const ConvDesc& dQ, const ConvDesc* sc = nullptr);
 
diff --git a/mask-rcnn-coreml_amd/csrc/kernels_conv_chain.hip b/mask-rcnn-coreml_amd/csrc/kernels_conv_chain.hip
--- a/mask-rcnn-coreml_amd/csrc/kernels_conv_chain.hip
+++ b/mask-rcnn-coreml_amd/csrc/kernels_conv_chain.hip
@@ -2,7 +2,7 @@
 
 namespace mrcnn {
 
-struct ChainArgs { ConvArgs p, q; };
+struct ChainArgs { ConvArgs p, q; const void* w3f; const void* w1f; const void* wscf; };
 
 __device__ __forceinline__ void chain_stage_acc(float* stage, const f32x16& acc, int l31, int kk)
 {
@@ -30,22 +30,19 @@
         _Pragma("unroll") for (int j = 0; j < N; ++j) acc[j] = __builtin_amdgcn_mfma_f32_32x32x16_f16(__builtin_bit_cast(f16x8, bv[j]), lo2, acc[j], 0, 0, 0);
 }
 
-template <int C, int PARTS, bool SC, bool WLDS>
-__global__ __launch_bounds__(WLDS ? 512 : 256, WLDS ? 1 : 2) void k_conv_chain(const ChainArgs ca)
-{
-    static_assert(!WLDS || C == 64, "the LDS-resident form holds C = 64's filters");
-    constexpr int NW = WLDS ? 8 : 4, C4 = 4 * C, KT = C / 32, TNP = 2, TNQ = C / 32;
-    constexpr int A_BYTES = WLDS ? 0 : KT * 32 * 128;
-    constexpr int W_BYTES = WLDS ? C4 * C * 2 : 0;
+template <int PARTS, bool SC>
+__global__ __launch_bounds__(512, 1) void k_conv_chain(const ChainArgs ca)
+{
+    constexpr int C = 64, NW = 8, C4 = 4 * C, KT = C / 32, TNP = 2, TNQ = C / 32;
+    constexpr int W_BYTES = C4 * C * 2;
     constexpr int WF_BYTES = W_BYTES * (SC ? 3 : 2);
-    __shared__ __attribute__((aligned(16))) unsigned char smem[WF_BYTES + NW * (A_BYTES + 32 * 32 * 4)];
+    __shared__ __attribute__((aligned(16))) unsigned char smem[WF_BYTES + NW * (32 * 32 * 4)];
     const ConvArgs& a = ca.p;
     const ConvArgs& aq = ca.q;
     const int t = threadIdx.x;
     const int wave = t >> 6, lane = t & 63;
     const int l31 = lane & 31, kk = lane >> 5;
-    unsigned char* const As = smem + WF_BYTES + wave * A_BYTES;
-    float* const stage = reinterpret_cast<float*>(smem + WF_BYTES + NW * A_BYTES) + wave * (32 * 32);
+    float* const stage = reinterpret_cast<float*>(smem + WF_BYTES) + wave * (32 * 32);
     const float* const in = static_cast<const float*>(a.in);
     const _Float16* const w3 = static_cast<const _Float16*>(a.wgt);
     const _Float16* const w1 = static_cast<const _Float16*>(aq.wgt);
@@ -54,7 +51,7 @@
     float* const outq = static_cast<float*>(aq.out);
     const _Float16* const wsc = static_cast<const _Float16*>(a.sc_wgt);
     const int swzb = (l31 >> 2) & 3;
-    if constexpr (WLDS) {
+    {
         auto stage_filter = [&](unsigned char* dst, const _Float16* src, int rows, int K) {
             const int cpr = K / 8;
             for (int idx = t; idx < rows * cpr; idx += NW * 64) {
@@ -69,8 +66,8 @@
     }
     bool out_of_range = false, out_of_range_q = false;
     for (int row0 = (blockIdx.x * NW + wave) * 32; row0 < a.M; row0 += gridDim.x * NW * 32) {
-    ChainParts ap[WLDS ? 2 * KT : 1];
-    if constexpr (WLDS) {
+    ChainParts ap[2 * KT];
+    {
         const int m = row0 + l31;
 #pragma unroll
         for (int g = 0; g < 2 * KT; ++g) {
@@ -78,22 +75,8 @@
             if (m < a.M) { u0 = *reinterpret_cast<const uint4*>(in + (long)m * C + g * 16 + 8 * kk); u1 = *reinterpret_cast<const uint4*>(in + (long)m * C + g * 16 + 8 * kk + 4); }
             ap[g] = chain_split<PARTS>(u0, u1);
         }
-    } else {
-#pragma unroll
-        for (int it = 0; it < C / 8; ++it) {
-            const int idx = it * 64 + lane;
-            const int r = idx / (C / 4), ch = idx - r * (C / 4);
-            const int m = row0 + r;
-            uint4 v = make_uint4(0u, 0u, 0u, 0u);
-            if (m < a.M) v = *reinterpret_cast<const uint4*>(in + (long)m * C + ch * 4);
-            *reinterpret_cast<uint4*>(As + (ch >> 3) * 4096 + r * 128 + (((ch & 7) ^ ((r >> 1) & 7)) << 4)) = v;
-        }
-        __builtin_amdgcn_wave_barrier();
-    }
-
-    const int swz = (l31 >> 1) & 7;
-    const unsigned char* const la = As + l31 * 128;
-    const int ca0 = ((0 + 2 * kk) ^ swz) << 4, ca1 = ((1 + 2 * kk) ^ swz) << 4, ca2 = ((4 + 2 * kk) ^ swz) << 4, ca3 = ((5 + 2 * kk) ^ swz) << 4;
+    }
+
     const int rrow = lane >> 3, c4 = (lane & 7) * 4;
     const bool relu = a.act == ACT_RELU, reluq = aq.act == ACT_RELU;
     bool ok[4];
@@ -112,8 +95,8 @@
         const int oh = rem / a.OW, ow = rem - oh * a.OW;
         sc_row = static_cast<const float*>(a.sc_in) + (long)b * a.sc_in_sB + (long)(oh * a.sc_stride) * a.sc_in_sH + (long)(ow * a.sc_stride) * a.sc_in_sW + 8 * kk;
     }
-    uint4 xr[SC && WLDS ? C / 4 : 1];
-    if constexpr (SC && WLDS) {
+    uint4 xr[SC ? C / 4 : 1];
+    if constexpr (SC) {
 #pragma unroll
         for (int i = 0; i < C / 4; ++i) {
             xr[i] = make_uint4(0u, 0u, 0u, 0u);
@@ -148,30 +131,17 @@
 #pragma unroll
             for (int g = 0; g < 2; ++g) {
                 uint4 bv[TNP];
-                if constexpr (WLDS) {
-#pragma unroll
-                    for (int j = 0; j < TNP; ++j) bv[j] = *reinterpret_cast<const uint4*>(smem + (kt * C4 + nc + j * 32 + l31) * 64 + (((2 * g + kk) ^ swzb) << 4));
-                    chain_mfma_parts<PARTS, TNP>(accP, bv, ap[2 * kt + g]);
-                } else {
-                    const uint4 u0 = *reinterpret_cast<const uint4*>(la + kt * 4096 + (g ? ca2 : ca0));
-                    const uint4 u1 = *reinterpret_cast<const uint4*>(la + kt * 4096 + (g ? ca3 : ca1));
-#pragma unroll
-                    for (int j = 0; j < TNP; ++j) bv[j] = *reinterpret_cast<const uint4*>(w3 + (long)(nc + j * 32 + l31) * C + kt * 32 + g * 16 + 8 * kk);
-                    chain_mfma_parts<PARTS, TNP>(accP, bv, chain_split<PARTS>(u0, u1));
-                }
+#pragma unroll
+                for (int j = 0; j < TNP; ++j) bv[j] = *reinterpret_cast<const uint4*>(smem + (kt * C4 + nc + j * 32 + l31) * 64 + (((2 * g + kk) ^ swzb) << 4));
+                chain_mfma_parts<PARTS, TNP>(accP, bv, ap[2 * kt + g]);
             }
         }
         if constexpr (SC) {
-            for (int g = 0; g < (WLDS ? C / 16 : a.sc_Cin / 16); ++g) {
-                uint4 u0 = make_uint4(0u, 0u, 0u, 0u), u1 = u0;
-                if constexpr (WLDS) { u0 = xr[2 * g]; u1 = xr[2 * g + 1]; }
-                else if (sc_ok) { u0 = *reinterpret_cast<const uint4*>(sc_row + g * 16); u1 = *reinterpret_cast<const uint4*>(sc_row + g * 16 + 4); }
+            for (int g = 0; g < C / 16; ++g) {
+                const uint4 u0 = xr[2 * g], u1 = xr[2 * g + 1];
                 uint4 bv[TNP];
 #pragma unroll
-                for (int j = 0; j < TNP; ++j) {
-                    if constexpr (WLDS) bv[j] = *reinterpret_cast<const uint4*>(smem + 2 * W_BYTES + ((g >> 1) * C4 + nc + j * 32 + l31) * 64 + (((2 * (g & 1) + kk) ^ swzb) << 4));
-                    else bv[j] = *reinterpret_cast<const uint4*>(wsc + (long)(nc + j * 32 + l31) * a.sc_Cin + g * 16 + 8 * kk);
-                }
+                for (int j = 0; j < TNP; ++j) bv[j] = *reinterpret_cast<const uint4*>(smem + 2 * W_BYTES + ((g >> 1) * C4 + nc + j * 32 + l31) * 64 + (((2 * (g & 1) + kk) ^ swzb) << 4));
                 chain_mfma_parts<PARTS, TNP>(accS, bv, chain_split<PARTS>(u0, u1));
             }
         }
@@ -221,10 +191,7 @@
                 const uint4 u1 = *reinterpret_cast<const uint4*>(&stage[l31 * 32 + (((4 * g + 2 * kk + 1) ^ (l31 & 7)) << 2)]);
                 uint4 bq[TNQ];
 #pragma unroll
-                for (int jq = 0; jq < TNQ; ++jq) {
-                    if constexpr (WLDS) bq[jq] = *reinterpret_cast<const uint4*>(smem + W_BYTES + ((nc / 32 + j) * C + jq * 32 + l31) * 64 + (((2 * g + kk) ^ swzb) << 4));
-                    else bq[jq] = *reinterpret_cast<const uint4*>(w1 + (long)(jq * 32 + l31) * C4 + nc + j * 32 + g * 16 + 8 * kk);
-                }
+                for (int jq = 0; jq < TNQ; ++jq) bq[jq] = *reinterpret_cast<const uint4*>(smem + W_BYTES + ((nc / 32 + j) * C + jq * 32 + l31) * 64 + (((2 * g + kk) ^ swzb) << 4));
                 chain_mfma_parts<PARTS, TNQ>(accQ, bq, chain_split<PARTS>(u0, u1));
             }
             __builtin_amdgcn_wave_barrier();
@@ -253,9 +220,263 @@
     if (aq.range_flag && out_of_range_q) atomicOr(aq.range_flag, 1);
 }
 
-void conv_chain_launch(hipStream_t s, const ConvArgs& p, const ConvArgs& q, int parts, bool wlds, int n_cus)
-{
-    ChainArgs ca{p, q};
+typedef unsigned ch_u32x4 __attribute__((ext_vector_type(4)));
+
+template <int PARTS, int N>
+__device__ __forceinline__ void chain_mfma_frags(f32x16 (&acc)[N], const ch_u32x4* fr, const ChainParts& pt)
+{
+    uint4 bv[N];
+    _Pragma("unroll") for (int j = 0; j < N; ++j) bv[j] = __builtin_bit_cast(uint4, fr[j]);
+    chain_mfma_parts<PARTS, N>(acc, bv, pt);
+}
+
+template <int PARTS, bool SC>
+__global__ __launch_bounds__(256, 2) void k_conv_chain_stream(const ChainArgs ca)
+{
+    constexpr int C = 128, C4 = 4 * C, KT = C / 32, TNQ = C / 32;
+    constexpr int NE = SC ? 4 : 6;
+    constexpr int A_BYTES = KT * 32 * 128;
+    __shared__ __attribute__((aligned(16))) unsigned char smem[4 * (A_BYTES + 32 * 32 * 4)];
+    typedef unsigned srd_t __attribute__((ext_vector_type(4)));
+    const ConvArgs& a = ca.p;
+    const ConvArgs& aq = ca.q;
+    const int t = threadIdx.x;
+    const int wave = t >> 6, lane = t & 63;
+    const int l31 = lane & 31, kk = lane >> 5;
+    const int row0 = (blockIdx.x * 4 + wave) * 32;
+    if (row0 >= a.M) return;
+    unsigned char* const As = smem + wave * A_BYTES;
+    float* const stage = reinterpret_cast<float*>(smem + 4 * A_BYTES) + wave * (32 * 32);
+    const float* const in = static_cast<const float*>(a.in);
+    float* const out = static_cast<float*>(a.out);
+    float* const outq = static_cast<float*>(aq.out);
+
+    auto make_srd = [](const void* p, unsigned long long bytes) {
+        const unsigned long long pa = (unsigned long long)(uintptr_t)p;
+        srd_t r;
+        r[0] = __builtin_amdgcn_readfirstlane((unsigned)pa);
+        r[1] = __builtin_amdgcn_readfirstlane((unsigned)(pa >> 32) & 0xffffu);
+        r[2] = __builtin_amdgcn_readfirstlane((unsigned)bytes);
+        r[3] = 0x00020000u;
+        return r;
+    };
+    const int ngs = SC ? a.sc_Cin / 16 : 0;
+    const srd_t srdW3 = make_srd(ca.w3f, (unsigned long long)C4 * C * 2), srdW1 = make_srd(ca.w1f, (unsigned long long)C * C4 * 2);
+    const srd_t srdWs = make_srd(SC ? ca.wscf : ca.w3f, SC ? (unsigned long long)C4 * a.sc_Cin * 2 : 0ull);
+    const srd_t srdSc = make_srd(a.scale, C4 * 4), srdSh = make_srd(a.shift, C4 * 4);
+    const srd_t srdSc2 = make_srd(SC ? a.sc_scale : a.scale, SC ? C4 * 4 : 0), srdSh2 = make_srd(SC ? a.sc_shift : a.shift, SC ? C4 * 4 : 0);
+    const srd_t srdR = make_srd(SC ? a.sc_in : a.res, SC ? (unsigned long long)a.B * (unsigned long long)a.sc_in_sB * 4ull : (unsigned long long)a.M * C4 * 4ull);
+
+    const unsigned vlane16 = (unsigned)lane * 16u;
+    const int rrow = lane >> 3, c4 = (lane & 7) * 4;
+    const unsigned vss = (unsigned)c4 * 4u;
+    bool ok[4];
+    long mrow[4];
+    unsigned rvo[4];
+#pragma unroll
+    for (int ps = 0; ps < 4; ++ps) {
+        const int m = row0 + 8 * ps + rrow;
+        ok[ps] = m < a.M; mrow[ps] = m;
+        rvo[ps] = (unsigned)m * (unsigned)(C4 * 4) + vss;
+    }
+    unsigned xoff = 0x80000000u;
+    if constexpr (SC) {
+        const int m = row0 + l31;
+        if (m < a.M) {
+            const int ohw = a.OH * a.OW;
+            const int b = m / ohw, rem = m - b * ohw;
+            const int oh = rem / a.OW, ow = rem - oh * a.OW;
+            xoff = (unsigned)(((long)b * a.sc_in_sB + (long)(oh * a.sc_stride) * a.sc_in_sH + (long)(ow * a.sc_stride) * a.sc_in_sW + 8 * kk) * 4);
+        }
+    }
+
+    ch_u32x4 fr[8];
+    ch_u32x4 ev[2][NE];
+    ch_u32x4 xa[2][2];
+#define CH_LOAD(DST, VOFF, SRD, SOFF) asm volatile("buffer_load_dwordx4 %0, %1, %2, %3 offen" : "=v"(DST) : "v"(VOFF), "s"(SRD), "s"(SOFF) : "memory")
+#define CH_LOAD16(DST, VOFF, SRD, SOFF) asm volatile("buffer_load_dwordx4 %0, %1, %2, %3 offen offset:16" : "=v"(DST) : "v"(VOFF), "s"(SRD), "s"(SOFF) : "memory")
+#define CH_WAIT(N_) asm volatile("s_waitcnt vmcnt(%0)" ::"n"(N_) : "memory")
+#define CH_PINS()                                                                                                \
+    {                                                                                                            \
+        _Pragma("unroll") for (int i_ = 0; i_ < 8; ++i_) asm volatile("" : "+v"(fr[i_]));                        \
+        _Pragma("unroll") for (int i_ = 0; i_ < NE; ++i_) { asm volatile("" : "+v"(ev[0][i_])); asm volatile("" : "+v"(ev[1][i_])); } \
+        if constexpr (SC) { asm volatile("" : "+v"(xa[0][0])); asm volatile("" : "+v"(xa[0][1])); asm volatile("" : "+v"(xa[1][0])); asm volatile("" : "+v"(xa[1][1])); } \
+    }
+#define CH_REQ_P(NC_, B_, S_) { const unsigned so_ = (unsigned)((((NC_) >> 5) + ((S_) & 1)) * 8192 + (4 * (B_) + ((S_) >> 1)) * 1024); CH_LOAD(fr[S_], vlane16, srdW3, so_); }
+#define CH_REQ_S(NC_, B_, S_) { const unsigned so_ = (unsigned)(((((NC_) >> 5) + ((S_) & 1)) * ngs + 4 * (B_) + ((S_) >> 1)) * 1024); CH_LOAD(fr[S_], vlane16, srdWs, so_); }
+#define CH_REQ_Q(NC_, J_, S_) { const unsigned so_ = (unsigned)((((NC_) >> 4) + 2 * (J_) + ((S_) >> 2)) * 4096 + ((S_) & 3) * 1024); CH_LOAD(fr[S_], vlane16, srdW1, so_); }
+#define CH_REQ_X(PAR_, G_) { const unsigned so_ = (unsigned)(G_) * 64u; CH_LOAD(xa[PAR_][0], xoff, srdR, so_); CH_LOAD16(xa[PAR_][1], xoff, srdR, so_); }
+#define CH_REQ_E(SET_, COL_, SRDR_)                                                                                   \
+    {                                                                                                            \
+        const unsigned so_ = (unsigned)(COL_) * 4u;                                                              \
+        if constexpr (SC) { CH_LOAD(ev[SET_][0], vss, srdSc, so_); CH_LOAD(ev[SET_][1], vss, srdSh, so_); CH_LOAD(ev[SET_][2], vss, srdSc2, so_); CH_LOAD(ev[SET_][3], vss, srdSh2, so_); } \
+        else {                                                                                                   \
+            _Pragma("unroll") for (int ps_ = 0; ps_ < 4; ++ps_) CH_LOAD(ev[SET_][ps_], rvo[ps_], SRDR_, so_);    \
+            CH_LOAD(ev[SET_][4], vss, srdSc, so_); CH_LOAD(ev[SET_][5], vss, srdSh, so_);                        \
+        }                                                                                                        \
+    }
+
+    CH_REQ_E(0, 0, srdR)
+    CH_REQ_E(1, 32, srdR)
+#pragma unroll
+    for (int s_ = 0; s_ < 8; ++s_) CH_REQ_P(0, 0, s_)
+    if constexpr (SC) { CH_REQ_X(0, 0) CH_REQ_X(1, 1) }
+    const __amdgpu_buffer_rsrc_t rsA = __builtin_amdgcn_make_buffer_rsrc(const_cast<float*>(in), 0, a.M * (C * 4), 0x00020000);
+#pragma unroll
+    for (int it = 0; it < C / 8; ++it) {
+        const int idx = it * 64 + lane;
+        const int r = idx / (C / 4), ch = idx - r * (C / 4);
+        const uint4 v = __builtin_bit_cast(uint4, __builtin_amdgcn_raw_buffer_load_b128(rsA, (row0 + r) * (C * 4) + ch * 16, 0, 0));
+        *reinterpret_cast<uint4*>(As + (ch >> 3) * 4096 + r * 128 + (((ch & 7) ^ ((r >> 1) & 7)) << 4)) = v;
+    }
+    __builtin_amdgcn_wave_barrier();
+
+    const int swz = (l31 >> 1) & 7;
+    const unsigned char* const la = As + l31 * 128;
+    const int ca0 = ((0 + 2 * kk) ^ swz) << 4, ca1 = ((1 + 2 * kk) ^ swz) << 4, ca2 = ((4 + 2 * kk) ^ swz) << 4, ca3 = ((5 + 2 * kk) ^ swz) << 4;
+    const bool relu = a.act == ACT_RELU, reluq = aq.act == ACT_RELU;
+    bool out_of_range = false, out_of_range_q = false;
+
+    f32x16 accQ[TNQ];
+#pragma unroll
+    for (int j = 0; j < TNQ; ++j)
+#pragma unroll
+        for (int e = 0; e < 16; ++e) accQ[j][e] = 0.0f;
+
+    for (int nc = 0; nc < C4; nc += 64) {
+        const int nc_next = (nc + 64) & (C4 - 1);
+        srd_t srdRn = srdR;
+        srdRn[2] = nc + 64 < C4 ? srdR[2] : 0u;
+        f32x16 accP[2], accS[2];
+#pragma unroll
+        for (int j = 0; j < 2; ++j)
+#pragma unroll
+            for (int e = 0; e < 16; ++e) { accP[j][e] = 0.0f; accS[j][e] = 0.0f; }
+#pragma unroll
+        for (int blk = 0; blk < 2; ++blk) {
+#pragma unroll
+            for (int i = 0; i < 4; ++i) {
+                const int h = 4 * blk + i, kt = h >> 1, g = h & 1;
+                CH_WAIT(6);
+                CH_PINS()
+                const uint4 u0 = *reinterpret_cast<const uint4*>(la + kt * 4096 + (g ? ca2 : ca0));
+                const uint4 u1 = *reinterpret_cast<const uint4*>(la + kt * 4096 + (g ? ca3 : ca1));
+                chain_mfma_frags<PARTS, 2>(accP, &fr[2 * i], chain_split<PARTS>(u0, u1));
+                if (blk == 0) { CH_REQ_P(nc, 1, 2 * i) CH_REQ_P(nc, 1, 2 * i + 1) }
+                else if constexpr (SC) { CH_REQ_S(nc, 0, 2 * i) CH_REQ_S(nc, 0, 2 * i + 1) }
+                else { CH_REQ_Q(nc, 0, 2 * i) CH_REQ_Q(nc, 0, 2 * i + 1) }
+            }
+        }
+        if constexpr (SC) {
+            const int nbs = ngs >> 2;
+            for (int b = 0; b < nbs; ++b) {
+                const bool last = b + 1 == nbs;
+#pragma unroll
+                for (int i = 0; i < 4; ++i) {
+                    const int G = 4 * b + i;
+                    CH_WAIT(6);
+                    CH_PINS()
+                    const uint4 u0 = __builtin_bit_cast(uint4, xa[i & 1][0]), u1 = __builtin_bit_cast(uint4, xa[i & 1][1]);
+                    chain_mfma_frags<PARTS, 2>(accS, &fr[2 * i], chain_split<PARTS>(u0, u1));
+                    const int Gn = G + 2 < ngs ? G + 2 : G + 2 - ngs;
+                    CH_REQ_X(i & 1, Gn)
+                    if (last) { CH_REQ_Q(nc, 0, 2 * i) CH_REQ_Q(nc, 0, 2 * i + 1) }
+                    else { CH_REQ_S(nc, b + 1, 2 * i) CH_REQ_S(nc, b + 1, 2 * i + 1) }
+                }
+            }
+        }
+#pragma unroll
+        for (int j = 0; j < 2; ++j) {
+            const int n = nc + j * 32 + c4;
+            if (j == 0) CH_WAIT(8); else CH_WAIT(8 + NE);
+            CH_PINS()
+            float4 rj[4];
+            if constexpr (SC) {
+                chain_stage_acc(stage, accS[j], l31, kk);
+                __builtin_amdgcn_wave_barrier();
+                const float4 sc2 = __builtin_bit_cast(float4, ev[j][2]), sh2 = __builtin_bit_cast(float4, ev[j][3]);
+#pragma unroll
+                for (int ps = 0; ps < 4; ++ps) {
+                    float4 y = *reinterpret_cast<const float4*>(&stage[(8 * ps + rrow) * 32 + (((lane & 7) ^ rrow) << 2)]);
+                    y.x = y.x * sc2.x + sh2.x; y.y = y.y * sc2.y + sh2.y; y.z = y.z * sc2.z + sh2.z; y.w = y.w * sc2.w + sh2.w;
+                    out_of_range = out_of_range || !(fabsf(y.x) < 65504.0f) || !(fabsf(y.y) < 65504.0f) || !(fabsf(y.z) < 65504.0f) || !(fabsf(y.w) < 65504.0f);
+                    rj[ps] = y;
+                }
+                __builtin_amdgcn_wave_barrier();
+            } else {
+#pragma unroll
+                for (int ps = 0; ps < 4; ++ps) rj[ps] = __builtin_bit_cast(float4, ev[j][ps]);
+            }
+            chain_stage_acc(stage, accP[j], l31, kk);
+            __builtin_amdgcn_wave_barrier();
+            const float4 sc = __builtin_bit_cast(float4, ev[j][SC ? 0 : 4]), sh = __builtin_bit_cast(float4, ev[j][SC ? 1 : 5]);
+#pragma unroll
+            for (int ps = 0; ps < 4; ++ps) {
+                float* const sp = &stage[(8 * ps + rrow) * 32 + (((lane & 7) ^ rrow) << 2)];
+                float4 x = *reinterpret_cast<const float4*>(sp);
+                x.x = x.x * sc.x + sh.x; x.y = x.y * sc.y + sh.y; x.z = x.z * sc.z + sh.z; x.w = x.w * sc.w + sh.w;
+                x.x += rj[ps].x; x.y += rj[ps].y; x.z += rj[ps].z; x.w += rj[ps].w;
+                if (relu) { x.x = fmaxf(x.x, 0.f); x.y = fmaxf(x.y, 0.f); x.z = fmaxf(x.z, 0.f); x.w = fmaxf(x.w, 0.f); }
+                if (ok[ps]) {
+                    out_of_range = out_of_range || !(fabsf(x.x) < 65504.0f) || !(fabsf(x.y) < 65504.0f) || !(fabsf(x.z) < 65504.0f) || !(fabsf(x.w) < 65504.0f);
+                    *reinterpret_cast<float4*>(out + mrow[ps] * C4 + n) = x;
+                }
+                *reinterpret_cast<float4*>(sp) = x;
+            }
+            __builtin_amdgcn_wave_barrier();
+            CH_REQ_E(j, nc_next + j * 32, srdRn)
+#pragma unroll
+            for (int g = 0; g < 2; ++g) {
+                CH_WAIT(4 + NE);
+                CH_PINS()
+                const uint4 u0 = *reinterpret_cast<const uint4*>(&stage[l31 * 32 + (((4 * g + 2 * kk) ^ (l31 & 7)) << 2)]);
+                const uint4 u1 = *reinterpret_cast<const uint4*>(&stage[l31 * 32 + (((4 * g + 2 * kk + 1) ^ (l31 & 7)) << 2)]);
+                chain_mfma_frags<PARTS, TNQ>(accQ, &fr[4 * g], chain_split<PARTS>(u0, u1));
+#pragma unroll
+                for (int s_ = 4 * g; s_ < 4 * g + 4; ++s_) {
+                    if (j == 0) CH_REQ_Q(nc, 1, s_)
+                    else CH_REQ_P(nc_next, 0, s_)
+                }
+            }
+            __builtin_amdgcn_wave_barrier();
+        }
+    }
+    CH_WAIT(0);
+    CH_PINS()
+#undef CH_REQ_E
+#undef CH_REQ_X
+#undef CH_REQ_Q
+#undef CH_REQ_S
+#undef CH_REQ_P
+#undef CH_PINS
+#undef CH_WAIT
+#undef CH_LOAD16
+#undef CH_LOAD
+#pragma unroll
+    for (int jq = 0; jq < TNQ; ++jq) {
+        const int n = jq * 32 + c4;
+        chain_stage_acc(stage, accQ[jq], l31, kk);
+        __builtin_amdgcn_wave_barrier();
+        const float4 sc = *reinterpret_cast<const float4*>(aq.scale + n), sh = *reinterpret_cast<const float4*>(aq.shift + n);
+#pragma unroll
+        for (int ps = 0; ps < 4; ++ps) {
+            float4 x = *reinterpret_cast<const float4*>(&stage[(8 * ps + rrow) * 32 + (((lane & 7) ^ rrow) << 2)]);
+            x.x = x.x * sc.x + sh.x; x.y = x.y * sc.y + sh.y; x.z = x.z * sc.z + sh.z; x.w = x.w * sc.w + sh.w;
+            if (reluq) { x.x = fmaxf(x.x, 0.f); x.y = fmaxf(x.y, 0.f); x.z = fmaxf(x.z, 0.f); x.w = fmaxf(x.w, 0.f); }
+            if (ok[ps]) {
+                out_of_range_q = out_of_range_q || !(fabsf(x.x) < 65504.0f) || !(fabsf(x.y) < 65504.0f) || !(fabsf(x.z) < 65504.0f) || !(fabsf(x.w) < 65504.0f);
+                *reinterpret_cast<float4*>(outq + mrow[ps] * C + n) = x;
+            }
+        }
+        __builtin_amdgcn_wave_barrier();
+    }
+    if (a.range_flag && out_of_range) atomicOr(a.range_flag, 1);
+    if (aq.range_flag && out_of_range_q) atomicOr(aq.range_flag, 1);
+}
+
+void conv_chain_launch(hipStream_t s, const ConvArgs& p, const ConvArgs& q, int parts, bool wlds, int n_cus, const void* w3f, const void* w1f, const void* wscf)
+{
+    ChainArgs ca{p, q, w3f, w1f, wscf};
     dim3 grid((p.M + 127) / 128), block(256);
     const bool sc = p.sc_in != nullptr;
     const int C = q.Cout;
@@ -264,16 +485,17 @@
         MRCNN_REQUIRE(C == 64 && (!sc || p.sc_Cin == 64) && n_cus > 0, MRCNN_ERR_INVALID, "conv_chain_launch: the LDS-resident form holds C = 64's filters");
         const int tiles256 = (p.M + 255) / 256;
         grid = dim3(tiles256 < n_cus ? tiles256 : n_cus); block = dim3(512);
-#define MRCNN_CHAIN_W(P_, S_) hipLaunchKernelGGL((k_conv_chain<64, P_, S_, true>), grid, block, 0, s, ca)
+#define MRCNN_CHAIN_W(P_, S_) hipLaunchKernelGGL((k_conv_chain<P_, S_>), grid, block, 0, s, ca)
         if (parts == 3) { if (sc) MRCNN_CHAIN_W(3, true); else MRCNN_CHAIN_W(3, false); }
         else { if (sc) MRCNN_CHAIN_W(2, true); else MRCNN_CHAIN_W(2, false); }
 #undef MRCNN_CHAIN_W
         return;
     }
     MRCNN_REQUIRE(C == 128, MRCNN_ERR_INVALID, "conv_chain_launch: C = 64 runs the LDS-resident form");
-#define MRCNN_CHAIN(C_, P_, S_) hipLaunchKernelGGL((k_conv_chain<C_, P_, S_, false>), grid, block, 0, s, ca)
-    if (parts == 3) { if (sc) MRCNN_CHAIN(128, 3, true); else MRCNN_CHAIN(128, 3, false); }
-    else { if (sc) MRCNN_CHAIN(128, 2, true); else MRCNN_CHAIN(128, 2, false); }
+    MRCNN_REQUIRE(w3f && w1f && (!sc || (wscf && p.sc_Cin % 64 == 0)) && (long)p.M * 2048 < (1L << 31), MRCNN_ERR_INVALID, "conv_chain_launch: the streaming form needs the fragment-ordered filters");
+#define MRCNN_CHAIN(P_, S_) hipLaunchKernelGGL((k_conv_chain_stream<P_, S_>), grid, block, 0, s, ca)
+    if (parts == 3) { if (sc) MRCNN_CHAIN(3, true); else MRCNN_CHAIN(3, false); }
+    else { if (sc) MRCNN_CHAIN(2, true); else MRCNN_CHAIN(2, false); }
 #undef MRCNN_CHAIN
 }
 
diff --git a/mask-rcnn-coreml_amd/csrc/kernels_conv_halo.hip b/mask-rcnn-coreml_amd/csrc/kernels_conv_halo.hip
--- a/mask-rcnn-coreml_amd/csrc/kernels_conv_halo.hip
+++ b/mask-rcnn-coreml_amd/csrc/kernels_conv_halo.hip
@@ -751,15 +751,15 @@
     }
 }
 
-__global__ __launch_bounds__(256) void k_halo_pack(const uint4* __restrict__ src, int Npad, int Cin, int taps, uint4* __restrict__ dst)
+__global__ __launch_bounds__(256) void k_halo_pack(const uint4* __restrict__ src, int Npad, int Cin, int taps, int group_major, uint4* __restrict__ dst)
 {
     const int NH = Cin / 16;
     const long total = (long)(Npad / 32) * NH * taps * 64;
     for (long e = (long)blockIdx.x * 256 + threadIdx.x; e < total; e += (long)gridDim.x * 256) {
         const int piece = (int)(e & 63);
         const long gs = e >> 6;
-        const int step = (int)(gs % (NH * taps));
-        const int g = (int)(gs / (NH * taps));
+        const int step = group_major ? (int)(gs / (Npad / 32)) : (int)(gs % (NH * taps));
+        const int g = group_major ? (int)(gs % (Npad / 32)) : (int)(gs / (NH * taps));
         const int h = step / taps, tap = step - h * taps;
         const int r = piece & 31, half = piece >> 5;
         const int n = g * 32 + r;
@@ -786,14 +786,14 @@
     HIP_CHECK(hipGetLastError());
 }
 
-void conv_halo_pack(hipStream_t s, const void* wgt_std, int Npad, int Cin, DevBuf& out, int taps)
-{
-    MRCNN_REQUIRE(Npad % 32 == 0 && Cin % 16 == 0 && (taps == 9 || taps == 1), MRCNN_ERR_SHAPE, "halo packing: Npad %d / Cin %d / taps %d", Npad, Cin, taps);
+void conv_halo_pack(hipStream_t s, const void* wgt_std, int Npad, int Cin, DevBuf& out, int taps, bool group_major)
+{
+    MRCNN_REQUIRE(Npad % 32 == 0 && Cin % 16 == 0 && (taps == 9 || taps == 1) && (!group_major || taps == 1), MRCNN_ERR_SHAPE, "halo packing: Npad %d / Cin %d / taps %d", Npad, Cin, taps);
     const size_t bytes = (size_t)Npad * taps * Cin * 2;
     out.alloc(bytes);
     const long total = (long)bytes / 16;
     const int grid = (int)((total + 255) / 256 < 4096 ? (total + 255) / 256 : 4096);
-    hipLaunchKernelGGL(k_halo_pack, dim3(grid), dim3(256), 0, s, static_cast<const uint4*>(wgt_std), Npad, Cin, taps, static_cast<uint4*>(out.p));
+    hipLaunchKernelGGL(k_halo_pack, dim3(grid), dim3(256), 0, s, static_cast<const uint4*>(wgt_std), Npad, Cin, taps, group_major ? 1 : 0, static_cast<uint4*>(out.p));
     HIP_CHECK(hipGetLastError());
 }
 
```

Measured after the change: 442.5 (median of 6 runs). No clear change (+0.5%).
